# weipeilun/vjepa2

Hardware: AMD Instinct MI355X
Metric: clips/sec/GPU (ViT-L/16, 16×256², bf16) fwd+bwd; 1→8 GPU scaling (higher is better)
Workload: dtype bf16; 1 GPU; vit_large (RoPE) + predictor 12x384, 16x256^2 clips, B=24/GPU, JEPA train step: target fwd + ctx fwd/bwd (2 masks) + predictor fwd/bwd + L1 + AdamW + EMA; model=vit_large, global_batch=24, seq_len=2048, parallelism=dp1

## Files before the change

include/vjepa_hip.h:

```cpp
#ifndef VJEPA_HIP_H
#define VJEPA_HIP_H
#include <stddef.h>

#ifdef __cplusplus
extern "C" {
#endif

int vj_version(void);
int vj_header_crc(void);
int vj_get_last_error(char* buf, size_t n);
int vj_device_sync(void);

enum {
  VJ_EPI_BF16 = 0,
  VJ_EPI_F32 = 1,
  VJ_EPI_F32_RESID = 2,
  VJ_EPI_GELU = 3,
  VJ_EPI_GELU_BWD = 4,
  VJ_EPI_ROPE = 5,
  VJ_EPI_PARTIAL = 6,
  VJ_EPI_BF16_RESID = 7
};

int vj_gemm_bf16(int M, int N, int K, const void* A, long lda, int a_kmajor, const void* B, long ldb, int b_kmajor,
                 int epi, const float* bias, const void* aux, long ldaux, void* C, long ldc, void* C2, long ldc2,
                 void* stream);
int vj_gemm_bf16_splitk(int M, int N, int K, const void* A, long lda, int a_kmajor, const void* B, long ldb,
                        int b_kmajor, int epi, const float* bias, const void* aux, long ldaux, void* C, long ldc,
                        void* C2, long ldc2, int splitk, float* ws, long ws_floats, void* stream);
int vj_gemm_bf16_wgrad(int M, int N, int K, const void* dy, long lddy, const void* x, long ldx, float* dw, long lddw,
                       int accumulate, float* db, int db_accumulate, int splitk, float* ws, long ws_floats,
                       void* stream);

int vj_attn_fwd(int T, int H, int hd, const void* qkv, long ld, int q_off, int k_off, int v_off, void* o, long ldo,
                float* stats, float scale, int ngroups, const int* nseq, const int* len, void* stream);
int vj_attn_bwd(int T, int H, int hd, const void* qkv, long ld, int q_off, int k_off, int v_off, const void* o,
                long ldo, const void* dout, long lddo, float* stats, void* dqkv, long ldd, float scale, int ngroups,
                const int* nseq, const int* len, const int* rope_ids, int rope_mod, int rope_tpf, int rope_tpr,
                const float* cos_t, const float* sin_t, void* stream);
int vj_attn_fwd_fc(int T, int H, int hd, const void* qkv, long ld, int q_off, int k_off, int v_off, void* o, long ldo,
                   float* stats, float scale, int ngroups, const int* nseq, const int* len, int fblk, void* stream);
int vj_attn_bwd_fc(int T, int H, int hd, const void* qkv, long ld, int q_off, int k_off, int v_off, const void* o,
                   long ldo, const void* dout, long lddo, float* stats, void* dqkv, long ldd, float scale, int ngroups,
                   const int* nseq, const int* len, const int* rope_ids, int rope_mod, int rope_tpf, int rope_tpr,
                   const float* cos_t, const float* sin_t, int fblk, void* stream);
int vj_attn_fwd_ex(int T, int H, int hd, const void* qkv, long ld, int q_off, int k_off, int v_off, void* o, long ldo,
                   float* stats, float scale, int ngroups, const int* nseq, const int* len, int fblk, float dropout_p,
                   unsigned seed, void* stream);
int vj_attn_bwd_ex(int T, int H, int hd, const void* qkv, long ld, int q_off, int k_off, int v_off, const void* o,
                   long ldo, const void* dout, long lddo, float* stats, void* dqkv, long ldd, float scale, int ngroups,
                   const int* nseq, const int* len, const int* rope_ids, int rope_mod, int rope_tpf, int rope_tpr,
                   const float* cos_t, const float* sin_t, int fblk, float dropout_p, unsigned seed, void* stream);

int vj_qkv_rope_gemm(int M, int K, const void* A, long lda, const void* B, long ldb, const float* bias, void* C,
                     long ldc, int H, int hd, const int* ids, int ids_mod, int tpf, int tpr, const float* cos_t,
                     const float* sin_t, int npos, void* stream);

int vj_gemm_fp8(int M, int N, int K, const void* A, long lda, const int* ea, const void* B, long ldb, const int* eb,
                int epi, const float* bias, const void* aux, long ldaux, void* C, long ldc, void* C2, long ldc2,
                void* stream);
int vj_qkv_rope_gemm_fp8(int M, int K, const void* A, long lda, const int* ea, const void* B, long ldb, const int* eb,
                         const float* bias, void* C, long ldc, int H, int hd, const int* ids, int ids_mod, int tpf,
                         int tpr, const float* cos_t, const float* sin_t, int npos, void* stream);
int vj_quant_rows_fp8(int M, int K, const void* x, int x_bf16, long ldx, void* y8, long ldy, int* yexp, void* stream);
int vj_layernorm_fwd_fp8(int M, int D, const void* x, int x_bf16, long ldx, const float* gamma, const float* beta,
                         float eps, void* y8, long ldy, int* yexp, float* mean, float* rstd, void* stream);

int vj_layernorm_fwd(int M, int D, const void* x, int x_bf16, long ldx, const float* gamma, const float* beta,
                     float eps, void* y, int y_f32, long ldy, float* mean, float* rstd, void* stream);
int vj_layernorm_bwd_blocks(int M);
int vj_layernorm_bwd(int M, int D, const void* dy, long lddy, const float* x, long ldx, const float* mean,
                     const float* rstd, const float* gamma, const float* dres_in, long ldri, float* dres, long ldr,
                     void* dres_bf16, long ldrb, float* dgamma, float* dbeta, float* sum_in, float* sum_out, float* ws,
                     long ws_floats, void* stream);
int vj_layernorm_bwd_bf16(int M, int D, const void* dy, long lddy, const void* x, long ldx, const float* mean,
                          const float* rstd, const float* gamma, const void* dres_in, long ldri, void* dres, long ldr,
                          float* dgamma, float* dbeta, float* sum_in, float* sum_out, float* ws, long ws_floats,
                          void* stream);

int vj_gelu_eval(int n, const void* x, void* y, void* dy, void* stream);

int vj_colsum_f32(int M, int N, const void* x, int x_bf16, long ld, float* out, int accumulate, float* ws,
                  long ws_floats, void* stream);

int vj_rope(int T, int H, int hd, void* qkv, long ld, int q_off, int k_off, const int* ids, int ids_mod,
            int tokens_per_frame, int tokens_per_row, const float* cos_tab, const float* sin_tab, int half,
            int inverse, void* stream);

int vj_im2col_tubelet(int R, int K, const long* idx, int B, int C, int Tf, int Hf, int Wf, int tub, int pch,
                      const float* clip, void* out, void* stream);

int vj_gather_rows(int R, int rowbytes, const void* src, long src_ld_bytes, const int* idx, void* dst,
                   long dst_ld_bytes, int scatter, void* stream);
int vj_fill_rows(int R, int D, float* dst, long ldd, const int* idx, const float* vec, void* stream);
int vj_add_rows(int R, int D, float* dst, long ldd, const float* table, long ldt, int trows, const int* idx,
                int idx_mod, void* stream);

int vj_pred_index(int B, int K, int Kp, const long* mx, const long* my, int row0, int bmod, int N, int* pos,
                  int* ctx_dst, int* tgt_rows, int* loss_rows, void* stream);
int vj_ids64to32(long n, const long* in, int* out, void* stream);

int vj_jepa_loss(int R, int D, const void* z, int z_bf16, long ldz, const void* tgt, int tgt_bf16, long ldt,
                 const int* loss_rows,
                 const float* gamma, const float* beta, float eps1, float eps2, float loss_exp, int ngroups,
                 const int* group_rows, float pair_weight, void* dz, long lddz, float* row_loss, float* loss_out,
                 void* stream);

int vj_check_finite(long n, const float* g, int* found_inf, void* stream);
int vj_adamw(long n, float* p, const float* g, float* m, float* v, void* p_bf16, float lr, float beta1, float beta2,
             float eps, float weight_decay, int step, float grad_scale, const int* found_inf, void* stream);
int vj_ema(long n, float* target, const float* online, float momentum, void* target_bf16, void* stream);
int vj_adamw_ema(long n, float* p, const float* g, float* m, float* v, void* p_bf16, float lr, float beta1,
                 float beta2, float eps, float weight_decay, int step, float grad_scale, const int* found_inf,
                 float* target, void* target_bf16, float momentum, void* stream);
int vj_cast_bf16(long n, const float* in, void* out, void* stream);
int vj_proxy_copy(void* dst, const void* src, long bytes, int blocks, int mode, void* stream);
int vj_set_reserved_cus(int n);
int vj_gemm256_plan(int M, int N, int K, int a_kmajor, int b_kmajor, int epi, int cus, int* out6);
int vj_transpose_bf16(int rows, int cols, const void* src, long ld_src, void* dst, long ld_dst, void* stream);
int vj_transpose_bf16_batch(int n, const long* desc, long total_tiles, void* stream);

int vj_swiglu_fwd(int M, int h, const void* x12, long ld, void* out, long ldo, void* stream);
int vj_swiglu_bwd(int M, int h, const void* dh, long lddh, const void* x12, long ld, void* dx12, long lddx,
                  void* stream);
int vj_rowscale_add(int M, int N, const float* y, long ldy, const float* scale, const void* resid, long ldr, void* out,
                    long ldo, int bf16_resid, void* stream);
int vj_rowscale_bf16(int M, int N, const float* dx, long ld, const float* scale, void* out, long ldo, void* stream);
int vj_dropout(int M, int N, const void* x, long ldx, int x_f32, const void* aux, long ldaux, const void* resid,
               long ldr, int resid_f32, void* out, long ldo, float dropout_p, unsigned seed, void* stream);

int vj_mask_count(int B, int duration, int height, int width, int npred, const int* boxes, int t, int h, int w,
                  int max_ctx, int* counts, void* stream);
int vj_mask_emit(int B, int duration, int height, int width, int npred, const int* boxes, int t, int h, int w,
                 int max_ctx, int mode, int k_enc, int k_pred, long* enc, long* pred, void* stream);

int vj_video_transform(int B, int T, int H, int W, int C, int S, const void* frames, const int* params,
                       const float* mean, const float* stdv, float* out, void* stream);

int vj_xattn_ws_floats(int B, int nq, int N, int H, int hd, long* out);
int vj_xattn_fwd(int B, int nq, int N, int H, int hd, const void* q, long ldq, const void* kv, long ldkv, void* o,
                 long ldo, float* lse2, float scale, float* ws, long ws_floats, void* stream);
int vj_xattn_bwd(int B, int nq, int N, int H, int hd, const void* q, long ldq, const void* kv, long ldkv,
                 const void* o, long ldo, const void* dout, long lddo, const float* lse2, float scale, void* dq,
                 long lddq, void* dkv, long lddkv, float* ws, long ws_floats, void* stream);

int vj_xent(int V, int B, int C, const float* logits, long ld, const void* labels, int labels_i64, float* loss,
            float* row_loss, float* dlogits, long lddl, int* pred, int* correct, void* stream);

int vj_focal(int B, int nseg, const float* const* logits, const long* ld, const int* C, const void* const* labels,
             int labels_i64, const unsigned char* const* valid, float* const* dlogits, const long* lddl,
             int* const* tp, int* const* fn, float alpha, float gamma, int k, int loss_kind, float* loss,
             float* row_loss, int* hit, void* stream);

int vj_cem_sample(int S, int rollout, const float* noise, const float* mean, const float* std, float maxnorm,
                  float gripper_clip, const int* axis_on, const float* axis_val, int close_from, float* actions,
                  void* stream);
int vj_pose_step(int S, const float* pose, long ldp, const float* action, long lda, float* out, long ldo,
                 void* stream);
int vj_plan_frame(int S, int R, int D, const float* src, long src_sample_stride, long src_row_stride, int normalize,
                  float eps, float* dst, long dst_sample_stride, const float* goal, float* energy, void* stream);
int vj_cem_update(int S, int rollout, int k, const float* energy, const float* actions, double momentum_mean,
                  double momentum_std, double momentum_mean_gripper, double momentum_std_gripper, float* mean,
                  float* std, int* elite_idx, void* stream);

int vj_gemm_f32(int M, int N, int K, const float* A, long lda, const float* B, long ldb, int epi, const float* bias,
                const float* resid, long ldr, float* C, long ldc, float* C2, long ldc2, void* stream);
int vj_attn_fwd_f32(int T, int H, int hd, const float* qkv, long ld, int q_off, int k_off, int v_off, float* o,
                    long ldo, float* lse, float scale, int ngroups, const int* nseq, const int* len, void* stream);
int vj_rope_f32(int T, int H, int hd, float* qkv, long ld, int q_off, int k_off, const int* ids, int ids_mod,
                int tokens_per_frame, int tokens_per_row, const float* cos_tab, const float* sin_tab, int half,
                void* stream);
int vj_im2col_tubelet_f32(int R, int K, const long* idx, int B, int C, int Tf, int Hf, int Wf, int tub, int pch,
                          const float* clip, float* out, void* stream);

#ifdef __cplusplus
}
#endif
#endif
```

vjepa2_amd/_lib.py:

```python

import ctypes
import os

import torch

LIB_PATH = os.environ.get("VJ_LIB") or os.path.join(os.path.dirname(os.path.abspath(__file__)), "libvjepa_hip.so")

_P = ctypes.c_void_p
_I = ctypes.c_int
_L = ctypes.c_long
_F = ctypes.c_float
_U = ctypes.c_uint
_D = ctypes.c_double

SIGNATURES = {
    "vj_version": [],
    "vj_header_crc": [],
    "vj_get_last_error": [ctypes.c_char_p, ctypes.c_size_t],
    "vj_device_sync": [],
    "vj_gemm_bf16": [_I, _I, _I, _P, _L, _I, _P, _L, _I, _I, _P, _P, _L, _P, _L, _P, _L, _P],
    "vj_gemm_bf16_splitk": [_I, _I, _I, _P, _L, _I, _P, _L, _I, _I, _P, _P, _L, _P, _L, _P, _L, _I, _P, _L, _P],
    "vj_gemm_bf16_wgrad": [_I, _I, _I, _P, _L, _P, _L, _P, _L, _I, _P, _I, _I, _P, _L, _P],
    "vj_attn_fwd": [_I, _I, _I, _P, _L, _I, _I, _I, _P, _L, _P, _F, _I, _P, _P, _P],
    "vj_attn_bwd": [_I, _I, _I, _P, _L, _I, _I, _I, _P, _L, _P, _L, _P, _P, _L, _F, _I, _P, _P, _P, _I, _I, _I, _P,
                    _P, _P],
    "vj_attn_fwd_fc": [_I, _I, _I, _P, _L, _I, _I, _I, _P, _L, _P, _F, _I, _P, _P, _I, _P],
    "vj_attn_bwd_fc": [_I, _I, _I, _P, _L, _I, _I, _I, _P, _L, _P, _L, _P, _P, _L, _F, _I, _P, _P, _P, _I, _I, _I, _P,
                       _P, _I, _P],
    "vj_attn_fwd_ex": [_I, _I, _I, _P, _L, _I, _I, _I, _P, _L, _P, _F, _I, _P, _P, _I, _F, _U, _P],
    "vj_attn_bwd_ex": [_I, _I, _I, _P, _L, _I, _I, _I, _P, _L, _P, _L, _P, _P, _L, _F, _I, _P, _P, _P, _I, _I, _I, _P,
                       _P, _I, _F, _U, _P],
    "vj_qkv_rope_gemm": [_I, _I, _P, _L, _P, _L, _P, _P, _L, _I, _I, _P, _I, _I, _I, _P, _P, _I, _P],
    "vj_layernorm_fwd": [_I, _I, _P, _I, _L, _P, _P, _F, _P, _I, _L, _P, _P, _P],
    "vj_gemm_fp8": [_I, _I, _I, _P, _L, _P, _P, _L, _P, _I, _P, _P, _L, _P, _L, _P, _L, _P],
    "vj_qkv_rope_gemm_fp8": [_I, _I, _P, _L, _P, _P, _L, _P, _P, _P, _L, _I, _I, _P, _I, _I, _I, _P, _P, _I, _P],
    "vj_quant_rows_fp8": [_I, _I, _P, _I, _L, _P, _L, _P, _P],
    "vj_layernorm_fwd_fp8": [_I, _I, _P, _I, _L, _P, _P, _F, _P, _L, _P, _P, _P, _P],
    "vj_video_transform": [_I, _I, _I, _I, _I, _I, _P, _P, _P, _P, _P, _P],
    "vj_mask_count": [_I, _I, _I, _I, _I, _P, _I, _I, _I, _I, _P, _P],
    "vj_mask_emit": [_I, _I, _I, _I, _I, _P, _I, _I, _I, _I, _I, _I, _I, _P, _P, _P],
    "vj_gemm_f32": [_I, _I, _I, _P, _L, _P, _L, _I, _P, _P, _L, _P, _L, _P, _L, _P],
    "vj_attn_fwd_f32": [_I, _I, _I, _P, _L, _I, _I, _I, _P, _L, _P, _F, _I, _P, _P, _P],
    "vj_rope_f32": [_I, _I, _I, _P, _L, _I, _I, _P, _I, _I, _I, _P, _P, _I, _P],
    "vj_im2col_tubelet_f32": [_I, _I, _P, _I, _I, _I, _I, _I, _I, _I, _P, _P, _P],
    "vj_layernorm_bwd_blocks": [_I],
    "vj_layernorm_bwd": [_I, _I, _P, _L, _P, _L, _P, _P, _P, _P, _L, _P, _L, _P, _L, _P, _P, _P, _P, _P, _L, _P],
    "vj_gelu_eval": [_I, _P, _P, _P, _P],
    "vj_layernorm_bwd_bf16": [_I, _I, _P, _L, _P, _L, _P, _P, _P, _P, _L, _P, _L, _P, _P, _P, _P, _P, _L, _P],
    "vj_colsum_f32": [_I, _I, _P, _I, _L, _P, _I, _P, _L, _P],
    "vj_rope": [_I, _I, _I, _P, _L, _I, _I, _P, _I, _I, _I, _P, _P, _I, _I, _P],
    "vj_im2col_tubelet": [_I, _I, _P, _I, _I, _I, _I, _I, _I, _I, _P, _P, _P],
    "vj_gather_rows": [_I, _I, _P, _L, _P, _P, _L, _I, _P],
    "vj_fill_rows": [_I, _I, _P, _L, _P, _P, _P],
    "vj_add_rows": [_I, _I, _P, _L, _P, _L, _I, _P, _I, _P],
    "vj_pred_index": [_I, _I, _I, _P, _P, _I, _I, _I, _P, _P, _P, _P, _P],
    "vj_ids64to32": [_L, _P, _P, _P],
    "vj_jepa_loss": [_I, _I, _P, _I, _L, _P, _I, _L, _P, _P, _P, _F, _F, _F, _I, _P, _F, _P, _L, _P, _P, _P],
    "vj_check_finite": [_L, _P, _P, _P],
    "vj_adamw": [_L, _P, _P, _P, _P, _P, _F, _F, _F, _F, _F, _I, _F, _P, _P],
    "vj_ema": [_L, _P, _P, _F, _P, _P],
    "vj_adamw_ema": [_L, _P, _P, _P, _P, _P, _F, _F, _F, _F, _F, _I, _F, _P, _P, _P, _F, _P],
    "vj_cast_bf16": [_L, _P, _P, _P],
    "vj_proxy_copy": [_P, _P, _L, _I, _I, _P],
    "vj_set_reserved_cus": [_I],
    "vj_gemm256_plan": [_I, _I, _I, _I, _I, _I, _I, ctypes.POINTER(_I)],
    "vj_transpose_bf16": [_I, _I, _P, _L, _P, _L, _P],
    "vj_transpose_bf16_batch": [_I, _P, _L, _P],
    "vj_swiglu_fwd": [_I, _I, _P, _L, _P, _L, _P],
    "vj_swiglu_bwd": [_I, _I, _P, _L, _P, _L, _P, _L, _P],
    "vj_rowscale_add": [_I, _I, _P, _L, _P, _P, _L, _P, _L, _I, _P],
    "vj_rowscale_bf16": [_I, _I, _P, _L, _P, _P, _L, _P],
    "vj_dropout": [_I, _I, _P, _L, _I, _P, _L, _P, _L, _I, _P, _L, _F, _U, _P],
    "vj_xattn_ws_floats": [_I, _I, _I, _I, _I, ctypes.POINTER(_L)],
    "vj_xattn_fwd": [_I, _I, _I, _I, _I, _P, _L, _P, _L, _P, _L, _P, _F, _P, _L, _P],
    "vj_xattn_bwd": [_I, _I, _I, _I, _I, _P, _L, _P, _L, _P, _L, _P, _L, _P, _F, _P, _L, _P, _L, _P, _L, _P],
    "vj_xent": [_I, _I, _I, _P, _L, _P, _I, _P, _P, _P, _L, _P, _P, _P],
    "vj_focal": [_I, _I, _P, _P, _P, _P, _I, _P, _P, _P, _P, _P, _F, _F, _I, _I, _P, _P, _P, _P],
    "vj_cem_sample": [_I, _I, _P, _P, _P, _F, _F, _P, _P, _I, _P, _P],
    "vj_pose_step": [_I, _P, _L, _P, _L, _P, _L, _P],
    "vj_plan_frame": [_I, _I, _I, _P, _L, _L, _I, _F, _P, _L, _P, _P, _P],
    "vj_cem_update": [_I, _I, _I, _P, _P, _D, _D, _D, _D, _P, _P, _P, _P],
}

_lib = None


def load():
    global _lib
    if _lib is not None:
        return _lib
    if not os.path.exists(LIB_PATH):
        raise RuntimeError(
            f"{LIB_PATH} not found: the HIP extension is not built (run `python -m vjepa2_amd.build` or "
            "__graft_entry__.build()). There is no CPU fallback."
        )
    lib = ctypes.CDLL(LIB_PATH)
    for name, args in SIGNATURES.items():
        fn = getattr(lib, name, None)
        if fn is None:
            if os.environ.get("VJ_LIB"):
                continue
            raise RuntimeError(f"{LIB_PATH} does not export {name}: stale build (rebuild the extension)")
        fn.argtypes = args
        fn.restype = ctypes.c_int
    if not os.environ.get("VJ_LIB"):
        import zlib

        hdr = os.path.join(os.path.dirname(os.path.dirname(os.path.abspath(__file__))), "include", "vjepa_hip.h")
        crc_fn = getattr(lib, "vj_header_crc", None)
        if crc_fn is None:
            raise RuntimeError(f"{LIB_PATH} predates vj_header_crc: stale build (rebuild the extension)")
        with open(hdr, "rb") as f:
            want = zlib.crc32(f.read()) & 0xFFFFFFFF
        got = crc_fn() & 0xFFFFFFFF
        if got != want:
            raise RuntimeError(f"{LIB_PATH} was built from another include/vjepa_hip.h (crc {got:08x}, "
                               f"header {want:08x}): stale build (rebuild the extension)")
    _lib = lib
    return lib


def last_error():
    buf = ctypes.create_string_buffer(1024)
    load().vj_get_last_error(buf, 1024)
    return buf.value.decode(errors="replace")


def call(name, *args):
    rc = getattr(load(), name)(*args)
    if rc != 0:
        raise RuntimeError(f"{name} failed (code {rc}): {last_error()}")
    return rc


def int_array(vals):
    vals = list(vals)
    return (ctypes.c_int * max(1, len(vals)))(*vals)
```

vjepa2_amd/csrc/vj_common.h:

```cpp
#pragma once
#include <hip/hip_runtime.h>
#include <stdint.h>
#include <stdio.h>
#include <string.h>

typedef __bf16 bf16x8 __attribute__((ext_vector_type(8)));
typedef __bf16 bf16x4 __attribute__((ext_vector_type(4)));
typedef short s16x4 __attribute__((ext_vector_type(4)));
typedef short s16x8 __attribute__((ext_vector_type(8)));
typedef float f32x16 __attribute__((ext_vector_type(16)));
typedef float f32x4 __attribute__((ext_vector_type(4)));
typedef float f32x2 __attribute__((ext_vector_type(2)));
typedef int i32x4 __attribute__((ext_vector_type(4)));
typedef int i32x8 __attribute__((ext_vector_type(8)));
typedef unsigned short bf16_t;

#define LDS_AS __attribute__((address_space(3)))

enum {
  VJ_OK = 0,
  VJ_ERR_ARG = 1,
  VJ_ERR_LAUNCH = 2,
  VJ_ERR_UNSUPPORTED = 3,
};

void vj_set_error(const char* fmt, ...);

#define VJ_CHECK_ARG(cond, ...)          \
  do {                                   \
    if (!(cond)) {                       \
      vj_set_error(__VA_ARGS__);         \
      return VJ_ERR_ARG;                 \
    }                                    \
  } while (0)

#define VJ_LAUNCH_CHECK(what)                                                    \
  do {                                                                           \
    hipError_t e_ = hipGetLastError();                                           \
    if (e_ != hipSuccess) {                                                      \
      vj_set_error("%s: launch failed: %s", what, hipGetErrorString(e_));        \
      return VJ_ERR_LAUNCH;                                                      \
    }                                                                            \
  } while (0)

__device__ __forceinline__ float bf2f(bf16_t v) { return __uint_as_float(((uint32_t)v) << 16); }
__device__ __forceinline__ bf16_t f2bf(float f) {
  __bf16 b = (__bf16)f;
  return __builtin_bit_cast(bf16_t, b);
}
typedef __bf16 bf16x2_t __attribute__((ext_vector_type(2)));
__device__ __forceinline__ uint32_t pack_bf2(float lo, float hi) {
  return __builtin_bit_cast(uint32_t, __builtin_convertvector((f32x2){lo, hi}, bf16x2_t));
}

template <int CTRL>
__device__ __forceinline__ float dpp(float v) {
  return __int_as_float(__builtin_amdgcn_mov_dpp(__float_as_int(v), CTRL, 0xF, 0xF, false));
}
template <int CTRL>
__device__ __forceinline__ uint32_t dpp_u(uint32_t v) {
  return (uint32_t)__builtin_amdgcn_mov_dpp((int)v, CTRL, 0xF, 0xF, false);
}
constexpr int DPP_XOR1 = 0xB1;
constexpr int DPP_XOR2 = 0x4E;
constexpr int DPP_HALF_MIRROR = 0x141;
constexpr int DPP_MIRROR = 0x140;
__device__ __forceinline__ float sum_xor16(float v) {
  const auto r = __builtin_amdgcn_permlane16_swap(__float_as_uint(v), __float_as_uint(v), false, false);
  return __uint_as_float(r[0]) + __uint_as_float(r[1]);
}
__device__ __forceinline__ float sum_xor32(float v) {
  const auto r = __builtin_amdgcn_permlane32_swap(__float_as_uint(v), __float_as_uint(v), false, false);
  return __uint_as_float(r[0]) + __uint_as_float(r[1]);
}
__device__ __forceinline__ float max_xor16(float v) {
  const auto r = __builtin_amdgcn_permlane16_swap(__float_as_uint(v), __float_as_uint(v), false, false);
  return fmaxf(__uint_as_float(r[0]), __uint_as_float(r[1]));
}
__device__ __forceinline__ float max_xor32(float v) {
  const auto r = __builtin_amdgcn_permlane32_swap(__float_as_uint(v), __float_as_uint(v), false, false);
  return fmaxf(__uint_as_float(r[0]), __uint_as_float(r[1]));
}

__device__ __forceinline__ float wave_sum(float v) {
  v += dpp<DPP_XOR1>(v);
  v += dpp<DPP_XOR2>(v);
  v += dpp<DPP_HALF_MIRROR>(v);
  v += dpp<DPP_MIRROR>(v);
  v = sum_xor16(v);
  return sum_xor32(v);
}
__device__ __forceinline__ float wave_max(float v) {
  v = fmaxf(v, dpp<DPP_XOR1>(v));
  v = fmaxf(v, dpp<DPP_XOR2>(v));
  v = fmaxf(v, dpp<DPP_HALF_MIRROR>(v));
  v = fmaxf(v, dpp<DPP_MIRROR>(v));
  v = max_xor16(v);
  return max_xor32(v);
}

__device__ __forceinline__ __amdgpu_buffer_rsrc_t make_rsrc(const void* base, uint32_t bytes) {
  const unsigned long long a = (unsigned long long)base;
  const unsigned long long lo = (unsigned)__builtin_amdgcn_readfirstlane((int)(unsigned)a);
  const unsigned long long hi = (unsigned)__builtin_amdgcn_readfirstlane((int)(unsigned)(a >> 32));
  const int n = __builtin_amdgcn_readfirstlane((int)bytes);
  return __builtin_amdgcn_make_buffer_rsrc((void*)(lo | (hi << 32)), (short)0, n, 0x00020000);
}
#ifndef VJ_DMA_CPOL
#define VJ_DMA_CPOL 0
#endif
__device__ __forceinline__ void dma16(__amdgpu_buffer_rsrc_t r, LDS_AS void* lds_wave_base, uint32_t voff) {
  __builtin_amdgcn_raw_ptr_buffer_load_lds(r, lds_wave_base, 16, voff, 0, 0, VJ_DMA_CPOL);
}
#define VJ_OOB 0x80000000u

__device__ __forceinline__ s16x4 ds_read_tr16(const LDS_AS void* p) {
  return __builtin_amdgcn_ds_read_tr16_b64_v4i16((LDS_AS s16x4*)p);
}
__device__ __forceinline__ s16x4 ds_read_tr16_async(const LDS_AS void* p) {
  s16x4 r;
  asm volatile("ds_read_b64_tr_b16 %0, %1" : "=v"(r) : "v"((uint32_t)(uintptr_t)p) : "memory");
  return r;
}
__device__ __forceinline__ void lds_wait() { asm volatile("s_waitcnt lgkmcnt(0)" ::: "memory"); }
template <typename T, int N>
__device__ __forceinline__ void tie(T (&x)[N]) {
#pragma unroll
  for (int i = 0; i < N; ++i) asm volatile("" : "+v"(x[i]));
}

__device__ __forceinline__ uint32_t f8pack4(float a, float b, float c, float d) {
  int w = __builtin_amdgcn_cvt_pk_fp8_f32(__builtin_amdgcn_fmed3f(a, -448.f, 448.f),
                                          __builtin_amdgcn_fmed3f(b, -448.f, 448.f), 0, false);
  w = __builtin_amdgcn_cvt_pk_fp8_f32(__builtin_amdgcn_fmed3f(c, -448.f, 448.f),
                                      __builtin_amdgcn_fmed3f(d, -448.f, 448.f), w, true);
  return (uint32_t)w;
}

enum { EPI_BF16 = 0, EPI_F32 = 1, EPI_F32_RESID = 2, EPI_GELU = 3, EPI_GELU_BWD = 4, EPI_ROPE = 5, EPI_PARTIAL = 6,
       EPI_BF16_RESID = 7, EPI_PARTIAL_RS = 8 };

static inline int vj_cdiv(long a, long b) { return (int)((a + b - 1) / b); }

__device__ __forceinline__ void gelu_cdf_grad(float x, float& cdf, float& dy) {
  const float zs = x * 0.84932180028801904f;
  const float a = fabsf(zs);
  const float t = __builtin_amdgcn_rcpf(fmaf(0.27273748087922250f, a, 1.f));
  float p = fmaf(1.061405429f, t, -1.453152027f);
  p = fmaf(p, t, 1.421413741f);
  p = fmaf(p, t, -0.284496736f);
  p = fmaf(p, t, 0.254829592f);
  p *= t;
  const float e = __builtin_amdgcn_exp2f(-zs * zs);
  cdf = fmaf(0.5f, copysignf(fmaf(-p, e, 1.f), zs), 0.5f);
  dy = fmaf(x * 0.39894228040143268f, e, cdf);
}
__device__ __forceinline__ void gelu_fwd_grad(float x, float& y, float& dy) {
  float cdf;
  gelu_cdf_grad(x, cdf, dy);
  y = x * cdf;
}

struct VjRope {
  const int* ids;
  int mod, tpf, tpr;
  int half, hd, D;
  const float* cos_t;
  const float* sin_t;
  int npos;
};

__device__ __forceinline__ uint32_t clamp_u31(long b) {
  if (b < 0) return 0;
  return b > 0x7fffffffL ? 0x7fffffffu : (uint32_t)b;
}

__device__ __forceinline__ uint32_t drop_mix(uint32_t x) {
  x ^= x >> 16;
  x *= 0x7feb352du;
  x ^= x >> 15;
  x *= 0x846ca68bu;
  x ^= x >> 16;
  return x;
}
__device__ __forceinline__ uint32_t drop_row(uint32_t seed, uint32_t row) { return drop_mix(seed ^ (row * 0x9e3779b1u)); }
__device__ __forceinline__ uint32_t drop_u(uint32_t rowkey, uint32_t col) { return drop_mix(rowkey + col * 0x85ebca77u); }
uint32_t vj_drop_thresh(float p);
```

vjepa2_amd/csrc/vj_gemm.hip:

```cpp
#include <stdlib.h>
#include "vj_common.h"

namespace {


struct GemmArgs {
  const bf16_t* A;
  const bf16_t* B;
  int M, N, K;
  long lda, ldb;
  void* C;
  long ldc;
  void* C2;
  long ldc2;
  const float* bias;
  const void* aux;
  long ldaux;
  int kslice;
  float* ws;
  const float* rs_ws = nullptr;
  float* rs_out = nullptr;
  int rs_acc = 0;
};

// ... 35 lines not shown

template <bool KMAJ>
__device__ __forceinline__ bf16x8 load_frag(const LDS_AS char* lds, int rb, int s, int lane) {
  if constexpr (KMAJ) {
    const int r = rb + (lane & 31);
    const int c = (2 * s + (lane >> 5)) ^ ((r >> 1) & 7);
    return *(const LDS_AS bf16x8*)(lds + r * 128 + c * 16);
  } else {
    const int r = rb + 16 * ((lane >> 4) & 1) + 4 * (lane & 3);
    const int kr = 16 * s + 8 * (lane >> 5) + ((lane >> 2) & 3);
    const int sw = (kr & 3) << 2;
    const int off = ((r >> 3) ^ sw) * 16 + (r & 7) * 2;
    const s16x4 lo = ds_read_tr16(lds + kr * 256 + off);
    const s16x4 hi = ds_read_tr16(lds + (kr + 4) * 256 + off);
    s16x8 v = {lo[0], lo[1], lo[2], lo[3], hi[0], hi[1], hi[2], hi[3]};
    return __builtin_bit_cast(bf16x8, v);
  }
}

template <bool AK, bool BKM, int EPI>
__global__ __launch_bounds__(256) void k_gemm(GemmArgs g) {
  __shared__ __attribute__((aligned(16))) char smem_raw[4 * TILE_BYTES];
  LDS_AS char* smem = (LDS_AS char*)smem_raw;
  const int lane = threadIdx.x & 63;
  const int wave = threadIdx.x >> 6;
  const int wm = wave >> 1, wn = wave & 1;
  const int m0 = blockIdx.y * BM, n0 = blockIdx.x * BN;

  const bf16_t* abase = AK ? g.A + (long)m0 * g.lda : g.A + m0;
  const bf16_t* bbase = BKM ? g.B + (long)n0 * g.ldb : g.B + n0;
  const uint32_t abytes = AK ? clamp_bytes((long)(g.M - m0) * g.lda * 2) : clamp_bytes(((long)g.K * g.lda - m0) * 2);
  const uint32_t bbytes = BKM ? clamp_bytes((long)(g.N - n0) * g.ldb * 2) : clamp_bytes(((long)g.K * g.ldb - n0) * 2);
  const __amdgpu_buffer_rsrc_t ra = make_rsrc(abase, abytes);
  const __amdgpu_buffer_rsrc_t rb = make_rsrc(bbase, bbytes);
  const int mleft = g.M - m0, nleft = g.N - n0;

  f32x16 acc[2][2];
#pragma unroll
  for (int i = 0; i < 2; ++i)
#pragma unroll
    for (int j = 0; j < 2; ++j)
#pragma unroll
      for (int r = 0; r < 16; ++r) acc[i][j][r] = 0.f;

  const int kb = blockIdx.z * g.kslice;
  const int ke = min(g.K, kb + g.kslice);
  const int nk = (ke - kb + BK - 1) / BK;
  stage_tile<AK>(ra, g.lda, mleft, kb, ke, smem, wave, lane);
  stage_tile<BKM>(rb, g.ldb, nleft, kb, ke, smem + TILE_BYTES, wave, lane);
  __syncthreads();

  for (int kt = 0; kt < nk; ++kt) {
    const int cur = kt & 1;
    if (kt + 1 < nk) {
      LDS_AS char* nxt = smem + (cur ^ 1) * 2 * TILE_BYTES;
      stage_tile<AK>(ra, g.lda, mleft, kb + (kt + 1) * BK, ke, nxt, wave, lane);
      stage_tile<BKM>(rb, g.ldb, nleft, kb + (kt + 1) * BK, ke, nxt + TILE_BYTES, wave, lane);
    }
    const LDS_AS char* As = smem + cur * 2 * TILE_BYTES;
    const LDS_AS char* Bs = As + TILE_BYTES;
#pragma unroll
    for (int s = 0; s < 4; ++s) {
      bf16x8 a0 = load_frag<AK>(As, wm * 64, s, lane);
      bf16x8 a1 = load_frag<AK>(As, wm * 64 + 32, s, lane);
      bf16x8 b0 = load_frag<BKM>(Bs, wn * 64, s, lane);
      bf16x8 b1 = load_frag<BKM>(Bs, wn * 64 + 32, s, lane);
      acc[0][0] = __builtin_amdgcn_mfma_f32_32x32x16_bf16(a0, b0, acc[0][0], 0, 0, 0);
      acc[0][1] = __builtin_amdgcn_mfma_f32_32x32x16_bf16(a0, b1, acc[0][1], 0, 0, 0);
      acc[1][0] = __builtin_amdgcn_mfma_f32_32x32x16_bf16(a1, b0, acc[1][0], 0, 0, 0);
      acc[1][1] = __builtin_amdgcn_mfma_f32_32x32x16_bf16(a1, b1, acc[1][1], 0, 0, 0);
    }
    __syncthreads();
  }

#pragma unroll
  for (int j = 0; j < 2; ++j) {
    const int n = n0 + wn * 64 + j * 32 + (lane & 31);
    if (n >= g.N) continue;
    const float bv = (EPI != EPI_PARTIAL && g.bias) ? g.bias[n] : 0.f;
#pragma unroll
    for (int i = 0; i < 2; ++i) {
#pragma unroll
      for (int r = 0; r < 16; ++r) {
        const int m = m0 + wm * 64 + i * 32 + (r & 3) + 8 * (r >> 2) + 4 * (lane >> 5);
        if (m >= g.M) continue;
        const float v = acc[i][j][r] + bv;
        if constexpr (EPI == EPI_PARTIAL) {
          g.ws[((long)blockIdx.z * g.M + m) * g.N + n] = v;
        } else if constexpr (EPI == EPI_BF16) {
          ((bf16_t*)g.C)[(long)m * g.ldc + n] = f2bf(v);
        } else if constexpr (EPI == EPI_F32) {
          ((float*)g.C)[(long)m * g.ldc + n] = v;
        } else if constexpr (EPI == EPI_F32_RESID) {
          const float res = ((const float*)g.aux)[(long)m * g.ldaux + n];
          ((float*)g.C)[(long)m * g.ldc + n] = res + v;
        } else if constexpr (EPI == EPI_BF16_RESID) {
          const float res = bf2f(((const bf16_t*)g.aux)[(long)m * g.ldaux + n]);
          ((bf16_t*)g.C)[(long)m * g.ldc + n] = f2bf(res + v);
        } else if constexpr (EPI == EPI_GELU) {
          float y, dy;
          gelu_fwd_grad(bf2f(f2bf(v)), y, dy);
          if (g.C) ((bf16_t*)g.C)[(long)m * g.ldc + n] = f2bf(dy);
          ((bf16_t*)g.C2)[(long)m * g.ldc2 + n] = f2bf(y);
        } else if constexpr (EPI == EPI_GELU_BWD) {
          const float dg = bf2f(((const bf16_t*)g.aux)[(long)m * g.ldaux + n]);
          ((bf16_t*)g.C)[(long)m * g.ldc + n] = f2bf(acc[i][j][r] * dg);
        }
      }
    }
  }
}

__device__ __forceinline__ void reduce_rowsum(const GemmArgs& g, int splitk, int m) {
  float s = 0.f;
  for (int z = 0; z < splitk; ++z) s += g.rs_ws[(long)z * g.M + m];
  g.rs_out[m] = g.rs_acc ? g.rs_out[m] + s : s;
}

__global__ void k_splitk_reduce4(GemmArgs g, int splitk, int epi) {
  const long i = ((long)blockIdx.x * blockDim.x + threadIdx.x) * 4;
  const long total = (long)g.M * g.N;
  if (i >= total) return;
  const int m = (int)(i / g.N), n = (int)(i % g.N);
  if (g.rs_out && n == 0) reduce_rowsum(g, splitk, m);
  float4 v = g.bias ? *(const float4*)(g.bias + n) : make_float4(0.f, 0.f, 0.f, 0.f);
  for (int z = 0; z < splitk; ++z) {
    const float4 w = *(const float4*)(g.ws + (long)z * total + i);
    v.x += w.x; v.y += w.y; v.z += w.z; v.w += w.w;
  }
  if (epi == EPI_F32_RESID) {
    const float4 r = *(const float4*)((const float*)g.aux + (long)m * g.ldaux + n);
    *(float4*)((float*)g.C + (long)m * g.ldc + n) = make_float4(r.x + v.x, r.y + v.y, r.z + v.z, r.w + v.w);
  } else if (epi == EPI_F32) {
    *(float4*)((float*)g.C + (long)m * g.ldc + n) = v;
  } else {
    *(uint2*)((bf16_t*)g.C + (long)m * g.ldc + n) = make_uint2(pack_bf2(v.x, v.y), pack_bf2(v.z, v.w));
  }
}

__global__ void k_splitk_reduce(GemmArgs g, int splitk, int epi) {
  const long i = (long)blockIdx.x * blockDim.x + threadIdx.x;
  const long total = (long)g.M * g.N;
  if (i >= total) return;
  const int m = (int)(i / g.N), n = (int)(i % g.N);
  if (g.rs_out && n == 0) reduce_rowsum(g, splitk, m);
  float v = g.bias ? g.bias[n] : 0.f;
  for (int z = 0; z < splitk; ++z) v += g.ws[(long)z * total + i];
  if (epi == EPI_F32_RESID) {
    ((float*)g.C)[(long)m * g.ldc + n] = ((const float*)g.aux)[(long)m * g.ldaux + n] + v;
  } else if (epi == EPI_F32) {
    ((float*)g.C)[(long)m * g.ldc + n] = v;
  } else {
    ((bf16_t*)g.C)[(long)m * g.ldc + n] = f2bf(v);
  }
}

template <bool AK, bool BKM>
int launch_epi(int epi, const GemmArgs& g, dim3 grid, hipStream_t st) {
  switch (epi) {
    case EPI_PARTIAL: hipLaunchKernelGGL((k_gemm<AK, BKM, EPI_PARTIAL>), grid, dim3(256), 0, st, g); break;
    case EPI_BF16: hipLaunchKernelGGL((k_gemm<AK, BKM, EPI_BF16>), grid, dim3(256), 0, st, g); break;
    case EPI_F32: hipLaunchKernelGGL((k_gemm<AK, BKM, EPI_F32>), grid, dim3(256), 0, st, g); break;
    case EPI_F32_RESID: hipLaunchKernelGGL((k_gemm<AK, BKM, EPI_F32_RESID>), grid, dim3(256), 0, st, g); break;
    case EPI_GELU: hipLaunchKernelGGL((k_gemm<AK, BKM, EPI_GELU>), grid, dim3(256), 0, st, g); break;
    case EPI_GELU_BWD: hipLaunchKernelGGL((k_gemm<AK, BKM, EPI_GELU_BWD>), grid, dim3(256), 0, st, g); break;
    case EPI_BF16_RESID: hipLaunchKernelGGL((k_gemm<AK, BKM, EPI_BF16_RESID>), grid, dim3(256), 0, st, g); break;
    default: vj_set_error("vj_gemm_bf16: unknown epilogue %d", epi); return VJ_ERR_ARG;
  }
  VJ_LAUNCH_CHECK("vj_gemm_bf16");
  return VJ_OK;
}

}

int vj_gemm256_partial(int M, int N, int K, const void* A, long lda, int a_kmajor, const void* B, long ldb,
                       int b_kmajor, int kslice, int splitk, float* ws, hipStream_t st, float* rsum);
int vj_gemm256_dispatch(int M, int N, int K, const void* A, long lda, int a_kmajor, const void* B, long ldb,
                        int b_kmajor, int epi, const float* bias, const void* aux, long ldaux, void* C, long ldc,
                        void* C2, long ldc2, hipStream_t st, const void* rope);

static int gemm_splitk(int M, int N, int K, const void* A, long lda, int a_kmajor, const void* B, long ldb,
                       int b_kmajor, int epi, const float* bias, const void* aux, long ldaux, void* C, long ldc,
                       void* C2, long ldc2, int splitk, float* ws, long ws_floats, void* stream, float* rs_out,
                       int rs_acc, int* rs_done) {
  if (rs_done) *rs_done = 0;
  if (M == 0 || N == 0) return VJ_OK;
  VJ_CHECK_ARG(M > 0 && N > 0 && K > 0, "vj_gemm_bf16: bad dims M=%d N=%d K=%d", M, N, K);
  VJ_CHECK_ARG(epi == EPI_BF16 || epi == EPI_F32 || epi == EPI_F32_RESID || epi == EPI_GELU || epi == EPI_GELU_BWD ||
                   epi == EPI_BF16_RESID,
               "vj_gemm_bf16: epilogue %d is not a public epilogue (0-4, 7; include/vjepa_hip.h)", epi);
  VJ_CHECK_ARG(A && B, "vj_gemm_bf16: null operand");
  VJ_CHECK_ARG(((uintptr_t)A & 15) == 0 && ((uintptr_t)B & 15) == 0, "vj_gemm_bf16: operands must be 16-B aligned");
  VJ_CHECK_ARG(lda % 8 == 0 && ldb % 8 == 0, "vj_gemm_bf16: lda/ldb must be multiples of 8 (lda=%ld ldb=%ld)", lda, ldb);
  VJ_CHECK_ARG(a_kmajor ? (K % 8 == 0) : (M % 8 == 0), "vj_gemm_bf16: A contiguous dim must be %%8");
  VJ_CHECK_ARG(b_kmajor ? (K % 8 == 0) : (N % 8 == 0), "vj_gemm_bf16: B contiguous dim must be %%8");
  VJ_CHECK_ARG(a_kmajor ? lda >= K : lda >= M, "vj_gemm_bf16: lda too small");
  VJ_CHECK_ARG(b_kmajor ? ldb >= K : ldb >= N, "vj_gemm_bf16: ldb too small");
  VJ_CHECK_ARG(epi == EPI_GELU ? (C2 != nullptr) : (C != nullptr), "vj_gemm_bf16: null output");
  VJ_CHECK_ARG((epi != EPI_F32_RESID && epi != EPI_GELU_BWD && epi != EPI_BF16_RESID) || aux,
               "vj_gemm_bf16: epilogue needs aux");
  VJ_CHECK_ARG((a_kmajor ? (long)M * lda : (long)K * lda) * 2 < 0x7fffffffL, "vj_gemm_bf16: A too large");
  VJ_CHECK_ARG((b_kmajor ? (long)N * ldb : (long)K * ldb) * 2 < 0x7fffffffL, "vj_gemm_bf16: B too large");
  if (splitk < 1) splitk = 1;
  int kslice = K;
  if (splitk > 1) {
    VJ_CHECK_ARG(epi == EPI_BF16 || epi == EPI_F32 || epi == EPI_F32_RESID,
                 "vj_gemm_bf16_splitk: split-K supports the BF16/F32/F32_RESID epilogues");
    kslice = vj_cdiv(vj_cdiv(K, splitk), BK) * BK;
    splitk = vj_cdiv(K, kslice);
    VJ_CHECK_ARG(ws && ws_floats >= (long)splitk * M * N, "vj_gemm_bf16_splitk: workspace needs %ld floats",
                 (long)splitk * M * N);
  }
  GemmArgs g{(const bf16_t*)A, (const bf16_t*)B, M, N, K, lda, ldb, C, ldc, C2, ldc2, bias, aux, ldaux, kslice, ws};
  dim3 grid(vj_cdiv(N, BN), vj_cdiv(M, BM), splitk);
  VJ_CHECK_ARG(grid.y <= 65535, "vj_gemm_bf16: M too large");
  hipStream_t st = (hipStream_t)stream;
  if (splitk == 1 && M >= 1024 && N >= 128) {
    const int rc = vj_gemm256_dispatch(M, N, K, A, lda, a_kmajor, B, ldb, b_kmajor, epi, bias, aux, ldaux, C, ldc, C2,
                                       ldc2, st, nullptr);
    if (rc != VJ_ERR_UNSUPPORTED) return rc;
  }
  if (splitk > 1) {
    int rc = VJ_ERR_UNSUPPORTED;
    const bool rs = rs_out && ws_floats >= (long)splitk * M * N + (long)splitk * M;
    rc = vj_gemm256_partial(M, N, K, A, lda, a_kmajor, B, ldb, b_kmajor, kslice, splitk, ws, st,
                            rs ? ws + (long)splitk * M * N : nullptr);
    if (rc == VJ_OK && rs) {
      g.rs_ws = ws + (long)splitk * M * N;
      g.rs_out = rs_out;
      g.rs_acc = rs_acc;
      if (rs_done) *rs_done = 1;
    }
    if (rc == VJ_ERR_UNSUPPORTED) {
      if (a_kmajor && b_kmajor) rc = launch_epi<true, true>(EPI_PARTIAL, g, grid, st);
      else if (a_kmajor && !b_kmajor) rc = launch_epi<true, false>(EPI_PARTIAL, g, grid, st);
      else if (!a_kmajor && b_kmajor) rc = launch_epi<false, true>(EPI_PARTIAL, g, grid, st);
      else rc = launch_epi<false, false>(EPI_PARTIAL, g, grid, st);
    }
    if (rc) return rc;
    const long total = (long)M * N;
    const bool vec = N % 4 == 0 && ldc % 4 == 0 && (epi != EPI_F32_RESID || ldaux % 4 == 0) &&
                     ((uintptr_t)C & 15) == 0 && ((uintptr_t)aux & 15) == 0 && ((uintptr_t)bias & 15) == 0;
    if (vec)
      hipLaunchKernelGGL(k_splitk_reduce4, dim3((unsigned)((total / 4 + 255) / 256)), dim3(256), 0, st, g, splitk, epi);
    else
      hipLaunchKernelGGL(k_splitk_reduce, dim3((unsigned)((total + 255) / 256)), dim3(256), 0, st, g, splitk, epi);
    VJ_LAUNCH_CHECK("vj_gemm_bf16_splitk(reduce)");
    return VJ_OK;
  }
  if (a_kmajor && b_kmajor) return launch_epi<true, true>(epi, g, grid, st);
  if (a_kmajor && !b_kmajor) return launch_epi<true, false>(epi, g, grid, st);
  if (!a_kmajor && b_kmajor) return launch_epi<false, true>(epi, g, grid, st);
  return launch_epi<false, false>(epi, g, grid, st);
}

extern "C" int vj_gemm_bf16_splitk(int M, int N, int K, const void* A, long lda, int a_kmajor, const void* B,
                                   long ldb, int b_kmajor, int epi, const float* bias, const void* aux, long ldaux,
                                   void* C, long ldc, void* C2, long ldc2, int splitk, float* ws, long ws_floats,
                                   void* stream) {
  return gemm_splitk(M, N, K, A, lda, a_kmajor, B, ldb, b_kmajor, epi, bias, aux, ldaux, C, ldc, C2, ldc2, splitk, ws,
                     ws_floats, stream, nullptr, 0, nullptr);
}

extern "C" int vj_colsum_f32(int M, int N, const void* x, int x_bf16, long ld, float* out, int accumulate, float* ws,
                             long ws_floats, void* stream);

extern "C" int vj_gemm_bf16_wgrad(int M, int N, int K, const void* dy, long lddy, const void* x, long ldx,
                                  float* dw, long lddw, int accumulate, float* db, int db_accumulate, int splitk,
                                  float* ws, long ws_floats, void* stream) {
  VJ_CHECK_ARG(dw, "vj_gemm_bf16_wgrad: null dw");
  int done = 0;
  const int rc = gemm_splitk(M, N, K, dy, lddy, 0, x, ldx, 0, accumulate ? EPI_F32_RESID : EPI_F32, nullptr,
                             accumulate ? dw : nullptr, lddw, dw, lddw, nullptr, 0, splitk, ws, ws_floats, stream, db,
                             db_accumulate, &done);
  if (rc || !db || done || M == 0) return rc;
  return vj_colsum_f32(K, M, dy, 1, lddy, db, db_accumulate, ws, ws_floats, stream);
}

extern "C" int vj_gemm_bf16(int M, int N, int K, const void* A, long lda, int a_kmajor, const void* B, long ldb,
                            int b_kmajor, int epi, const float* bias, const void* aux, long ldaux, void* C, long ldc,
                            void* C2, long ldc2, void* stream) {
  return vj_gemm_bf16_splitk(M, N, K, A, lda, a_kmajor, B, ldb, b_kmajor, epi, bias, aux, ldaux, C, ldc, C2, ldc2, 1,
                             nullptr, 0, stream);
}
```

vjepa2_amd/csrc/vj_gemm256.hip:

```cpp
#include <stdlib.h>
#include <atomic>
#include <type_traits>
#include "vj_gemm_tile.h"

namespace {

#if VJ_GEMM_STAMPS
__device__ long vj_gemm_stamps[2048 * 16 * 4];
__device__ long vj_gemm_istamps[2048 * 2 * 16];
#endif

template <int N>
__device__ __forceinline__ void vm_wait() {
  static_assert(N >= 0 && N <= 24 && N % 4 == 0, "vm_wait: add the count");
  if constexpr (N == 0) asm volatile("s_waitcnt vmcnt(0)" ::: "memory");
  else if constexpr (N == 4) asm volatile("s_waitcnt vmcnt(4)" ::: "memory");
  else if constexpr (N == 8) asm volatile("s_waitcnt vmcnt(8)" ::: "memory");
  else if constexpr (N == 12) asm volatile("s_waitcnt vmcnt(12)" ::: "memory");
  else if constexpr (N == 16) asm volatile("s_waitcnt vmcnt(16)" ::: "memory");
  else if constexpr (N == 20) asm volatile("s_waitcnt vmcnt(20)" ::: "memory");
  else asm volatile("s_waitcnt vmcnt(24)" ::: "memory");
}

template <bool AK, bool BKM, int EPI, int BN, bool F8 = false, int NWV = 8, int BMT = 256, int STG = 0>
__global__ __launch_bounds__(NWV * 64, 2) void k_gemm256(G256 g) {
  using Cfg = Cfg256<AK, BKM, EPI, BN, F8, NWV, BMT, STG>;
  static_assert(Cfg::supported, "k_gemm256: unsupported (layout, epilogue, tile) combination");
  constexpr bool PART = Cfg::PART, RS = Cfg::RS, DIRECT = Cfg::DIRECT, AUX = Cfg::AUX, F32OUT = Cfg::F32OUT;
  constexpr bool EARLY1 = Cfg::EARLY1, GTAB = Cfg::GTAB, S64 = Cfg::S64, ASYNC = Cfg::ASYNC;
  constexpr int BM = Cfg::BM, MH = Cfg::MH, BK = Cfg::BK, NT = Cfg::NT, WNX = Cfg::WNX, WM = Cfg::WM, WN = Cfg::WN;
  constexpr int PB = Cfg::PB, NTN = Cfg::NTN, A_BYTES = Cfg::A_BYTES, STAGE = Cfg::STAGE, DMAW = Cfg::DMAW;
  constexpr int NSL = Cfg::NSL, DIST = Cfg::DIST, USZ = Cfg::USZ, GSZ = Cfg::GSZ, SA = Cfg::SA, SB = Cfg::SB;
  constexpr int EA = Cfg::EA, EB = Cfg::EB, WRS = Cfg::WRS;
  static_assert(EA >= 2 && EB >= 3, "S64 waits assume at least one interval of DMA lead");
  static_assert(Cfg::SLOT_END <= Cfg::LDS_BYTES && Cfg::GTAB_END <= Cfg::LDS_BYTES && Cfg::RING_END <= Cfg::LDS_BYTES &&
                    Cfg::S64_END <= Cfg::RING_END && Cfg::TAB_END <= Cfg::LDS_BYTES && Cfg::RTAB_END <= Cfg::LDS_BYTES &&
                    Cfg::IMG_END <= Cfg::SLOT_END,
                "an LDS region ends past the array");
  static_assert(Cfg::lds_disjoint, "LDS regions overlap");
  static_assert(Cfg::LDS_BYTES * Cfg::BLOCKS_PER_CU <= LDS_PER_CU, "the CU's workgroups exceed its LDS");
  auto rowoff = [](int i) { return S64 ? (i >> 2) * 128 + (i & 3) * 16 : i * 16; };
  __shared__ __attribute__((aligned(16))) char smem_raw[Cfg::LDS_BYTES];
  LDS_AS char* smem = (LDS_AS char*)smem_raw;
  [[maybe_unused]] LDS_AS char* ring = smem + Cfg::RING0;

  const int lane = threadIdx.x & 63;
  const int wave = __builtin_amdgcn_readfirstlane(threadIdx.x >> 6);
  const int wr = wave / WNX, wc = wave % WNX;

  const int ntile = g.tiles_m * g.tiles_n;
  const int nb = ntile * g.nsplit;
  const int P = gridDim.x >> 3;
  const int xcd = blockIdx.x & 7, jb = blockIdx.x >> 3;
  const int q = nb >> 3, rmd = nb & 7;
  const int run0 = xcd < rmd ? xcd * (q + 1) : rmd * (q + 1) + (xcd - rmd) * q;
  const int runend = run0 + q + (xcd < rmd ? 1 : 0);
  if (run0 + jb >= runend) return;

  auto make_tile = [&](int wg) {
    Tile T;
    const int z = wg / ntile, w = wg - z * ntile;
    int tm, tn;
    if (g.group > 0) {
      const int per = g.group * g.tiles_n, grp = w / per, first = grp * g.group;
      const int gm = min(g.tiles_m - first, g.group), loc = w - grp * per;
      tm = first + loc % gm;
      tn = loc / gm;
    } else {
      tm = w / g.tiles_n;
      tn = w - tm * g.tiles_n;
    }
    T.m0 = __builtin_amdgcn_readfirstlane(tm * BM);
    T.n0 = __builtin_amdgcn_readfirstlane(tn * BN);
    T.z = __builtin_amdgcn_readfirstlane(z);
    const int kb = T.z * g.kslice;
    T.Keff = min(g.K, kb + g.kslice) - kb;
    T.nk = (T.Keff + BK - 1) / BK;
    return T;
  };
  auto rsrc_a = [&](const Tile& T) {
    const int kb = T.z * g.kslice;
    const bf16_t* abase = AK ? g.A + (long)T.m0 * g.lda + kb : g.A + (long)kb * g.lda + T.m0;
    return make_rsrc(abase, AK ? clampb((long)(g.M - T.m0) * g.lda * 2 - kb * 2L)
                               : clampb(((long)(g.K - kb) * g.lda - T.m0) * 2));
  };
  auto rsrc_b = [&](const Tile& T) {
    const int kb = T.z * g.kslice;
    const bf16_t* bbase = BKM ? g.B + (long)T.n0 * g.ldb + kb : g.B + (long)kb * g.ldb + T.n0;
    return make_rsrc(bbase, BKM ? clampb((long)(g.N - T.n0) * g.ldb * 2 - kb * 2L)
                                : clampb(((long)(g.K - kb) * g.ldb - T.n0) * 2));
  };
  const bool iss = DMAW == 8 || wave < DMAW;
  auto load_k = [&](__amdgpu_buffer_rsrc_t ra, __amdgpu_buffer_rsrc_t rb, const Tile& T, int t, int slot,
                    int lane) {
    LDS_AS char* s = smem + slot * STAGE;
    if (iss) {
      stage<AK, BM, false, DMAW, BK, WNX, PB>(ra, g.lda, g.M - T.m0, t * BK, T.Keff, s, wave, lane);
      stage<BKM, BN, DIRECT, DMAW, BK, WNX, PB>(rb, g.ldb, g.N - T.n0, t * BK, T.Keff, s + A_BYTES, wave, lane);
    }
  };
  auto load_tile = [&](const Tile& T, int t, int slot, int lane) {
    load_k(rsrc_a(T), rsrc_b(T), T, t, slot, lane);
  };
  auto load_tile8 = [&](const Tile& T, int t, int slot, int lane) {
    LDS_AS char* s = smem + slot * STAGE;
    stage<AK, BM, false, NWV, BK, WNX, PB>(rsrc_a(T), g.lda, g.M - T.m0, t * BK, T.Keff, s, wave, lane);
    stage<BKM, BN, DIRECT, NWV, BK, WNX, PB>(rsrc_b(T), g.ldb, g.N - T.n0, t * BK, T.Keff, s + A_BYTES, wave, lane);
  };

  constexpr int RTR = EPI == EPI_ROPE ? (ROPE_TAB_MAX + NT - 1) / NT : 0;
  [[maybe_unused]] f32x2 rpf[RTR > 0 ? RTR : 1];
  [[maybe_unused]] const int ntab = EPI == EPI_ROPE ? g.rope.npos * g.rope.half : 0;
  if constexpr (EPI == EPI_ROPE) {
#pragma unroll
    for (int i = 0; i < RTR; ++i) {
      const int e = threadIdx.x + NT * i;
      rpf[i] = e < ntab ? f32x2{g.rope.cos_t[e], g.rope.sin_t[e]} : f32x2{0.f, 0.f};
    }
  }
  [[maybe_unused]] LDS_AS int* rpos = (LDS_AS int*)(smem + Cfg::RPOS_OFF);
  [[maybe_unused]] LDS_AS f32x2* rtab = (LDS_AS f32x2*)(smem + Cfg::RTAB_OFF);

  int wg = run0 + jb;
  Tile cur = make_tile(wg);
  int par = 0;

  [[maybe_unused]] const int nku = STG ? (g.K + 31) / 32 : 0;
  [[maybe_unused]] int dwg = wg, dku = 0, dpos = 0;
  [[maybe_unused]] __amdgpu_buffer_rsrc_t drs;
  [[maybe_unused]] uint32_t dvo[4];
  const bool isA = wave < 4;
  auto dma_setup = [&]() {
    if (dwg < runend) {
      const Tile T = make_tile(dwg);
      const int left = isA ? g.M - T.m0 : g.N - T.n0;
      const long ld = isA ? g.lda : g.ldb;
      if (isA) drs = make_rsrc(g.A + (long)T.m0 * g.lda, clampb((long)left * g.lda * 2));
      else drs = make_rsrc(g.B + (long)T.n0 * g.ldb, clampb((long)left * g.ldb * 2));
#pragma unroll
      for (int j = 0; j < 4; ++j) {
        const int r = (4 * (wave & 3) + j) * 16 + (lane >> 2);
        const int c = (lane & 3) ^ kswz32(r);
        int gr = r;
        if (!isA) {
          const int rl = r & 63;
          gr = (r - rl) + 4 * (rl & 15) + (rl >> 4);
        }
        dvo[j] = gr < left ? (uint32_t)(gr * ld * 2 + c * 16) : VJ_OOB;
      }
    } else {
#pragma unroll
      for (int j = 0; j < 4; ++j) dvo[j] = VJ_OOB;
    }
  };
  auto dma_half = [&](auto h_c) {
    constexpr int h = decltype(h_c)::value;
    LDS_AS char* dst = ring + (dpos % NSL) * USZ + (isA ? 0 : 16384) + (4 * (wave & 3) + 2 * h) * 1024;
    const int soff = __builtin_amdgcn_readfirstlane(dku * 64);
    __builtin_amdgcn_raw_ptr_buffer_load_lds(drs, dst, 16, dvo[2 * h], soff, 0, 0);
    __builtin_amdgcn_raw_ptr_buffer_load_lds(drs, dst + 1024, 16, dvo[2 * h + 1], soff, 0, 0);
    if constexpr (h == 1) {
      ++dpos;
      if (++dku == nku) {
        dku = 0;
        dwg += P;
        dma_setup();
      }
    }
  };
  [[maybe_unused]] const int nks = S64 ? g.K >> 6 : 0;
  [[maybe_unused]] const long dld = isA ? g.lda : g.ldb;
  [[maybe_unused]] const bf16_t* dbase = isA ? g.A : g.B;
  [[maybe_unused]] int dleft = 0, dq = 0, dk = 0, q64 = 0;
  auto dma_setup64 = [&]() {
    if (dwg < runend) {
      const Tile T = make_tile(dwg);
      dbase = isA ? g.A + (long)T.m0 * g.lda : g.B + (long)T.n0 * g.ldb;
      dleft = isA ? g.M - T.m0 : g.N - T.n0;
    } else {
      dleft = 0;
    }
  };
  auto dma_gran = [&]() {
    const int h = dk & 1;
    const __amdgpu_buffer_rsrc_t rs = make_rsrc(dbase + (h ? 128 * dld : 0), clampb((long)(dleft - 128 * h) * dld * 2));
    const int soff = __builtin_amdgcn_readfirstlane((dk >> 1) * 128);
    LDS_AS char* dst = ring + (isA ? dq % SA : SA + dq % SB) * GSZ + (wave & 3) * 4096;
#pragma unroll
    for (int k = 0; k < 4; ++k)
      __builtin_amdgcn_raw_ptr_buffer_load_lds(rs, dst + k * 1024, 16, dvo[k], soff, 0, 0);
    ++dq;
    if (++dk == 2 * nks) {
      dk = 0;
      dwg += P;
      dma_setup64();
    }
  };
  if constexpr (S64) {
#pragma unroll
    for (int k = 0; k < 4; ++k) {
      const int r = 32 * (wave & 3) + 8 * k + (lane >> 3);
      const int c = (lane & 7) ^ ((r >> 1) & 7);
      const int rl = r & 63;
      const int gr = isA ? r : (r - rl) + 4 * (rl & 15) + (rl >> 4);
      dvo[k] = (uint32_t)(gr * dld * 2 + c * 16);
    }
    dma_setup64();
    for (int i = 0; i < (isA ? EA : EB); ++i) dma_gran();
  } else if constexpr (STG) {
    dma_setup();
#pragma unroll
    for (int i = 0; i < DIST; ++i) {
      dma_half(std::integral_constant<int, 0>{});
      dma_half(std::integral_constant<int, 1>{});
    }
  } else {
    load_tile(cur, 0, 0, lane);
    if (cur.nk > 1) load_tile(cur, 1, 1, lane);
  }
  if constexpr (EPI == EPI_ROPE) {
#pragma unroll
    for (int i = 0; i < RTR; ++i) {
      const int e = threadIdx.x + NT * i;
      if (e < ntab) rtab[e] = rpf[i];
    }
  }
  if constexpr (GTAB) gelu_tab_fill((LDS_AS f32x2*)(smem + Cfg::GTAB_OFF), threadIdx.x, NT);

  f32x4 acc[2 * MH][NTN];
  auto accv = [&](int i, int j, int r) -> float { return acc[i][j][r]; };
  auto accs = [&](int i, int j, int r, float v) { acc[i][j][r] = v; };
  bf16x8 Aa[MH], Ab[MH], Ba[NTN], Bb[NTN];
  auto rdA = [&](bf16x8 (&X)[MH], int slot, int mh, int ks) {
    const LDS_AS char* s = smem + slot * STAGE;
#pragma unroll
    for (int i = 0; i < MH; ++i) X[i] = frag<AK, BM, BK>(s, wr * WM + (mh * MH + i) * 16, ks, lane);
  };
  auto rdB = [&](bf16x8 (&Y)[NTN], int slot, int ks) {
    const LDS_AS char* s = smem + slot * STAGE + A_BYTES;
#pragma unroll
    for (int j = 0; j < NTN; ++j) Y[j] = frag<BKM, BN, BK>(s, wc * WN + j * 16, ks, lane);
  };
  [[maybe_unused]] int f8sa[8], f8sb[NTN];
  [[maybe_unused]] i32x8 Xa[2], Xb[2], Y8[NTN];
  auto cat = [](bf16x8 lo, bf16x8 hi) {
    const i32x4 l = __builtin_bit_cast(i32x4, lo), h = __builtin_bit_cast(i32x4, hi);
    return __builtin_shufflevector(l, h, 0, 1, 2, 3, 4, 5, 6, 7);
  };
  auto rdA8 = [&](i32x8 (&X)[2], int slot, int qq) {
    const LDS_AS char* s = smem + slot * STAGE;
#pragma unroll
    for (int i = 0; i < 2; ++i)
      X[i] = cat(frag<AK, BM>(s, wr * 128 + (2 * qq + i) * 16, 0, lane),
                 frag<AK, BM>(s, wr * 128 + (2 * qq + i) * 16, 1, lane));
  };
  auto rdB8 = [&](int j0, int j1, int slot) {
    const LDS_AS char* s = smem + slot * STAGE + A_BYTES;
#pragma unroll
    for (int j = j0; j < j1; ++j)
      Y8[j] = cat(frag<BKM, BN>(s, wc * WN + j * 16, 0, lane), frag<BKM, BN>(s, wc * WN + j * 16, 1, lane));
  };
  auto mm8 = [&](const i32x8 (&X)[2], int qq, int j0, int j1) {
#pragma unroll
    for (int i = 0; i < 2; ++i)
#pragma unroll
      for (int j = j0; j < j1; ++j)
        acc[2 * qq + i][j] = __builtin_amdgcn_mfma_scale_f32_16x16x128_f8f6f4(X[i], Y8[j], acc[2 * qq + i][j], 0, 0,
                                                                              0, f8sa[2 * qq + i], 0, f8sb[j]);
  };
  [[maybe_unused]] float rsa = 0.f, rsb = 0.f;
  [[maybe_unused]] bool rs_on = false;
  auto rsum8 = [](const bf16x8& x, float s) {
    typedef __bf16 bf16x2_t __attribute__((ext_vector_type(2)));
    const bf16x2_t one = {(__bf16)1.0f, (__bf16)1.0f};
    s = __builtin_amdgcn_fdot2_f32_bf16(__builtin_shufflevector(x, x, 0, 1), one, s, false);
    s = __builtin_amdgcn_fdot2_f32_bf16(__builtin_shufflevector(x, x, 2, 3), one, s, false);
    s = __builtin_amdgcn_fdot2_f32_bf16(__builtin_shufflevector(x, x, 4, 5), one, s, false);
    return __builtin_amdgcn_fdot2_f32_bf16(__builtin_shufflevector(x, x, 6, 7), one, s, false);
  };
  auto rs_phase = [&](const bf16x8 (&X)[MH], int mh) {
    if constexpr (RS && MH == 4) {
      if (rs_on && (wc >> 1) == mh) {
        if (wc & 1) {
          rsa = rsum8(X[2], rsa);
          rsb = rsum8(X[3], rsb);
        } else {
          rsa = rsum8(X[0], rsa);
          rsb = rsum8(X[1], rsb);
        }
      }
    }
  };
  auto mm = [&](const bf16x8 (&X)[MH], int mh, const bf16x8 (&Y)[NTN]) {
#pragma unroll
    for (int i = 0; i < MH; ++i)
#pragma unroll
      for (int j = 0; j < NTN; ++j)
        acc[mh * MH + i][j] = __builtin_amdgcn_mfma_f32_16x16x32_bf16(X[i], Y[j], acc[mh * MH + i][j], 0, 0, 0);
    rs_phase(X, mh);
  };
  auto mm_rows = [&](const bf16x8 (&X)[MH], int mh, const bf16x8 (&Y)[NTN], int i0, int i1) {
#pragma unroll
    for (int i = 0; i < MH; ++i)
      if (i >= i0 && i < i1)
#pragma unroll
        for (int j = 0; j < NTN; ++j)
          acc[mh * MH + i][j] = __builtin_amdgcn_mfma_f32_16x16x32_bf16(X[i], Y[j], acc[mh * MH + i][j], 0, 0, 0);
    if (i1 == MH) rs_phase(X, mh);
  };
  auto release = [&](bf16x8 (&X)[MH], bf16x8 (&Y)[NTN]) {
    if constexpr (ASYNC) {
      lds_wait();
      tie(X);
      tie(Y);
    }
  };

#if VJ_GEMM_STAMPS
  int stamp_it = 0;
#endif
  for (;;) {
#if VJ_GEMM_STAMPS
    const long st0 = __builtin_amdgcn_s_memtime();
    long st_k1 = 0;
#endif
    const int wgn = wg + P;
    const bool has_next = wgn < runend;
    const int nk = cur.nk;
    const int parn = (nk + par) & 1;
    const int sle = (nk - 1 + par) & 1;
    [[maybe_unused]] int pf_id = 0;
    if constexpr (EPI == EPI_ROPE) {
      const int t = threadIdx.x;
      if (t < BM && cur.m0 + t < g.M) pf_id = g.rope.ids ? g.rope.ids[cur.m0 + t] : (cur.m0 + t) % g.rope.mod;
    }
#pragma unroll
    for (int i = 0; i < 2 * MH; ++i)
#pragma unroll
      for (int j = 0; j < NTN; ++j) acc[i][j] = f32x4{0.f, 0.f, 0.f, 0.f};
    if constexpr (RS) {
      rs_on = g.rsum && cur.n0 == 0;
      rsa = rsb = 0.f;
    }
    if constexpr (F8) {
#pragma unroll
      for (int i = 0; i < 8; ++i) {
        const int m = cur.m0 + wr * 128 + i * 16 + (lane & 15);
        f8sa[i] = 127 + (m < g.M ? g.ea[m] : 0);
      }
#pragma unroll
      for (int j = 0; j < NTN; ++j) {
        int r = wc * WN + j * 16 + (lane & 15);
        if constexpr (DIRECT) {
          const int rl = r % WN;
          r = (r - rl) + NTN * (rl & 15) + (rl >> 4);
        }
        const int n = cur.n0 + r;
        f8sb[j] = 127 + (n < g.N ? g.eb[n] : 0);
      }
    }
    [[maybe_unused]] float biasp[NTN];
    if constexpr (STG) {
      const int nbp = cur.n0 + wc * WN + NTN * (lane & 15);
#pragma unroll
      for (int j = 0; j < NTN; ++j) biasp[j] = 0.f;
      if (EPI != EPI_GELU_BWD && g.bias && nbp < g.N) {
        const float4 bv = *(const float4*)(g.bias + nbp);
        biasp[0] = bv.x; biasp[1] = bv.y; biasp[2] = bv.z; biasp[3] = bv.w;
      }
    }
    [[maybe_unused]] f32x4 auxr[AUX && STG ? 4 : 1];
    auto stg_aux = [&] {
      if constexpr (AUX && STG) {
        const int m = cur.m0 + wr * WRS + 4 * (lane >> 4);
        const int n = cur.n0 + wc * WN + NTN * (lane & 15);
#pragma unroll
        for (int r = 0; r < 4; ++r) {
          const bool ok = m + r < g.M && n < g.N;
          const long off = ok ? (long)(m + r) * g.ldaux + n : 0;
          if constexpr (EPI == EPI_F32_RESID) {
            auxr[r] = *(const f32x4*)((const float*)g.aux + off);
          } else {
            const uint2 x = *(const uint2*)((const bf16_t*)g.aux + off);
            auxr[r] = f32x4{__builtin_bit_cast(float, x.x), __builtin_bit_cast(float, x.y), 0.f, 0.f};
          }
        }
      }
    };
    if constexpr (S64) {
      if (wg == run0 + jb) {
        if (isA) vm_wait<4 * (EA - 1)>();
        else vm_wait<4 * (EB - 2)>();
        __builtin_amdgcn_s_barrier();
        if (wr == 1) __builtin_amdgcn_s_barrier();
      }
      auto bar = [] {
        __builtin_amdgcn_sched_barrier(0);
        __builtin_amdgcn_s_barrier();
        __builtin_amdgcn_sched_barrier(0);
      };
      auto mm64 = [&](auto h_c) {
        constexpr int h = decltype(h_c)::value;
#pragma unroll
        for (int i = 0; i < 4; ++i)
#pragma unroll
          for (int j = 0; j < 4; ++j)
            acc[4 * h + i][j] = __builtin_amdgcn_mfma_f32_16x16x32_bf16(Aa[i], Ba[j], acc[4 * h + i][j], 0, 0, 0);
#pragma unroll
        for (int i = 0; i < 4; ++i)
#pragma unroll
          for (int j = 0; j < 4; ++j)
            acc[4 * h + i][j] = __builtin_amdgcn_mfma_f32_16x16x32_bf16(Ab[i], Bb[j], acc[4 * h + i][j], 0, 0, 0);
      };
      const int qt = q64;
#if VJ_GEMM_STAMPS
      long* ist = (stamp_it == 1 && (wave & 3) == 0 && lane == 0 && blockIdx.x < 2048)
                      ? vj_gemm_istamps + ((long)blockIdx.x * 2 + (wave >> 2)) * 16 : nullptr;
      auto istamp = [&](int s, int k) {
        if (ist && s >= 1 && s <= 4) ist[(s - 1) * 4 + k] = __builtin_amdgcn_s_memtime();
      };
#else
      auto istamp = [](int, int) {};
#endif
      for (int s = 0; s < nks; ++s) {
        const int p = qt + 2 * s;
        const LDS_AS char* sA0 = ring + (p % SA) * GSZ;
        const LDS_AS char* sA1 = ring + ((p + 1) % SA) * GSZ;
        const LDS_AS char* sB = ring + (SA + (p + (wc >> 1)) % SB) * GSZ;
        const bool last = s + 1 == nks;
#pragma unroll
        for (int i = 0; i < 4; ++i) Aa[i] = frag<true, 128, 64>(sA0, wr * 64 + i * 16, 0, lane);
#pragma unroll
        for (int j = 0; j < 4; ++j) Ba[j] = frag<true, 128, 64>(sB, (wc & 1) * 64 + j * 16, 0, lane);
#pragma unroll
        for (int i = 0; i < 4; ++i) Ab[i] = frag<true, 128, 64>(sA0, wr * 64 + i * 16, 1, lane);
#pragma unroll
        for (int j = 0; j < 4; ++j) Bb[j] = frag<true, 128, 64>(sB, (wc & 1) * 64 + j * 16, 1, lane);
        dma_gran();
        if (isA) vm_wait<4 * (EA - 1)>();
        if (AUX && last) stg_aux();
        bar();
        istamp(s, 0);
        mm64(std::integral_constant<int, 0>{});
        bar();
        istamp(s, 1);
#pragma unroll
        for (int i = 0; i < 4; ++i) Aa[i] = frag<true, 128, 64>(sA1, wr * 64 + i * 16, 0, lane);
#pragma unroll
        for (int i = 0; i < 4; ++i) Ab[i] = frag<true, 128, 64>(sA1, wr * 64 + i * 16, 1, lane);
        dma_gran();
        constexpr int WA = 4 * (EA - 1), WB = 4 * (EB - 2);
        if (AUX && last) {
          if (isA) vm_wait<WA + 4>();
          else vm_wait<WB + 4>();
        } else {
          if (isA) vm_wait<WA>();
          else vm_wait<WB>();
        }
        bar();
        istamp(s, 2);
        mm64(std::integral_constant<int, 1>{});
#if VJ_GEMM_STAMPS
        if (s == 0) st_k1 = __builtin_amdgcn_s_memtime();
#endif
        if (!last || wr == 0) bar();
        istamp(s, 3);
      }
      q64 = qt + 2 * nks;
    } else if constexpr (STG) {
      if (wg == run0 + jb) {
        if constexpr (DIST == 3) asm volatile("s_waitcnt vmcnt(8)" ::: "memory");
        else asm volatile("s_waitcnt vmcnt(4)" ::: "memory");
        __builtin_amdgcn_s_barrier();
        if (wr == 1) __builtin_amdgcn_s_barrier();
      }
      const int q0 = dpos - DIST;
      auto bar = [] {
        __builtin_amdgcn_sched_barrier(0);
        __builtin_amdgcn_s_barrier();
        __builtin_amdgcn_sched_barrier(0);
      };
      for (int u = 0; u < nku; ++u) {
        const LDS_AS char* sA = ring + ((q0 + u) % NSL) * USZ;
        const LDS_AS char* sB = sA + 16384;
#pragma unroll
        for (int i = 0; i < 4; ++i) Aa[i] = frag<true, 256, 32>(sA, wr * 128 + i * 16, 0, lane);
#pragma unroll
        for (int j = 0; j < NTN; ++j) Ba[j] = frag<true, 256, 32>(sB, wc * WN + j * 16, 0, lane);
#pragma unroll
        for (int i = 0; i < 4; ++i) Ab[i] = frag<true, 256, 32>(sA, wr * 128 + 64 + i * 16, 0, lane);
        dma_half(std::integral_constant<int, 0>{});
        dma_half(std::integral_constant<int, 1>{});
        if (AUX && u == nku - 1 && nku > 1) {
          if constexpr (DIST == 3) asm volatile("s_waitcnt vmcnt(12)" ::: "memory");
          else asm volatile("s_waitcnt vmcnt(8)" ::: "memory");
        } else {
          if constexpr (DIST == 3) asm volatile("s_waitcnt vmcnt(8)" ::: "memory");
          else asm volatile("s_waitcnt vmcnt(4)" ::: "memory");
        }
        if (AUX && u == nku - 2) stg_aux();
        if (AUX && nku == 1) stg_aux();
        bar();
        mm(Aa, 0, Ba);
        mm(Ab, 1, Ba);
#if VJ_GEMM_STAMPS
        if (u == 1) st_k1 = __builtin_amdgcn_s_memtime();
#endif
        if (u + 1 < nku || wr == 0) bar();
      }
    } else {
      asm volatile("s_waitcnt vmcnt(0)" ::: "memory");
      __syncthreads();
      if constexpr (F8) {
        rdA8(Xa, par, 0);
        rdB8(0, NTN / 2, par);
      } else {
        rdA(Aa, par, 0, 0);
        rdB(Ba, par, 0);
      }

      const __amdgpu_buffer_rsrc_t ra = rsrc_a(cur), rb = rsrc_b(cur);
      constexpr bool SPREAD = NWV == 8 && !F8 && BK == 64;
      constexpr int SPLIT = MH == 4 ? SPLIT_AT : MH - 1;
      auto ktile = [&](const int t, auto tail_c) {
        constexpr bool TAIL = decltype(tail_c)::value;
        const int sl = (t + par) & 1;
        if constexpr (F8) {
          rdB8(NTN / 2, NTN, sl);
          rdA8(Xb, sl, 1);
          __builtin_amdgcn_sched_barrier(0);
          mm8(Xa, 0, 0, NTN / 2);
          mm8(Xa, 0, NTN / 2, NTN);
          __builtin_amdgcn_sched_barrier(0);
          rdA8(Xa, sl, 2);
          __builtin_amdgcn_sched_barrier(0);
          mm8(Xb, 1, 0, NTN);
          __builtin_amdgcn_sched_barrier(0);
          rdA8(Xb, sl, 3);
          __builtin_amdgcn_sched_barrier(0);
          mm8(Xa, 2, 0, NTN);
          __builtin_amdgcn_sched_barrier(0);
        } else if constexpr (BK == 32) {
          rdA(Ab, sl, 1, 0);
          __builtin_amdgcn_sched_barrier(0);
          mm(Aa, 0, Ba);
          __builtin_amdgcn_sched_barrier(0);
        } else {
          release(Aa, Ba);
          rdA(Ab, sl, 1, 0);
          __builtin_amdgcn_sched_barrier(0);
          mm(Aa, 0, Ba);
          __builtin_amdgcn_sched_barrier(0);
          release(Ab, Ba);
          rdA(Aa, sl, 0, 1);
          rdB(Bb, sl, 1);
          __builtin_amdgcn_sched_barrier(0);
          mm(Ab, 1, Ba);
          __builtin_amdgcn_sched_barrier(0);
          release(Aa, Bb);
          rdA(Ab, sl, 1, 1);
          __builtin_amdgcn_sched_barrier(0);
          mm(Aa, 0, Bb);
          __builtin_amdgcn_sched_barrier(0);
        }
        if (t + 1 < nk) asm volatile("s_waitcnt vmcnt(0) lgkmcnt(0)" ::: "memory");
        else asm volatile("s_waitcnt lgkmcnt(0)" ::: "memory");
        if constexpr (ASYNC) {
          tie(Ab);
          tie(Bb);
        }
        __builtin_amdgcn_s_barrier();
        __builtin_amdgcn_sched_barrier(0);
        if constexpr (!TAIL) {
          if constexpr (SPREAD) {
            if (iss)
              stage<AK, BM, false, DMAW, BK, WNX, PB>(ra, g.lda, g.M - cur.m0, (t + 2) * BK, cur.Keff,
                                                       smem + sl * STAGE, wave, lane);
          } else {
            load_k(ra, rb, cur, t + 2, sl, lane);
          }
        } else if (has_next) {
          int lt = lane;
          asm volatile("" : "+v"(lt));
          const Tile nx = make_tile(wgn);
          if (t + 2 == nk) {
            load_tile(nx, 0, sl, lt);
          } else {
            if (nk == 1) load_tile(nx, 0, sl ^ 1, lt);
            if (EARLY1 && nx.nk > 1) load_tile8(nx, 1, sl, lt);
          }
        }
        auto b_pieces = [&] {
          if (iss)
            stage<BKM, BN, DIRECT, DMAW, BK, WNX, PB>(rb, g.ldb, g.N - cur.n0, (t + 2) * BK, cur.Keff,
                                                       smem + sl * STAGE + A_BYTES, wave, lane);
        };
        if constexpr (F8) {
          if (t + 1 < nk) rdA8(Xa, sl ^ 1, 0);
          __builtin_amdgcn_sched_barrier(0);
          mm8(Xb, 3, 0, NTN / 2);
          __builtin_amdgcn_sched_barrier(0);
          if (t + 1 < nk) rdB8(0, NTN / 2, sl ^ 1);
          __builtin_amdgcn_sched_barrier(0);
          mm8(Xb, 3, NTN / 2, NTN);
          __builtin_amdgcn_sched_barrier(0);
        } else if constexpr (BK == 32) {
          mm(Ab, 1, Ba);
          __builtin_amdgcn_sched_barrier(0);
          if (t + 1 < nk) {
            rdA(Aa, sl ^ 1, 0, 0);
            rdB(Ba, sl ^ 1, 0);
          }
          __builtin_amdgcn_sched_barrier(0);
        } else {
          if (t + 1 < nk) {
            rdA(Aa, sl ^ 1, 0, 0);
            rdB(Ba, sl ^ 1, 0);
          }
          __builtin_amdgcn_sched_barrier(0);
          if constexpr (SPREAD && !TAIL) {
            mm_rows(Ab, 1, Bb, 0, SPLIT);
            __builtin_amdgcn_sched_barrier(0);
            b_pieces();
            __builtin_amdgcn_sched_barrier(0);
            mm_rows(Ab, 1, Bb, SPLIT, MH);
          } else {
            mm(Ab, 1, Bb);
          }
          __builtin_amdgcn_sched_barrier(0);
        }
      };
      int t = 0;
      for (; t + 2 < nk; ++t) ktile(t, std::false_type{});
      for (; t < nk; ++t) ktile(t, std::true_type{});
    }

#if VJ_GEMM_STAMPS
    const long st1 = __builtin_amdgcn_s_memtime();
#endif
    int lane_e = lane;
    asm volatile("" : "+v"(lane_e));
    if constexpr (DIRECT) {
      const int lane = lane_e;
      const int lrow = 4 * (lane >> 4);
      const int nb = cur.n0 + wc * WN + NTN * (lane & 15);
      const bool nok = nb < g.N;
      const int mb = cur.m0 + wr * WRS + lrow;
      float bias[NTN];
#pragma unroll
      for (int j = 0; j < NTN; ++j) bias[j] = STG ? biasp[j] : 0.f;
      if (!STG && EPI != EPI_GELU_BWD && !PART && g.bias && nok)
#pragma unroll
        for (int j = 0; j < NTN; ++j) bias[j] = g.bias[nb + j];
      [[maybe_unused]] bool ract[NTN / 2];
      [[maybe_unused]] int rsh[NTN / 2], rf0[NTN / 2], rf1[NTN / 2];
      if constexpr (EPI == EPI_ROPE) {
        const RopeP& r = g.rope;
        const int t = threadIdx.x;
        if (t < BM) {
          const int fr = pf_id / r.tpf, rem = pf_id - r.tpf * fr, hr = rem / r.tpr;
          rpos[t] = fr | (hr << 10) | ((rem - r.tpr * hr) << 20);
        }
        const int sw = 2 * r.half, e0 = (nb % r.D) % r.hd;
#pragma unroll
        for (int p = 0; p < NTN / 2; ++p) {
          const int e = e0 + 2 * p, ax = e / sw, js = e - ax * sw;
          ract[p] = nok && nb < 2 * r.D && e < 3 * sw;
          rsh[p] = 10 * ax;
          rf0[p] = js % r.half;
          rf1[p] = (js + 1) % r.half;
        }
        __syncthreads();
      }
      [[maybe_unused]] float aux[AUX_PF + 1][4][NTN];
      [[maybe_unused]] const long off_aux = AUX ? (long)mb * g.ldaux + nb : 0;
      auto fetch = [&](int i, float (&dst)[4][NTN]) {
#pragma unroll
        for (int r = 0; r < 4; ++r) {
          const int m = mb + rowoff(i) + r;
          const bool ok = m < g.M && nok;
          const long off = ok ? off_aux + (long)(rowoff(i) + r) * g.ldaux : 0;
          if constexpr (EPI == EPI_F32_RESID) {
            if constexpr (NTN == 4) {
              const float4 x = *(const float4*)((const float*)g.aux + off);
              dst[r][0] = x.x; dst[r][1] = x.y; dst[r][2] = x.z; dst[r][3] = x.w;
            } else {
              const float2 x = *(const float2*)((const float*)g.aux + off);
              dst[r][0] = x.x; dst[r][1] = x.y;
            }
          } else {
            if constexpr (NTN == 4) {
              const uint2 x = *(const uint2*)((const bf16_t*)g.aux + off);
              dst[r][0] = bf_lo(x.x); dst[r][1] = bf_hi(x.x);
              dst[r][2] = bf_lo(x.y); dst[r][3] = bf_hi(x.y);
            } else {
              const uint32_t x = *(const uint32_t*)((const bf16_t*)g.aux + off);
              dst[r][0] = bf_lo(x); dst[r][1] = bf_hi(x);
            }
          }
        }
      };
      const bool odd = lane & 1;
      const int nb8 = nb - (odd ? 4 : 0);
      const bool nok8 = nb8 < g.N;
      const int mrow = mb + (odd ? 2 : 0);
      auto store_wide = [&](bf16_t* base, long ld, long off, int i, const uint32_t (&pk)[4][2]) {
        uint32_t snd[4], keep[4], rcv[4];
#pragma unroll
        for (int k = 0; k < 4; ++k) {
          snd[k] = odd ? pk[k >> 1][k & 1] : pk[2 + (k >> 1)][k & 1];
          keep[k] = odd ? pk[2 + (k >> 1)][k & 1] : pk[k >> 1][k & 1];
        }
#pragma unroll
        for (int k = 0; k < 4; ++k) rcv[k] = dpp_u<DPP_XOR1>(snd[k]);
#pragma unroll
        for (int h = 0; h < 2; ++h) {
          if (mrow + rowoff(i) + h < g.M && nok8) {
            const uint32_t a = 2 * h, b = 2 * h + 1;
            const uint4 v = make_uint4(odd ? rcv[a] : keep[a], odd ? rcv[b] : keep[b], odd ? keep[a] : rcv[a],
                                       odd ? keep[b] : rcv[b]);
            *(uint4*)(base + off + (long)(rowoff(i) + h) * ld) = v;
          }
        }
      };
      [[maybe_unused]] const long off_c = (long)mrow * g.ldc + nb8;
      [[maybe_unused]] const long off_c2 = EPI == EPI_GELU ? (long)mrow * g.ldc2 + nb8 : 0;
      [[maybe_unused]] const long off_f = PART ? ((long)cur.z * g.M + mb) * g.N + nb
                                                             : (long)mb * g.ldc + nb;
      [[maybe_unused]] const long ld_f = PART ? (long)g.N : g.ldc;
      [[maybe_unused]] float* const base_f = PART ? g.ws : (float*)g.C;
      if constexpr (AUX)
#pragma unroll
        for (int i = 0; i < AUX_PF; ++i) {
          if constexpr (STG) {
            static_assert(AUX_PF == 1, "STG prefetches one m-tile of aux rows");
#pragma unroll
            for (int r = 0; r < 4; ++r) {
              if constexpr (EPI == EPI_F32_RESID) {
#pragma unroll
                for (int j = 0; j < NTN; ++j) aux[0][r][j] = auxr[r][j];
              } else {
                aux[0][r][0] = bf_lo(auxr[r][0]); aux[0][r][1] = bf_hi(auxr[r][0]);
                aux[0][r][2] = bf_lo(auxr[r][1]); aux[0][r][3] = bf_hi(auxr[r][1]);
              }
            }
          } else {
            fetch(i, aux[i]);
          }
        }
      auto rows = [&](auto save_c) {
      constexpr bool SAVE_D = decltype(save_c)::value;
#pragma unroll
      for (int i = 0; i < 2 * MH; ++i) {
        if constexpr (AUX) {
          if (i + AUX_PF < 2 * MH) fetch(i + AUX_PF, aux[(i + AUX_PF) % (AUX_PF + 1)]);
          if (!STG && i == 2 * MH - 1 - AUX_PF && has_next) {
            const Tile nxt = make_tile(wgn);
            if (nxt.nk > 1) load_tile8(nxt, 1, sle, lane);
          }
        }
        if constexpr (F32OUT && NTN == 4) {
#pragma unroll
          for (int a = 0; a < 4; ++a)
#pragma unroll
            for (int b = a + 1; b < 4; ++b) {
              float x = accv(i, a, b), y = accv(i, b, a);
              asm volatile("v_swap_b32 %0, %1" : "+v"(x), "+v"(y));
              accs(i, a, b, x);
              accs(i, b, a, y);
            }
#pragma unroll
          for (int r = 0; r < 4; ++r)
#pragma unroll
            for (int e = 0; e < 4; ++e) {
              float x = accv(i, r, e);
              asm volatile("v_add_f32 %0, %0, %1" : "+v"(x) : "v"(bias[e]));
              if constexpr (EPI == EPI_F32_RESID) asm volatile("v_add_f32 %0, %0, %1" : "+v"(x) : "v"(aux[i % (AUX_PF + 1)][r][e]));
              accs(i, r, e, x);
            }
#pragma unroll
          for (int r = 0; r < 4; ++r) {
            const int m = mb + rowoff(i) + r;
            if (m < g.M && nok) {
              float* dst = base_f + off_f + (long)(rowoff(i) + r) * ld_f;
              *(f32x4*)dst = acc[i][r];
            }
          }
          continue;
        }
        [[maybe_unused]] uint32_t pk[4][2], ga[4][2];
#pragma unroll
        for (int r = 0; r < 4; ++r) {
          const int m = mb + rowoff(i) + r;
          float v[NTN];
#pragma unroll
          for (int j = 0; j < NTN; ++j) v[j] = accv(i, j, r) + bias[j];
          if constexpr (EPI == EPI_ROPE) {
            const int rp = rpos[wr * WRS + rowoff(i) + lrow + r];
#pragma unroll
            for (int p = 0; p < NTN / 2; ++p) {
              if (!ract[p]) continue;
              const int pos = min((rp >> rsh[p]) & 1023, g.rope.npos - 1) * g.rope.half;
              const f32x2 a = rtab[pos + rf0[p]], b = rtab[pos + rf1[p]];
              const float x0 = v[2 * p], x1 = v[2 * p + 1];
              v[2 * p] = x0 * a[0] - x1 * a[1];
              v[2 * p + 1] = x1 * b[0] + x0 * b[1];
            }
          }
          if constexpr (EPI == EPI_F32_RESID || EPI == EPI_BF16_RESID) {
#pragma unroll
            for (int j = 0; j < NTN; ++j) v[j] += aux[i % (AUX_PF + 1)][r][j];
          }
          if constexpr (F32OUT) {
            if (m < g.M && nok) {
              float* dst = base_f + off_f + (long)(rowoff(i) + r) * ld_f;
              *(float4*)dst = make_float4(v[0], v[1], v[2], v[3]);
            }
          } else {
#pragma unroll
            for (int q2 = 0; q2 < 2; ++q2) {
              if constexpr (EPI == EPI_GELU_BWD)
                pk[r][q2] = pack_bf2(v[2 * q2] * aux[i % (AUX_PF + 1)][r][2 * q2],
                                     v[2 * q2 + 1] * aux[i % (AUX_PF + 1)][r][2 * q2 + 1]);
              else
                pk[r][q2] = pack_bf2(v[2 * q2], v[2 * q2 + 1]);
              if constexpr (EPI == EPI_GELU) {
                if constexpr (GTAB) ga[r][q2] = gelu_pair_tab<SAVE_D>(pk[r][q2], smem + Cfg::GTAB_OFF, &pk[r][q2]);
                else ga[r][q2] = gelu_pair(pk[r][q2], SAVE_D ? &pk[r][q2] : nullptr);
              }
            }
          }
        }
        if constexpr (!F32OUT) {
          if (EPI != EPI_GELU || SAVE_D) store_wide((bf16_t*)g.C, g.ldc, off_c, i, pk);
          if constexpr (EPI == EPI_GELU) store_wide((bf16_t*)g.C2, g.ldc2, off_c2, i, ga);
        }
      }
      };
      if (EPI == EPI_GELU && g.C) rows(std::true_type{});
      else rows(std::false_type{});
    } else {
      const int lane = lane_e;
      constexpr int STR = Cfg::STR, LPR = Cfg::LPR, RPI = Cfg::RPI, MTP = Cfg::MTP, PR = Cfg::PR, IT = Cfg::IT;
      LDS_AS float* wl = (LDS_AS float*)(smem + sle * STAGE + wave * PR * STR * 4);
      if constexpr (RS && MH == 4) {
        if (rs_on) {
          float sa = rsa + __shfl_xor(rsa, 16), sb = rsb + __shfl_xor(rsb, 16);
          sa += __shfl_xor(sa, 32);
          sb += __shfl_xor(sb, 32);
          const int m = cur.m0 + wr * 128 + 32 * wc + (lane & 31);
          if (lane < 32 && m < g.M) g.rsum[(long)cur.z * g.M + m] = lane < 16 ? sa : sb;
        }
      }
      bool ract[2] = {false, false};
      int rsh[2] = {0, 0}, rf0[2] = {0, 0}, rf1[2] = {0, 0};
      const int col = (lane % LPR) * 4;
      const int ncol = cur.n0 + wc * WN + col;
      if constexpr (EPI == EPI_ROPE) {
        const RopeP& r = g.rope;
        const int t = threadIdx.x;
        if (t < BM) {
          const int fr = pf_id / r.tpf, rem = pf_id - r.tpf * fr, hr = rem / r.tpr;
          rpos[t] = fr | (hr << 10) | ((rem - r.tpr * hr) << 20);
        }
        const int sw = 2 * r.half, e0 = (ncol % r.D) % r.hd;
#pragma unroll
        for (int p = 0; p < 2; ++p) {
          const int e = e0 + 2 * p, ax = e / sw, js = e - ax * sw;
          ract[p] = ncol < 2 * r.D && e < 3 * sw;
          rsh[p] = 10 * ax;
          rf0[p] = js % r.half;
          rf1[p] = (js + 1) % r.half;
        }
        __syncthreads();
      }
      float4 bias4 = make_float4(0.f, 0.f, 0.f, 0.f);
      if (EPI != EPI_GELU_BWD && !PART && g.bias && ncol < g.N) bias4 = *(const float4*)(g.bias + ncol);
#pragma unroll
      for (int pass = 0; pass < 8 / MTP; ++pass) {
#pragma unroll
        for (int ii = 0; ii < MTP; ++ii)
#pragma unroll
          for (int j = 0; j < NTN; ++j)
#pragma unroll
            for (int r = 0; r < 4; ++r)
              wl[(ii * 16 + (lane >> 4) * 4 + r) * STR + j * 16 + (lane & 15)] = acc[pass * MTP + ii][j][r];
        __builtin_amdgcn_s_waitcnt(0xc07f);
        [[maybe_unused]] float4 rres[EPI == EPI_F32_RESID ? IT : 1];
        [[maybe_unused]] uint2 rpre[EPI == EPI_GELU_BWD || EPI == EPI_BF16_RESID ? IT : 1];
        if constexpr (AUX) {
#pragma unroll
          for (int it = 0; it < IT; ++it) {
            const int m = cur.m0 + wr * 128 + pass * PR + it * RPI + lane / LPR;
            const bool ok = m < g.M && ncol < g.N;
            const long mm2 = ok ? m : 0;
            const int nn = ok ? ncol : 0;
            if constexpr (EPI == EPI_F32_RESID) rres[it] = *(const float4*)((const float*)g.aux + mm2 * g.ldaux + nn);
            else rpre[it] = *(const uint2*)((const bf16_t*)g.aux + mm2 * g.ldaux + nn);
          }
        }
#pragma unroll
        for (int it = 0; it < IT; ++it) {
          const int row = it * RPI + lane / LPR;
          const f32x4 v4 = *(const LDS_AS f32x4*)(wl + row * STR + col);
          const int m = cur.m0 + wr * 128 + pass * PR + row;
          const int n = ncol;
          if (m >= g.M || n >= g.N) continue;
          float v[4] = {v4[0] + bias4.x, v4[1] + bias4.y, v4[2] + bias4.z, v4[3] + bias4.w};
          if constexpr (EPI == EPI_BF16 || EPI == EPI_ROPE) {
            if constexpr (EPI == EPI_ROPE) {
              const int rp = rpos[wr * 128 + pass * PR + row];
#pragma unroll
              for (int p = 0; p < 2; ++p) {
                if (!ract[p]) continue;
                const int pos = min((rp >> rsh[p]) & 1023, g.rope.npos - 1) * g.rope.half;
                const f32x2 a = rtab[pos + rf0[p]], b = rtab[pos + rf1[p]];
                const float x0 = v[2 * p], x1 = v[2 * p + 1];
                v[2 * p] = x0 * a[0] - x1 * a[1];
                v[2 * p + 1] = x1 * b[0] + x0 * b[1];
              }
            }
            *(uint2*)((bf16_t*)g.C + (long)m * g.ldc + n) = make_uint2(pack_bf2(v[0], v[1]), pack_bf2(v[2], v[3]));
          } else if constexpr (EPI == EPI_F32) {
            *(float4*)((float*)g.C + (long)m * g.ldc + n) = make_float4(v[0], v[1], v[2], v[3]);
          } else if constexpr (PART) {
            *(float4*)(g.ws + ((long)cur.z * g.M + m) * g.N + n) = make_float4(v[0], v[1], v[2], v[3]);
          } else if constexpr (EPI == EPI_F32_RESID) {
            const float4 rr = rres[it];
            *(float4*)((float*)g.C + (long)m * g.ldc + n) = make_float4(rr.x + v[0], rr.y + v[1], rr.z + v[2], rr.w + v[3]);
          } else if constexpr (EPI == EPI_GELU) {
            uint32_t d0, d1;
            const uint32_t a0 = gelu_pair(pack_bf2(v[0], v[1]), &d0), a1 = gelu_pair(pack_bf2(v[2], v[3]), &d1);
            if (g.C) *(uint2*)((bf16_t*)g.C + (long)m * g.ldc + n) = make_uint2(d0, d1);
            *(uint2*)((bf16_t*)g.C2 + (long)m * g.ldc2 + n) = make_uint2(a0, a1);
          } else if constexpr (EPI == EPI_BF16_RESID) {
            const uint2 pu = rpre[it];
            *(uint2*)((bf16_t*)g.C + (long)m * g.ldc + n) =
                make_uint2(pack_bf2(bf_lo(pu.x) + v[0], bf_hi(pu.x) + v[1]), pack_bf2(bf_lo(pu.y) + v[2], bf_hi(pu.y) + v[3]));
          } else {
            const uint2 pu = rpre[it];
            *(uint2*)((bf16_t*)g.C + (long)m * g.ldc + n) =
                make_uint2(pack_bf2(v[0] * bf_lo(pu.x), v[1] * bf_hi(pu.x)), pack_bf2(v[2] * bf_lo(pu.y), v[3] * bf_hi(pu.y)));
          }
        }
        __builtin_amdgcn_s_waitcnt(0xc07f);
      }
      __syncthreads();
      if (has_next) {
        const Tile nxt = make_tile(wgn);
        if (nxt.nk > 1) load_tile8(nxt, 1, sle, lane);
      }
    }

#if VJ_GEMM_STAMPS
    {
      if constexpr (!STG) asm volatile("s_waitcnt vmcnt(0)" ::: "memory");
      const long st2 = __builtin_amdgcn_s_memtime();
      if (threadIdx.x == 0 && blockIdx.x < 2048 && stamp_it < 16) {
        long* d = vj_gemm_stamps + ((long)blockIdx.x * 16 + stamp_it) * 4;
        d[0] = st0; d[1] = st1; d[2] = st2; d[3] = st_k1;
      }
      ++stamp_it;
    }
#endif
    if constexpr (STG) {
      if (wr == 1 || !has_next) __builtin_amdgcn_s_barrier();
    }
    if (!has_next) break;
    wg = wgn;
    cur = make_tile(wgn);
    par = parn;
  }
}

int num_cus() {
  static int cus[64];
  int dev = 0;
  if (hipGetDevice(&dev) != hipSuccess || dev < 0 || dev >= 64) dev = 0;
  if (cus[dev] <= 0) {
    int v = 0;
    if (hipDeviceGetAttribute(&v, hipDeviceAttributeMultiprocessorCount, dev) != hipSuccess || v <= 0) v = 256;
    cus[dev] = v;
  }
  return cus[dev];
}

struct Knobs {
  int stg, stg64, bm192, w2, w2_192;
  int group;
  int pxcd;
};
Knobs read_knobs() {
  auto sw = [](const char* name) {
    const char* e = getenv(name);
    return e && (e[0] == '0' || e[0] == '1') ? e[0] - '0' : -1;
  };
  const char* grp = getenv("VJ_GEMM_GROUP");
  const char* px = getenv("VJ_GEMM_PXCD");
  return Knobs{sw("VJ_GEMM_STG"),   sw("VJ_GEMM_STG64"), sw("VJ_GEMM_BM192"),
               sw("VJ_GEMM_2W"),    sw("VJ_GEMM_2W192"), grp ? (atoi(grp) > 0 ? atoi(grp) : 0) : -1,
               px && atoi(px) > 0 ? atoi(px) : 0};
}

std::atomic<int> g_reserved_cus{0};

int grid256(long nb, int per_cu, const Knobs& kn) {
  int per_xcd = per_cu * (num_cus() - g_reserved_cus.load(std::memory_order_relaxed)) / 8;
  if (kn.pxcd > 0) per_xcd = kn.pxcd;
  if (per_xcd < 1) per_xcd = 1;
  const long need = (nb + 7) / 8;
  return 8 * (int)(need < per_xcd ? need : per_xcd);
}

int tile_group(const Knobs& kn) { return kn.group >= 0 ? kn.group : 4; }

bool wide_tile_ok(int N) { return N % 256 == 0 || (N > 256 && vj_cdiv(N, 256) * 256L * 100 <= 115L * N); }

struct Plan256 {
  bool ok;
  int bm, bn, waves, stg, per_cu, group;
};

Plan256 plan256(int M, int N, int K, bool a_kmajor, bool b_kmajor, int epi, int cus, const Knobs& kn) {
  if (epi < EPI_BF16 || (epi > EPI_ROPE && epi != EPI_BF16_RESID) || N % 8) return Plan256{false};
  Plan256 p{true, 256, wide_tile_ok(N) ? 256 : 128, 8, 0, 1, tile_group(kn)};
  if (!a_kmajor || !b_kmajor) return p;
  if (kn.w2 >= 0 ? kn.w2 : p.bn == 128) {
    p.bn = 128;
    p.waves = 4;
    p.per_cu = 2;
    if (kn.w2_192 != 0 && epi != EPI_ROPE) p.bm = 192;
    return p;
  }
  if (p.bn == 128) return p;
  if (K % 32 == 0 && kn.stg != 0) {
    const bool aux = epi == EPI_F32_RESID || epi == EPI_BF16_RESID || epi == EPI_GELU_BWD;
    p.stg = (kn.stg64 == 0 || K % 64) ? 1 : 2;
    if (aux && p.stg == 1 && kn.stg != 1) p.stg = 0;
  }
  if (p.stg == 2 && kn.bm192 != 1) return p;
  const long tn = vj_cdiv(N, 256);
  const long r256 = (vj_cdiv(M, 256) * tn + cus - 1) / cus, r192 = (vj_cdiv(M, 192) * tn + cus - 1) / cus;
  if (kn.bm192 >= 0 ? kn.bm192 : r192 * 192 * 108 < r256 * 256 * 85) {
    p.bm = 192;
    p.stg = 0;
  }
  return p;
}

template <int... E>
struct EpiList {};
using Epilogues = EpiList<EPI_BF16, EPI_F32, EPI_F32_RESID, EPI_GELU, EPI_GELU_BWD, EPI_ROPE, EPI_PARTIAL, EPI_BF16_RESID,
                          EPI_PARTIAL_RS>;

template <bool AK, bool BKM, int EPI, int BN, bool F8, int NWV, int BMT, int STG>
int launch_epi256(const G256& g, hipStream_t st, const Knobs& kn) {
  using Cfg = Cfg256<AK, BKM, EPI, BN, F8, NWV, BMT, STG>;
  if constexpr (Cfg::supported) {
    const dim3 grid(grid256((long)g.tiles_m * g.tiles_n * g.nsplit, Cfg::BLOCKS_PER_CU, kn));
    hipLaunchKernelGGL((k_gemm256<AK, BKM, EPI, BN, F8, NWV, BMT, STG>), grid, dim3(Cfg::THREADS), 0, st, g);
    VJ_LAUNCH_CHECK("vj_gemm256");
    return VJ_OK;
  } else {
    return VJ_ERR_UNSUPPORTED;
  }
}

template <bool AK, bool BKM, int BN, bool F8, int NWV, int BMT, int STG, int... E>
int launch_list256(int epi, const G256& g, hipStream_t st, const Knobs& kn, EpiList<E...>) {
  int rc = -1;
  (void)((epi == E && ((rc = launch_epi256<AK, BKM, E, BN, F8, NWV, BMT, STG>(g, st, kn)), true)) || ...);
  if (rc >= 0) return rc;
  vj_set_error("vj_gemm256: bad epilogue %d", epi);
  return VJ_ERR_ARG;
}
template <bool AK, bool BKM, int BN, bool F8 = false, int NWV = 8, int BMT = 256, int STG = 0>
int launch256(int epi, const G256& g, hipStream_t st, const Knobs& kn) {
  return launch_list256<AK, BKM, BN, F8, NWV, BMT, STG>(epi, g, st, kn, Epilogues{});
}

int launch_plan(const Plan256& p, bool ak, bool bkm, int epi, G256& g, hipStream_t st, const Knobs& kn) {
  g.tiles_m = vj_cdiv(g.M, p.bm);
  g.tiles_n = vj_cdiv(g.N, p.bn);
  g.group = p.group;
  if (p.waves == 4)
    return p.bm == 192 ? launch256<true, true, 128, false, 4, 192>(epi, g, st, kn)
                       : launch256<true, true, 128, false, 4, 256>(epi, g, st, kn);
  if (p.bm == 192) return launch256<true, true, 256, false, 8, 192>(epi, g, st, kn);
  if (p.stg == 2) return launch256<true, true, 256, false, 8, 256, 2>(epi, g, st, kn);
  if (p.stg == 1) return launch256<true, true, 256, false, 8, 256, 1>(epi, g, st, kn);
  if (p.bn == 256) {
    if (ak) return bkm ? launch256<true, true, 256>(epi, g, st, kn) : launch256<true, false, 256>(epi, g, st, kn);
    return bkm ? launch256<false, true, 256>(epi, g, st, kn) : launch256<false, false, 256>(epi, g, st, kn);
  }
  if (ak) return bkm ? launch256<true, true, 128>(epi, g, st, kn) : launch256<true, false, 128>(epi, g, st, kn);
  return bkm ? launch256<false, true, 128>(epi, g, st, kn) : launch256<false, false, 128>(epi, g, st, kn);
}

}

extern "C" int vj_set_reserved_cus(int n) {
  VJ_CHECK_ARG(n >= 0 && n <= num_cus() - 8, "vj_set_reserved_cus: %d of %d CUs", n, num_cus());
  g_reserved_cus.store(n, std::memory_order_relaxed);
  return VJ_OK;
}

extern "C" int vj_gemm256_plan(int M, int N, int K, int a_kmajor, int b_kmajor, int epi, int cus, int* out6) {
  VJ_CHECK_ARG(M > 0 && N > 0 && K > 0 && cus >= 0 && out6, "vj_gemm256_plan: bad arguments");
  const Plan256 p = plan256(M, N, K, a_kmajor, b_kmajor, epi, cus ? cus : num_cus(), read_knobs());
  if (!p.ok) return VJ_ERR_UNSUPPORTED;
  const int v[6] = {p.bm, p.bn, p.waves, p.stg, p.per_cu, p.group};
  memcpy(out6, v, sizeof(v));
  return VJ_OK;
}

int vj_gemm256_dispatch(int M, int N, int K, const void* A, long lda, int a_kmajor, const void* B, long ldb,
                        int b_kmajor, int epi, const float* bias, const void* aux, long ldaux, void* C, long ldc,
                        void* C2, long ldc2, hipStream_t st, const void* rope) {
  if (ldc % 4 || ldc2 % 4 || ldaux % 4) return VJ_ERR_UNSUPPORTED;
  if (((uintptr_t)C & 15) || ((uintptr_t)C2 & 15) || ((uintptr_t)aux & 15) || ((uintptr_t)bias & 15))
    return VJ_ERR_UNSUPPORTED;
  const Knobs kn = read_knobs();
  const Plan256 p = plan256(M, N, K, a_kmajor, b_kmajor, epi, num_cus(), kn);
  if (!p.ok) return VJ_ERR_UNSUPPORTED;
  G256 g{(const bf16_t*)A, (const bf16_t*)B, M, N, K, lda, ldb, C, ldc, C2, ldc2, bias, aux, ldaux,
         0, 0, RopeP{}, K, 1, nullptr, 0};
  if (epi == EPI_ROPE) {
    if (!rope) return VJ_ERR_UNSUPPORTED;
    g.rope = *(const RopeP*)rope;
    if (g.rope.hd % 4 || g.rope.D % 4 || g.rope.npos < 1 || g.rope.npos > 1024) return VJ_ERR_UNSUPPORTED;
    if ((long)g.rope.npos * g.rope.half > ROPE_TAB_MAX) return VJ_ERR_UNSUPPORTED;
  }
  return launch_plan(p, a_kmajor, b_kmajor, epi, g, st, kn);
}

int vj_gemm256_partial(int M, int N, int K, const void* A, long lda, int a_kmajor, const void* B, long ldb,
                       int b_kmajor, int kslice, int splitk, float* ws, hipStream_t st, float* rsum) {
  if (a_kmajor || b_kmajor || N % 8 || M < 256 || N < 128) return VJ_ERR_UNSUPPORTED;
  const Knobs kn = read_knobs();
  const Plan256 p{true, 256, wide_tile_ok(N) ? 256 : 128, 8, 0, 1, tile_group(kn)};
  if ((long)vj_cdiv(M, p.bm) * vj_cdiv(N, p.bn) * splitk > 0x7fffffffL) return VJ_ERR_UNSUPPORTED;
  G256 g{(const bf16_t*)A, (const bf16_t*)B, M, N, K, lda, ldb, nullptr, 0, nullptr, 0, nullptr, nullptr, 0,
         0, 0, RopeP{}, kslice, splitk, ws, 0};
  g.rsum = rsum;
  return launch_plan(p, false, false, rsum ? EPI_PARTIAL_RS : EPI_PARTIAL, g, st, kn);
}

extern "C" int vj_gemm_bf16(int M, int N, int K, const void* A, long lda, int a_kmajor, const void* B, long ldb,
                            int b_kmajor, int epi, const float* bias, const void* aux, long ldaux, void* C, long ldc,
                            void* C2, long ldc2, void* stream);

extern "C" int vj_rope(int T, int H, int hd, void* qkv, long ld, int q_off, int k_off, const int* ids, int ids_mod,
                       int tokens_per_frame, int tokens_per_row, const float* cos_tab, const float* sin_tab, int half,
                       int inverse, void* stream);

extern "C" int vj_qkv_rope_gemm(int M, int K, const void* A, long lda, const void* B, long ldb, const float* bias,
                                void* C, long ldc, int H, int hd, const int* ids, int ids_mod, int tpf, int tpr,
                                const float* cos_t, const float* sin_t, int npos, void* stream) {
  if (M == 0) return VJ_OK;
  const int N = 3 * H * hd;
  VJ_CHECK_ARG(hd % 8 == 0 && cos_t && sin_t && (ids || ids_mod > 0), "vj_qkv_rope_gemm: bad rope arguments");
  VJ_CHECK_ARG(tpf > 0 && tpr > 0 && npos > 0, "vj_qkv_rope_gemm: tokens_per_frame/row and npos must be > 0");
  const int half = (hd / 3) / 2;
  if (M >= 1024) {
    RopeP rp{ids, ids_mod, tpf, tpr, half, hd, H * hd, cos_t, sin_t, npos};
    const int rc = vj_gemm256_dispatch(M, N, K, A, lda, 1, B, ldb, 1, EPI_ROPE, bias, nullptr, 0, C, ldc, nullptr, 0,
                                       (hipStream_t)stream, &rp);
    if (rc != VJ_ERR_UNSUPPORTED) return rc;
  }
  int rc = vj_gemm_bf16(M, N, K, A, lda, 1, B, ldb, 1, EPI_BF16, bias, nullptr, 0, C, ldc, nullptr, 0, stream);
  if (rc) return rc;
  return vj_rope(M, H, hd, C, ldc, 0, H * hd, ids, ids_mod, tpf, tpr, cos_t, sin_t, half, 0, stream);
}

static int gemm256_f8(int M, int N, int K, const void* A, long lda, const int* ea, const void* B, long ldb,
                      const int* eb, int epi, const float* bias, const void* aux, long ldaux, void* C, long ldc,
                      void* C2, long ldc2, hipStream_t st, const RopeP* rope) {
  if (M == 0 || N == 0) return VJ_OK;
  VJ_CHECK_ARG(M > 0 && N > 0 && K > 0 && K % 16 == 0 && lda % 16 == 0 && ldb % 16 == 0 && lda >= K && ldb >= K,
               "vj_gemm_fp8: K, lda, ldb must be multiples of 16 (M=%d N=%d K=%d lda=%ld ldb=%ld)", M, N, K, lda, ldb);
  VJ_CHECK_ARG(N % 8 == 0 && ldc % 4 == 0 && ldc2 % 4 == 0 && ldaux % 4 == 0, "vj_gemm_fp8: N %% 8, ld %% 4");
  VJ_CHECK_ARG(!(((uintptr_t)A | (uintptr_t)B | (uintptr_t)C | (uintptr_t)C2 | (uintptr_t)aux | (uintptr_t)bias) & 15),
               "vj_gemm_fp8: operands must be 16-B aligned");
  VJ_CHECK_ARG(A && B && ea && eb, "vj_gemm_fp8: null operand or scale exponents");
  VJ_CHECK_ARG(epi == EPI_BF16 || epi == EPI_F32 || epi == EPI_F32_RESID || epi == EPI_GELU || epi == EPI_ROPE,
               "vj_gemm_fp8: epilogue %d unsupported (forward only)", epi);
  VJ_CHECK_ARG(epi != EPI_F32_RESID || aux, "vj_gemm_fp8: EPI_F32_RESID needs the residual");
  VJ_CHECK_ARG(epi != EPI_GELU || C2, "vj_gemm_fp8: EPI_GELU needs the activation output C2");
  VJ_CHECK_ARG(epi == EPI_GELU || C, "vj_gemm_fp8: output C is required");
  VJ_CHECK_ARG((long)M * lda < 0x7fffffffL && (long)N * ldb < 0x7fffffffL, "vj_gemm_fp8: operand too large");
  const Knobs kn = read_knobs();
  G256 g{(const bf16_t*)A, (const bf16_t*)B, M, N, K / 2, lda / 2, ldb / 2, C, ldc, C2, ldc2, bias, aux, ldaux,
         vj_cdiv(M, 256), vj_cdiv(N, 128), RopeP{}, K / 2, 1, nullptr, tile_group(kn), ea, eb};
  if (epi == EPI_ROPE) {
    VJ_CHECK_ARG(rope != nullptr, "vj_gemm_fp8: EPI_ROPE needs the rope tables");
    g.rope = *rope;
    VJ_CHECK_ARG(g.rope.hd % 4 == 0 && g.rope.D % 4 == 0 && g.rope.npos >= 1 && g.rope.npos <= 1024 &&
                     (long)g.rope.npos * g.rope.half <= ROPE_TAB_MAX,
                 "vj_gemm_fp8: rope table too large (npos=%d)", g.rope.npos);
  }
  return launch256<true, true, 128, true>(epi, g, st, kn);
}

extern "C" int vj_gemm_fp8(int M, int N, int K, const void* A, long lda, const int* ea, const void* B, long ldb,
                           const int* eb, int epi, const float* bias, const void* aux, long ldaux, void* C, long ldc,
                           void* C2, long ldc2, void* stream) {
  VJ_CHECK_ARG(epi != EPI_ROPE, "vj_gemm_fp8: use vj_qkv_rope_gemm_fp8 for the RoPE epilogue");
  return gemm256_f8(M, N, K, A, lda, ea, B, ldb, eb, epi, bias, aux, ldaux, C, ldc, C2, ldc2, (hipStream_t)stream,
                    nullptr);
}

extern "C" int vj_qkv_rope_gemm_fp8(int M, int K, const void* A, long lda, const int* ea, const void* B, long ldb,
                                    const int* eb, const float* bias, void* C, long ldc, int H, int hd,
                                    const int* ids, int ids_mod, int tpf, int tpr, const float* cos_t,
                                    const float* sin_t, int npos, void* stream) {
  if (M == 0) return VJ_OK;
  VJ_CHECK_ARG(hd % 8 == 0 && cos_t && sin_t && (ids || ids_mod > 0), "vj_qkv_rope_gemm_fp8: bad rope arguments");
  VJ_CHECK_ARG(tpf > 0 && tpr > 0 && npos > 0, "vj_qkv_rope_gemm_fp8: tokens_per_frame/row and npos must be > 0");
  const RopeP rp{ids, ids_mod, tpf, tpr, (hd / 3) / 2, hd, H * hd, cos_t, sin_t, npos};
  return gemm256_f8(M, 3 * H * hd, K, A, lda, ea, B, ldb, eb, EPI_ROPE, bias, nullptr, 0, C, ldc, nullptr, 0,
                    (hipStream_t)stream, &rp);
}

#if VJ_GEMM_STAMPS
extern "C" int vj_debug_gemm_stamps(void* dst, long nbytes) {
  hipMemset(dst, 0, 0);
  return hipMemcpyFromSymbol(dst, HIP_SYMBOL(vj_gemm_stamps), nbytes, 0, hipMemcpyDeviceToHost) == hipSuccess ? 0 : 1;
}
extern "C" int vj_debug_gemm_istamps(void* dst, long nbytes) {
  return hipMemcpyFromSymbol(dst, HIP_SYMBOL(vj_gemm_istamps), nbytes, 0, hipMemcpyDeviceToHost) == hipSuccess ? 0 : 1;
}
extern "C" int vj_debug_gemm_stamps_clear() {
  static long z[2048 * 16 * 4];
  return hipMemcpyToSymbol(HIP_SYMBOL(vj_gemm_stamps), z, sizeof(z), 0, hipMemcpyHostToDevice) == hipSuccess ? 0 : 1;
}
#endif
```

vjepa2_amd/csrc/vj_gemm_tile.h:

```cpp
#pragma once
#include "vj_common.h"

namespace {


using RopeP = VjRope;

struct G256 {
  const bf16_t* A;
  const bf16_t* B;
  int M, N, K;
  long lda, ldb;
  void* C;
  long ldc;
  void* C2;
  long ldc2;
  const float* bias;
  const void* aux;
  long ldaux;
  int tiles_m, tiles_n;
  RopeP rope;
  int kslice;
  int nsplit;
  float* ws;
  int group;
  const int* ea = nullptr;
  const int* eb = nullptr;
  float* rsum = nullptr;
};

constexpr int BK = 64;
constexpr int TAB_BYTES = 16384;
constexpr int ROPE_TAB_MAX = (TAB_BYTES - 256 * 4) / 8;

__device__ __forceinline__ uint32_t clampb(long b) {
  if (b < 0) return 0;
  return b > 0x7fffffffL ? 0x7fffffffu : (uint32_t)b;
}

__device__ __forceinline__ int mn_swz(int k) { return 2 * (k & 3) + 8 * ((k >> 3) & 1); }

__device__ __forceinline__ int kswz32(int r) { return 3 * ((r >> 3) & 1); }

template <bool KMAJ, int ROWS, bool PERM = false, int NW = 8, int BKT = 64, int WNX = 4, int PB = 16>
__device__ __forceinline__ void stage(__amdgpu_buffer_rsrc_t rs, long ld, int rows_left, int k0, int K,
                                      LDS_AS char* lds, int wave, int lane) {
  constexpr int PIECES = ROWS * BKT * 2 / 1024;
  constexpr int PPW = PIECES / NW;
  static_assert(KMAJ || BKT == 64, "MN-major staging is written for 64-deep K tiles");
#pragma unroll
  for (int i = 0; i < PPW; ++i) {
    const int p = wave * PPW + i;
    uint32_t voff;
    if constexpr (KMAJ) {
      constexpr int CPR = BKT / 8, RPP = 64 / CPR;
      const int r = p * RPP + lane / CPR;
      const int c = (lane % CPR) ^ (BKT == 64 ? ((r >> 1) & 7) : kswz32(r));
      const int kk = k0 + c * 8;
      int gr = r;
      if constexpr (PERM) {
        constexpr int WN = ROWS / WNX, NTN = WN / PB;
        const int rl = r % WN;
        gr = (r - rl) + NTN * (rl % PB) + (rl / PB);
      }
      voff = (gr < rows_left && kk < K) ? (uint32_t)(((long)gr * ld + kk) * 2) : VJ_OOB;
    } else {
      constexpr int CPR = ROWS / 8;
      constexpr int RPP = 64 / CPR;
      const int kr = p * RPP + lane / CPR;
      const int c = (lane % CPR) ^ mn_swz(kr);
      const int col = c * 8;
      voff = (k0 + kr < K && col < rows_left) ? (uint32_t)(((long)(k0 + kr) * ld + col) * 2) : VJ_OOB;
    }
    dma16(rs, lds + p * 1024, voff);
  }
}

template <bool KMAJ, int ROWS, int BKT = 64>
__device__ __forceinline__ bf16x8 frag(const LDS_AS char* lds, int rb, int s, int lane) {
  if constexpr (KMAJ) {
    const int r = rb + (lane & 15);
    if constexpr (BKT == 32) {
      const int c = (lane >> 4) ^ kswz32(r);
      return *(const LDS_AS bf16x8*)(lds + r * 64 + c * 16);
    }
    const int c = (4 * s + (lane >> 4)) ^ ((r >> 1) & 7);
    return *(const LDS_AS bf16x8*)(lds + r * 128 + c * 16);
  } else {
    const int gi = lane & 15;
    const int k0 = 32 * s + 8 * (lane >> 4) + (gi >> 2);
    const int col = rb + 4 * (gi & 3);
    const int within = (col & 7) * 2;
    const int c = col >> 3;
    const s16x4 lo = ds_read_tr16_async(lds + k0 * (ROWS * 2) + ((c ^ mn_swz(k0)) * 16) + within);
    const s16x4 hi = ds_read_tr16_async(lds + (k0 + 4) * (ROWS * 2) + ((c ^ mn_swz(k0 + 4)) * 16) + within);
    s16x8 v = {lo[0], lo[1], lo[2], lo[3], hi[0], hi[1], hi[2], hi[3]};
    return __builtin_bit_cast(bf16x8, v);
  }
}

__device__ __forceinline__ uint32_t gelu_pair(uint32_t pk, uint32_t* dpk) {
  float y0, d0, y1, d1;
  gelu_fwd_grad(__builtin_bit_cast(float, pk << 16), y0, d0);
  gelu_fwd_grad(__builtin_bit_cast(float, pk & 0xffff0000u), y1, d1);
  if (dpk) *dpk = pack_bf2(d0, d1);
  return pack_bf2(y0, y1);
}

constexpr uint32_t GT_LO = 0x3A80;
constexpr uint32_t GT_HI = 0x417F;
constexpr int GT_N = GT_HI - GT_LO + 2;
constexpr int GT_BYTES = 2 * GT_N * 8;

__device__ __forceinline__ void gelu_tab_fill(LDS_AS f32x2* tab, int tid, int nthreads) {
  for (int e = tid; e < 2 * GT_N; e += nthreads) {
    const uint32_t i = (uint32_t)e >> 1, sg = (uint32_t)e & 1;
    const uint32_t bits = (i == 0 ? 0u : GT_LO - 1 + i) | (sg << 15);
    float cdf, dy;
    gelu_cdf_grad(__builtin_bit_cast(float, bits << 16), cdf, dy);
    tab[e] = f32x2{cdf, dy};
  }
}

template <bool SAVE_D>
__device__ __forceinline__ uint32_t gelu_pair_tab(uint32_t pk, const LDS_AS char* tab, uint32_t* dpk) {
  typedef unsigned short u16x2 __attribute__((ext_vector_type(2)));
  const u16x2 b = __builtin_bit_cast(u16x2, pk);
  u16x2 i = __builtin_elementwise_sub_sat(b & (u16x2)0x7fff, (u16x2)(GT_LO - 1));
  i = __builtin_elementwise_min(i, (u16x2)(GT_N - 1));
  const uint32_t a = __builtin_bit_cast(uint32_t, (u16x2)((i << 4) | ((b >> 12) & (u16x2)8)));
  const float x0 = __builtin_bit_cast(float, pk << 16), x1 = __builtin_bit_cast(float, pk & 0xffff0000u);
  if constexpr (SAVE_D) {
    const f32x2 t0 = *(const LDS_AS f32x2*)(tab + (a & 0xffffu));
    const f32x2 t1 = *(const LDS_AS f32x2*)(tab + (a >> 16));
    *dpk = pack_bf2(fmaf(x0, 0.f, t0[1]), fmaf(x1, 0.f, t1[1]));
    return pack_bf2(x0 * t0[0], x1 * t1[0]);
  } else {
    const float c0 = *(const LDS_AS float*)(tab + (a & 0xffffu));
    const float c1 = *(const LDS_AS float*)(tab + (a >> 16));
    return pack_bf2(x0 * c0, x1 * c1);
  }
}

struct Tile {
  int m0, n0, z, Keff, nk;
};

__device__ __forceinline__ float bf_lo(uint32_t u) { return __builtin_bit_cast(float, u << 16); }
__device__ __forceinline__ float bf_hi(uint32_t u) { return __builtin_bit_cast(float, u & 0xffff0000u); }
__device__ __forceinline__ float bf_lo(float u) { return __builtin_bit_cast(float, __builtin_bit_cast(uint32_t, u) << 16); }
__device__ __forceinline__ float bf_hi(float u) {
  return __builtin_bit_cast(float, __builtin_bit_cast(uint32_t, u) & 0xffff0000u);
}

constexpr int SPLIT_AT = 3;
constexpr int DMA_WAVES = 4;
constexpr int AUX_PF = 1;

constexpr int LDS_PER_CU = 163840;
constexpr int cmax(int a, int b) { return a > b ? a : b; }

template <bool AK, bool BKM, int EPI, int BN, bool F8, int NWV, int BMT, int STG>
struct Cfg256 {
  static constexpr bool PART = EPI == EPI_PARTIAL || EPI == EPI_PARTIAL_RS;
  static constexpr bool RS = EPI == EPI_PARTIAL_RS;
  static constexpr int BM = BMT;
  static constexpr int MH = BM / 64;
  static constexpr int BK = (NWV == 8 || BMT == 192) ? 64 : 32;
  static constexpr int NT = NWV * 64;
  static constexpr int WNX = NWV / 2;
  static constexpr int WMX = NWV / WNX;
  static constexpr int WM = BM / WMX;
  static constexpr int WN = BN / WNX;
  static constexpr int PB = 16;
  static constexpr int NTN = WN / PB;
  static constexpr int A_BYTES = BM * BK * 2;
  static constexpr int B_BYTES = BN * BK * 2;
  static constexpr int STAGE = A_BYTES + B_BYTES;
  static constexpr bool VALU_EPI = EPI == EPI_ROPE || EPI == EPI_GELU || EPI == EPI_GELU_BWD;
  static constexpr int DMAW = NWV != 8 ? NWV : (VALU_EPI || BN != 256 || F8) ? 8 : DMA_WAVES;
  static constexpr bool DIRECT = BKM && NTN == 4;
  static constexpr bool AUX = EPI == EPI_F32_RESID || EPI == EPI_GELU_BWD || EPI == EPI_BF16_RESID;
  static constexpr bool F32OUT = EPI == EPI_F32 || EPI == EPI_F32_RESID || PART;
  static constexpr bool ASYNC = !AK || !BKM;
  static constexpr bool EARLY1 = DIRECT && !AUX;

  static constexpr bool supported =
      (!STG || (AK && BKM && !F8 && NWV == 8 && BMT == 256 && BN == 256 && !PART)) &&
      (!F8 || (AK && BKM && (EPI == EPI_BF16 || EPI == EPI_F32 || EPI == EPI_F32_RESID || EPI == EPI_GELU ||
                             EPI == EPI_ROPE))) &&
      (NWV == 8 || (NWV == 4 && AK && BKM && !F8)) &&
      (BMT == 256 || (BMT == 192 && !F8 && AK && DIRECT && (NWV == 8 || EPI != EPI_ROPE))) &&
      (EPI != EPI_BF16_RESID || (AK && BKM)) && (!PART || (!AK && !BKM));

  static constexpr bool GTAB = STG && EPI == EPI_GELU;
  static constexpr int USZ = 32768;
  static constexpr int NSL = STG ? ((EPI == EPI_ROPE || GTAB) ? 4 : 5) : 1;
  static constexpr int DIST = NSL - 2;
  static constexpr bool S64 = STG == 2;
  static constexpr int GSZ = 16384;
  static constexpr int SA = 4, SB = 4;
  static constexpr int EA = SA - 1, EB = SB - 1;
  static constexpr int WRS = S64 ? 64 : WM;

  static constexpr int STR = WN + 4;
  static constexpr int LPR = WN / 4;
  static constexpr int RPI = 64 / LPR;
  static constexpr int MTP = (NWV * 32 * STR * 4 <= STAGE) ? 2 : 1;
  static constexpr int PR = 16 * MTP;
  static constexpr int IT = PR / RPI;

  static constexpr int SLOT_OFF = 0, SLOT_END = STG ? 0 : 2 * STAGE;
  static constexpr int GTAB_OFF = 0, GTAB_END = GTAB ? GT_BYTES : 0;
  static constexpr int RING0 = GTAB ? 32768 : 0, RING_END = STG ? RING0 + NSL * USZ : 0;
  static constexpr int S64_END = S64 ? RING0 + (SA + SB) * GSZ : 0;
  static constexpr int TABB = (STG ? EPI != EPI_ROPE : (NWV == 4 && BMT == 192)) ? 0 : TAB_BYTES;
  static constexpr int TAB_OFF = 2 * STAGE, TAB_END = TABB ? TAB_OFF + TABB : 0;
  static constexpr int RPOS_OFF = TAB_OFF, RTAB_OFF = RPOS_OFF + BM * 4;
  static constexpr int RTAB_END = EPI == EPI_ROPE ? RTAB_OFF + ROPE_TAB_MAX * 8 : 0;
  static constexpr int IMG_END = DIRECT ? 0 : STAGE + NWV * PR * STR * 4;
  static constexpr int LDS_BYTES = cmax(cmax(SLOT_END, RING_END), TAB_END);
  static constexpr int THREADS = NT;
  static constexpr int BLOCKS_PER_CU = NWV == 4 ? 2 : 1;
  static constexpr bool lds_disjoint = GTAB_END <= RING0 && (TABB == 0 || cmax(SLOT_END, RING_END) <= TAB_OFF) &&
                                       (EPI != EPI_ROPE || RTAB_END <= TAB_END);
};

}
```

vjepa2_amd/functions.py:

```python

import os
import weakref

import torch

from . import ops
from .ops import BF16, EPI_BF16, EPI_BF16_RESID, EPI_F32, EPI_F32_RESID, EPI_GELU, F32



def weight_bf16(p):
    v = getattr(p, "_vj_bf16", None)
    if v is not None:
        return v
    key = (p.data_ptr(), p._version)
    c = getattr(p, "_vj_bf16_cache", None)
    if c is None or c[0] != key:
        c = (key, ops.cast_bf16(p.detach().contiguous()))
        p._vj_bf16_cache = c
    return c[1]


SHADOW_EPOCH = [0]


def weight_bf16_t(p):
    src = weight_bf16(p)
    arena_owned = getattr(p, "_vj_bf16", None) is not None
    key = (src.data_ptr(), SHADOW_EPOCH[0] if arena_owned else p._version)
    c = getattr(p, "_vj_bf16_t", None)
    if c is None or c[0] != key:
        out = c[1] if c is not None and c[1].shape == (src.shape[1], src.shape[0]) else None
        c = (key, ops.transpose_bf16(src.reshape(src.shape[0], -1), out=out))
        p._vj_bf16_t = c
        if arena_owned:
            _WT_REG[id(p)] = p
    return c[1]


_WT_REG = weakref.WeakValueDictionary()
_WT_BATCH = [None]


def refresh_weight_transposes():
    stale = [p for p in _WT_REG.values() if p._vj_bf16_t[0][1] != SHADOW_EPOCH[0]]
    if not stale:
        return
    pairs = []
    for p in stale:
        src = weight_bf16(p)
        pairs.append((src.reshape(src.shape[0], -1), p._vj_bf16_t[1]))
    key = tuple((s.data_ptr(), d.data_ptr()) for s, d in pairs)
    if _WT_BATCH[0] is None or _WT_BATCH[0][0] != key:
        desc, tiles = ops.transpose_batch_desc(pairs)
        _WT_BATCH[0] = (key, desc, tiles)
    ops.transpose_bf16_batch(_WT_BATCH[0][1], len(pairs), _WT_BATCH[0][2])
    for p, (s, _) in zip(stale, pairs):
        p._vj_bf16_t = ((s.data_ptr(), SHADOW_EPOCH[0]), p._vj_bf16_t[1])


def weight_fp8(p):
    arena_owned = getattr(p, "_vj_bf16", None) is not None
    key = (p.data_ptr(), SHADOW_EPOCH[0] if arena_owned else p._version)
    c = getattr(p, "_vj_fp8", None)
    if c is None or c[0] != key:
        w = p.detach().reshape(p.shape[0], -1)
        if not w.is_contiguous():
            w = w.contiguous()
        out = c[1] if c is not None else (None, None)
        c = (key, ops.quant_rows_fp8(w, out=out[0], exps=out[1]))
        p._vj_fp8 = c
    return c[1]


def grad_buf(p):
    if p.grad is None:
        p.grad = torch.zeros_like(p)
    a = getattr(p, "_vj_arena", None)
    if a is not None and p._vj_gepoch != a.epoch:
        p.grad.zero_()
        p._vj_gepoch = a.epoch
    return p.grad


def wgrad_buf(p):
    a = getattr(p, "_vj_arena", None)
    if a is None or p.grad is None:
        return grad_buf(p), True
    p._vj_ow = True
    if p._vj_gepoch != a.epoch:
        p._vj_gepoch = a.epoch
        return p.grad, False
    return p.grad, True


def wgrad(dy, x, w, shape=None, lin=None):
    buf, acc = wgrad_buf(w)
    db = _bias_buf(lin) if lin is not None else None
    ops.linear_wgrad(dy, x, buf if shape is None else buf.view(*shape), accumulate=acc, db=db)


_ROPE_TABLES = {}


def rope_tables(hd, device, npos):
    key = (hd, str(device), npos)
    t = _ROPE_TABLES.get(key)
    if t is None:
        sw = 2 * ((hd // 3) // 2)
        omega = torch.arange(sw // 2, dtype=torch.float32)
        omega /= sw / 2.0
        omega = 1.0 / 10000**omega
        freq = torch.arange(npos, dtype=torch.float32)[:, None] * omega[None, :]
        t = (freq.cos().contiguous().to(device), freq.sin().contiguous().to(device))
        if t[0].is_cuda:
            torch.cuda.current_stream().synchronize()
        _ROPE_TABLES[key] = t
    return t


class TokenLayout:

    def __init__(self, groups, ids=None, ids_mod=0, tpf=1, tpr=1, fblk=0):
        self.fblk = int(fblk)
        self.groups = [(int(n), int(l)) for n, l in groups if n > 0]
        self.T = sum(n * l for n, l in self.groups)
        self.ids, self.ids_mod, self.tpf, self.tpr = ids, int(ids_mod), int(tpf), int(tpr)
        self.npos = max(-(-self.ids_mod // self.tpf), -(-self.tpf // self.tpr), self.tpr, 1)




def _attn_scale(attn, hd, lay=None):
    if attn.use_sdpa or (lay is not None and lay.fblk > 0):
        return hd**-0.5
    return attn.scale


def _resid_epi(x):
    return EPI_BF16_RESID if x.dtype == BF16 else EPI_F32_RESID


def block_forward_fp8(x, blk, lay):
    attn, mlp = blk.attn, blk.mlp
    if getattr(mlp, "swiglu", False) or _drop_scales(blk, lay, x.device) is not None or _has_dropout(blk):
        raise NotImplementedError("the fp8 block path covers the GELU MLP without drop_path / dropout")
    H = attn.num_heads
    hd = x.shape[1] // H
    ln1, e1 = ops.layernorm_fwd_fp8(x, blk.norm1.weight, blk.norm1.bias, blk.norm1.eps)
    w8, ew = weight_fp8(attn.qkv.weight)
    if attn.use_rope:
        c, s = rope_tables(hd, x.device, lay.npos)
        qkv = ops.qkv_rope_fp8(ln1, e1, w8, ew, attn.qkv.bias, H, hd, lay.ids, lay.ids_mod, lay.tpf, lay.tpr, c, s)
    else:
        qkv = ops.linear_fwd_fp8(ln1, e1, w8, ew, attn.qkv.bias, EPI_BF16)
    o, _ = ops.attn_fwd(qkv, H, hd, lay.groups, _attn_scale(attn, hd, lay), fblk=lay.fblk)
    x_mid = ops.linear_fwd(o, weight_bf16(attn.proj.weight), attn.proj.bias, _resid_epi(x), resid=x)
    ln2, e2 = ops.layernorm_fwd_fp8(x_mid, blk.norm2.weight, blk.norm2.bias, blk.norm2.eps)
    w18, ew1 = weight_fp8(mlp.fc1.weight)
    _, act = ops.linear_fwd_fp8(ln2, e2, w18, ew1, mlp.fc1.bias, EPI_GELU)
    return ops.linear_fwd(act, weight_bf16(mlp.fc2.weight), mlp.fc2.bias, _resid_epi(x), resid=x_mid)


def _drop_scales(blk, lay, device):
    dp = blk.drop_path
    if not getattr(dp, "drop_prob", None) or not dp.training:
        return None
    lens = getattr(lay, "_vj_seq_lens", None)
    if lens is None or lens.device != torch.device(device):
        lens = lay._vj_seq_lens = torch.tensor([ln for n, ln in lay.groups for _ in range(n)], device=device)
    return tuple(dp.sample(lens.numel(), device).repeat_interleave(lens, output_size=lay.T) for _ in range(2))


class DropCfg:

    def __init__(self, attn=None, mlp=None):
        self.pa, self.pp = _attn_drop_probs(attn) if attn is not None else (0.0, 0.0)
        self.pm = _mlp_drop_prob(mlp) if mlp is not None else 0.0
        self.sa, self.sp, self.sm1, self.sm2 = (_drop_seed() if p > 0 else 0 for p in (self.pa, self.pp, self.pm,
                                                                                        self.pm))

    @property
    def branches(self):
        return self.pp > 0 or self.pm > 0


def _attn_drop_probs(attn):
    if getattr(attn, "use_sdpa", True):
        pa = float(getattr(attn, "proj_drop_prob", 0.0) or 0.0)
    else:
        pa = float(attn.attn_drop.p) if attn.attn_drop.training else 0.0
    pp = float(attn.proj_drop.p) if attn.proj_drop.training else 0.0
    return pa, pp


def _mlp_drop_prob(mlp):
    drop = None if getattr(mlp, "swiglu", False) else getattr(mlp, "drop", None)
    return float(drop.p) if drop is not None and drop.training else 0.0


def _has_dropout(blk):
    return any(_attn_drop_probs(blk.attn)) or _mlp_drop_prob(blk.mlp) > 0


def _drop_seed():
    return int(torch.randint(0, 2**32, (1,), dtype=torch.int64))


def _drop_cfg(blk):
    return DropCfg(blk.attn, blk.mlp) if _has_dropout(blk) else None


def _branch_out(inp, lin, resid, scale, p=0.0, seed=0):
    if scale is None and p == 0:
        return ops.linear_fwd(inp, weight_bf16(lin.weight), lin.bias, _resid_epi(resid), resid=resid)
    y = ops.linear_fwd(inp, weight_bf16(lin.weight), lin.bias, EPI_F32)
    if p == 0:
        return ops.rowscale_add(y, scale, resid)
    if scale is None:
        return ops.dropout(y, p, seed, resid=resid)
    return ops.rowscale_add(ops.dropout(y, p, seed).float(), scale, resid)


def _branch_grad(dxo, scale, p, seed):
    g = ops.rowscale_bf16(dxo, scale) if scale is not None else dxo
    if p > 0:
        return ops.dropout(g, p, seed)
    return g if g.dtype == BF16 else ops.cast_bf16(g)


def _mlp_forward(ln2, mlp, save, p=0.0, seed=0):
    T = ln2.shape[0]
    if getattr(mlp, "swiglu", False):
        h = mlp.fc1.weight.shape[0]
        x12 = torch.empty(T, 2 * h, dtype=BF16, device=ln2.device)
        ops.linear_fwd(ln2, weight_bf16(mlp.fc1.weight), mlp.fc1.bias, EPI_BF16, out=x12[:, :h])
        ops.linear_fwd(ln2, weight_bf16(mlp.fc2.weight), mlp.fc2.bias, EPI_BF16, out=x12[:, h:])
        hidden = ops.swiglu_fwd(x12)
        return hidden, mlp.fc3, ((x12, hidden) if save else None)
    dgelu = torch.empty(T, mlp.fc1.weight.shape[0], dtype=BF16, device=ln2.device) if save else None
    _, act = ops.linear_fwd(ln2, weight_bf16(mlp.fc1.weight), mlp.fc1.bias, EPI_GELU, out=dgelu)
    if p > 0:
        act = ops.dropout(act, p, seed)
    return act, mlp.fc2, ((dgelu, act) if save else None)


def block_forward(x, blk, lay, save):
    T, D = x.shape
    attn, mlp = blk.attn, blk.mlp
    H = attn.num_heads
    hd = D // H
    scales = _drop_scales(blk, lay, x.device)
# ... 34 lines not shown
    x_mid = ops.linear_fwd_f32(o, attn.proj.weight.detach().float(), attn.proj.bias, EPI_F32_RESID, resid=x)
    ln2, _, _ = ops.layernorm_fwd(x_mid, blk.norm2.weight, blk.norm2.bias, blk.norm2.eps, out_dtype=F32,
                                  want_stats=False)
    _, act = ops.linear_fwd_f32(ln2, mlp.fc1.weight.detach().float(), mlp.fc1.bias, EPI_GELU)
    return ops.linear_fwd_f32(act, mlp.fc2.weight.detach().float(), mlp.fc2.bias, EPI_F32_RESID, resid=x_mid)


def patch_embed_forward_f32(clip, pe, masks, pos_table=None, pos_ids=None, pos_mod=0):
    proj = pe.proj
    D = proj.weight.shape[0]
    p, tub = pe.patch_size, pe.tubelet_size
    cols = ops.im2col_f32(clip, p, tub) if masks is None else torch.cat(
        [ops.im2col_f32(clip, p, tub, idx=m.contiguous()) for m in masks], 0)
    x = ops.linear_fwd_f32(cols, proj.weight.detach().float().reshape(D, -1).contiguous(), proj.bias, EPI_F32)
    if pos_table is not None:
        ops.add_rows(x, pos_table, idx=pos_ids, idx_mod=pos_mod)
    return x



_WG_STREAMS = {}


def wgrad_stream():
    if os.environ.get("VJ_WGRAD_STREAM", "1") != "1" or not torch.cuda.is_available():
        return None
    dev = torch.cuda.current_device()
    s = _WG_STREAMS.get(dev)
    if s is None:
        s = _WG_STREAMS[dev] = torch.cuda.Stream(device=dev)
    return s


def join_wgrad_stream():
    s = _WG_STREAMS.get(torch.cuda.current_device()) if torch.cuda.is_available() else None
    if s is not None:
        torch.cuda.current_stream().wait_stream(s)


_WG_JOIN_TASK = [None]


class JoinQueue(list):
    """Work to issue on the weight-gradient stream right after its next join with the current stream
    (distributed.GradReducer: a bucket's all-reduce also needs the LayerNorm / bias gradients written on
    the current stream; riding on the join every block's weight gradients take anyway saves a join of
    its own per bucket). One queue per owner, so two armed reducers in one process (a trainer and an
    eval probe, two frames-per-clip groups) never issue each other's collectives; at a join the queues
    are drained in the order their owners were created, which is the same host program order on every
    rank, whatever the interleaving of the owners' backward hooks."""


_JOIN_QUEUES = []


def join_queue():
    q = JoinQueue()
    _JOIN_QUEUES.append(weakref.ref(q))
    return q


def _drain_join_queues():
    live = []
    for r in _JOIN_QUEUES:
        q = r()
        if q is None:
            continue
        live.append(r)
        while q:
            q.pop(0)()
    _JOIN_QUEUES[:] = live


def drain_join_queue(q):
    if not q:
        return
    side = wgrad_stream()
    if side is None:
        while q:
            q.pop(0)()
        return
    side.wait_stream(torch.cuda.current_stream())
    with torch.cuda.stream(side):
        while q:
            q.pop(0)()


def _join_at_backward_end():
    _WG_JOIN_TASK[0] = None
    join_wgrad_stream()


class _OnWgradStream:

    def __init__(self, *tensors):
        self.tensors = tensors
        self.side = wgrad_stream()
        self.ctx = None

    def __enter__(self):
        if self.side is None:
            return self
        self.side.wait_stream(torch.cuda.current_stream())
        for t in self.tensors:
            t.record_stream(self.side)
        task = torch._C._current_graph_task_id()
        self.join_on_exit = task == -1
        if task != -1 and _WG_JOIN_TASK[0] != task:
            torch.autograd.Variable._execution_engine.queue_callback(_join_at_backward_end)
            _WG_JOIN_TASK[0] = task
        self.ctx = torch.cuda.stream(self.side)
        self.ctx.__enter__()
        _drain_join_queues()
        return self

    def __exit__(self, *exc):
        if self.ctx is not None:
            self.ctx.__exit__(*exc)
            if self.join_on_exit:
                join_wgrad_stream()
        return False


def _bias_buf(lin):
    return grad_buf(lin.bias) if lin.bias is not None and lin.bias.requires_grad else None


def _bias_grad(lin, dy):
    if lin.bias is not None and lin.bias.requires_grad:
        ops.colsum(dy, grad_buf(lin.bias))


def _ln_grads(ln):
    if ln.weight is None:
        return None, None
    return grad_buf(ln.weight), grad_buf(ln.bias)


def _mlp_backward(dy_b, mlp, ln2, saved, p=0.0, seed=0):
    if getattr(mlp, "swiglu", False):
        x12, hidden = saved
        h = hidden.shape[1]
        with _OnWgradStream(dy_b, hidden):
            wgrad(dy_b, hidden, mlp.fc3.weight)
        dh = ops.linear_dgrad(dy_b, weight_bf16(mlp.fc3.weight), wt=weight_bf16_t(mlp.fc3.weight))
        dx12 = ops.swiglu_bwd(dh, x12)
        dx1, dx2 = dx12[:, :h], dx12[:, h:]
        with _OnWgradStream(dx12, ln2):
            wgrad(dx1, ln2, mlp.fc1.weight, lin=mlp.fc1)
            wgrad(dx2, ln2, mlp.fc2.weight, lin=mlp.fc2)
        dl = ops.linear_dgrad(dx1, weight_bf16(mlp.fc1.weight), wt=weight_bf16_t(mlp.fc1.weight))
        return ops.linear_dgrad(dx2, weight_bf16(mlp.fc2.weight), wt=weight_bf16_t(mlp.fc2.weight), resid=dl)
    dgelu, act = saved
    with _OnWgradStream(dy_b, act):
        wgrad(dy_b, act, mlp.fc2.weight)
    if p > 0:
        dh = ops.linear_dgrad(dy_b, weight_bf16(mlp.fc2.weight), wt=weight_bf16_t(mlp.fc2.weight))
        dpre = ops.dropout(dh, p, seed, aux=dgelu)
    else:
        dpre = ops.linear_dgrad(dy_b, weight_bf16(mlp.fc2.weight), gelu_grad=dgelu, wt=weight_bf16_t(mlp.fc2.weight))
    with _OnWgradStream(dpre, ln2):
        wgrad(dpre, ln2, mlp.fc1.weight, lin=mlp.fc1)
    return ops.linear_dgrad(dpre, weight_bf16(mlp.fc1.weight), wt=weight_bf16_t(mlp.fc1.weight))


def block_backward(dxo, blk, lay, saved):
    x, ln1, m1, r1, qkv, o, stats, x_mid, ln2, m2, r2, msaved, scales, dc = saved
    branch_drop = dc is not None and dc.branches
    attn, mlp = blk.attn, blk.mlp
    out_lin = mlp.fc3 if getattr(mlp, "swiglu", False) else mlp.fc2
    T, D = x.shape
    H = attn.num_heads
    hd = D // H
    if branch_drop:
        dy_mlp = _branch_grad(dxo, scales and scales[1], dc.pm, dc.sm2)
        _bias_grad(out_lin, dy_mlp)
    elif dxo.dtype == BF16:
        dy_mlp = dxo
    elif scales is None:
        twin = getattr(dxo, "_vj_grad_bf16", None)
        dy_mlp = twin[0] if twin is not None and twin[1] == dxo._version else ops.cast_bf16(dxo)
    else:
        dy_mlp = ops.rowscale_bf16(dxo, scales[1])
        _bias_grad(out_lin, dy_mlp)
    dln2 = _mlp_backward(dy_mlp, mlp, ln2, msaved, *((dc.pm, dc.sm1) if dc else ()))
    gw, gb = _ln_grads(blk.norm2)
    fused = scales is None and not branch_drop
    dxm, dxm_b = ops.layernorm_bwd(dln2, x_mid, m2, r2, blk.norm2.weight, dres_in=dxo, dweight=gw, dbias=gb,
                                   want_bf16=fused, sum_in=_bias_buf(out_lin) if fused else None,
                                   sum_out=_bias_buf(attn.proj) if fused else None)
    if not fused:
        dxm_b = _branch_grad(dxm, scales and scales[0], dc.pp if dc else 0.0, dc.sp if dc else 0)
        _bias_grad(attn.proj, dxm_b)
    with _OnWgradStream(dxm_b, o):
        wgrad(dxm_b, o, attn.proj.weight)
    do = ops.linear_dgrad(dxm_b, weight_bf16(attn.proj.weight), wt=weight_bf16_t(attn.proj.weight))
    rope = None
    if attn.use_rope:
        c, s = rope_tables(hd, x.device, lay.npos)
        rope = (lay.ids, lay.ids_mod, lay.tpf, lay.tpr, c, s)
    dqkv = ops.attn_bwd(qkv, o, do, stats, H, hd, lay.groups, _attn_scale(attn, hd, lay), rope=rope, fblk=lay.fblk,
                        dropout_p=dc.pa if dc else 0.0, seed=dc.sa if dc else 0)
    with _OnWgradStream(dqkv, ln1):
        wgrad(dqkv, ln1, attn.qkv.weight, lin=attn.qkv)
    dln1 = ops.linear_dgrad(dqkv, weight_bf16(attn.qkv.weight), wt=weight_bf16_t(attn.qkv.weight))
    gw, gb = _ln_grads(blk.norm1)
    dxi, dxi_b = ops.layernorm_bwd(dln1, x, m1, r1, blk.norm1.weight, dres_in=dxm, dweight=gw, dbias=gb,
                                   want_bf16=True)
    if dxi.dtype == F32:
        dxi._vj_grad_bf16 = (dxi_b, dxi._version)
    return dxi


def _fire_hook(mod):
    hook = getattr(mod, "_vj_grad_ready", None)
    if hook is not None:
        hook(mod)


class _BlockFn(torch.autograd.Function):
    @staticmethod
    def forward(ctx, x, anchor, blk, lay):
        y, saved = block_forward(x, blk, lay, save=True)
        ctx.blk, ctx.lay, ctx.saved = blk, lay, saved
        return y

    @staticmethod
    def backward(ctx, dy):
        dx = block_backward(dy.contiguous(), ctx.blk, ctx.lay, ctx.saved)
        ctx.saved = None
        _fire_hook(ctx.blk)
        return dx, None, None, None


def _needs_grad(x, mod):
    return torch.is_grad_enabled() and (
        (x is not None and x.requires_grad) or any(p.requires_grad for p in mod.parameters()))


def run_block(x, blk, lay, fp8=False):
    if _needs_grad(x, blk):
        if fp8:
            raise NotImplementedError("the fp8 block path is forward-only (the no-grad target encoder)")
        return _BlockFn.apply(x, blk.norm1.weight, blk, lay)
    if fp8:
        return block_forward_fp8(x, blk, lay)
    return block_forward(x, blk, lay, save=False)[0]




def attn_module_forward(x, attn, lay):
    H = attn.num_heads
    hd = x.shape[1] // H
    if attn.use_rope:
        c, s = rope_tables(hd, x.device, lay.npos)
        qkv = ops.qkv_rope(x, weight_bf16(attn.qkv.weight), attn.qkv.bias, H, hd, lay.ids, lay.ids_mod, lay.tpf,
                           lay.tpr, c, s)
    else:
        qkv = ops.linear_fwd(x, weight_bf16(attn.qkv.weight), attn.qkv.bias, EPI_BF16)
    dc = DropCfg(attn=attn) if any(_attn_drop_probs(attn)) else None
    o, stats = ops.attn_fwd(qkv, H, hd, lay.groups, _attn_scale(attn, hd, lay), fblk=lay.fblk,
                            dropout_p=dc.pa if dc else 0.0, seed=dc.sa if dc else 0)
    y = ops.linear_fwd(o, weight_bf16(attn.proj.weight), attn.proj.bias, EPI_F32)
    if dc is not None and dc.pp > 0:
        y = ops.dropout(y, dc.pp, dc.sp).float()
    return y, (x, qkv, o, stats, dc)


def attn_module_backward(dy, attn, lay, saved):
    x, qkv, o, stats, dc = saved
    H = attn.num_heads
    hd = x.shape[1] // H
    if dc is not None and dc.pp > 0:
        dy = ops.dropout(dy, dc.pp, dc.sp).float()
    dy_b = ops.cast_bf16(dy)
    do = ops.linear_dgrad(dy_b, weight_bf16(attn.proj.weight), wt=weight_bf16_t(attn.proj.weight))
    wgrad(dy_b, o, attn.proj.weight)
    _bias_grad(attn.proj, dy)
    rope = None
    if attn.use_rope:
        c, s = rope_tables(hd, x.device, lay.npos)
        rope = (lay.ids, lay.ids_mod, lay.tpf, lay.tpr, c, s)
    dqkv = ops.attn_bwd(qkv, o, do, stats, H, hd, lay.groups, _attn_scale(attn, hd, lay), rope=rope, fblk=lay.fblk,
                        dropout_p=dc.pa if dc else 0.0, seed=dc.sa if dc else 0)
    dx = ops.linear_dgrad(dqkv, weight_bf16(attn.qkv.weight), wt=weight_bf16_t(attn.qkv.weight))
    wgrad(dqkv, x, attn.qkv.weight, lin=attn.qkv)
    return dx


def mlp_module_forward(x, mlp):
    dc = DropCfg(mlp=mlp) if _mlp_drop_prob(mlp) > 0 else None
    hidden, out_lin, msaved = _mlp_forward(x, mlp, True, *((dc.pm, dc.sm1) if dc else ()))
    y = ops.linear_fwd(hidden, weight_bf16(out_lin.weight), out_lin.bias, EPI_F32)
    if dc is not None:
        y = ops.dropout(y, dc.pm, dc.sm2).float()
    return y, (x, msaved, dc)


def mlp_module_backward(dy, mlp, saved):
    x, msaved, dc = saved
    if dc is not None:
        dy = ops.dropout(dy, dc.pm, dc.sm2).float()
    dx = _mlp_backward(ops.cast_bf16(dy), mlp, x, msaved, *((dc.pm, dc.sm1) if dc else ()))
    _bias_grad(mlp.fc3 if getattr(mlp, "swiglu", False) else mlp.fc2, dy)
    return dx


class _SubLayerFn(torch.autograd.Function):

    @staticmethod
    def forward(ctx, x, anchor, mod, lay):
        xb = ops.cast_bf16(x.contiguous()) if x.dtype != BF16 else x.contiguous()
        if lay is None:
            y, saved = mlp_module_forward(xb, mod)
        else:
            y, saved = attn_module_forward(xb, mod, lay)
        ctx.mod, ctx.lay, ctx.saved, ctx.in_dtype = mod, lay, saved, x.dtype
        return y

    @staticmethod
    def backward(ctx, dy):
        dy = dy.contiguous().float()
        if ctx.lay is None:
            dx = mlp_module_backward(dy, ctx.mod, ctx.saved)
        else:
            dx = attn_module_backward(dy, ctx.mod, ctx.lay, ctx.saved)
        ctx.saved = None
        _fire_hook(ctx.mod)
        return dx.to(ctx.in_dtype), None, None, None


def run_sublayer(x, mod, lay=None):
    if _needs_grad(x, mod):
        return _SubLayerFn.apply(x, next(mod.parameters()), mod, lay)
    xb = ops.cast_bf16(x.contiguous()) if x.dtype != BF16 else x.contiguous()
    return (mlp_module_forward(xb, mod) if lay is None else attn_module_forward(xb, mod, lay))[0]




def patch_embed_forward(clip, pe, masks, pos_table=None, pos_ids=None, pos_mod=0, save=False, out_bf16=False):
    proj = pe.proj
    D = proj.weight.shape[0]
    kdim = proj.weight[0].numel()
    p, tub = pe.patch_size, pe.tubelet_size
    if masks is None:
        cols = ops.im2col(clip, p, tub)
    else:
        B = clip.shape[0]
        R = sum(B * m.shape[1] for m in masks)
        cols = torch.empty(R, kdim, dtype=BF16, device=clip.device)
        r0 = 0
        for m in masks:
            n = B * m.shape[1]
            ops.im2col(clip, p, tub, idx=m.contiguous(), out=cols[r0:r0 + n])
            r0 += n
    assert not (out_bf16 and pos_table is not None), "bf16 tokens: no pos-embed add (RoPE models)"
    x = ops.linear_fwd(cols, weight_bf16(proj.weight).view(D, kdim), proj.bias, EPI_BF16 if out_bf16 else EPI_F32)
    if pos_table is not None:
        ops.add_rows(x, pos_table, idx=pos_ids, idx_mod=pos_mod)
    return x, (cols if save else None)


class _PatchEmbedFn(torch.autograd.Function):
    @staticmethod
    def forward(ctx, clip, anchor, pe, masks, pos_table, pos_ids, pos_mod, out_bf16):
        x, cols = patch_embed_forward(clip, pe, masks, pos_table, pos_ids, pos_mod, save=True, out_bf16=out_bf16)
        ctx.pe, ctx.cols = pe, cols
        return x

    @staticmethod
    def backward(ctx, dx):
        proj = ctx.pe.proj
        D = proj.weight.shape[0]
        dx = dx.contiguous()
        wgrad(dx if dx.dtype == BF16 else ops.cast_bf16(dx), ctx.cols, proj.weight, (D, -1))
        _bias_grad(proj, dx)
        ctx.cols = None
        _fire_hook(ctx.pe)
        return None, None, None, None, None, None, None, None


def run_patch_embed(clip, pe, masks, pos_table=None, pos_ids=None, pos_mod=0, out_bf16=False):
    if _needs_grad(None, pe):
        return _PatchEmbedFn.apply(clip, pe.proj.weight, pe, masks, pos_table, pos_ids, pos_mod, out_bf16)
    return patch_embed_forward(clip, pe, masks, pos_table, pos_ids, pos_mod, out_bf16=out_bf16)[0]




class _LayerNormFn(torch.autograd.Function):
    @staticmethod
    def forward(ctx, x, anchor, ln, out_dtype):
        y, m, r = ops.layernorm_fwd(x, ln.weight, ln.bias, ln.eps, out_dtype=out_dtype)
        ctx.ln, ctx.x, ctx.m, ctx.r = ln, x, m, r
        return y

    @staticmethod
    def backward(ctx, dy):
        dy = dy.contiguous()
        dy_b = dy if dy.dtype == BF16 else ops.cast_bf16(dy)
        gw, gb = _ln_grads(ctx.ln)
        dx, _ = ops.layernorm_bwd(dy_b, ctx.x, ctx.m, ctx.r, ctx.ln.weight, dweight=gw, dbias=gb)
        ctx.x = ctx.m = ctx.r = None
        _fire_hook(ctx.ln)
        return dx, None, None, None


def run_layernorm(x, ln, out_dtype=F32):
    if _needs_grad(x, ln):
        return _LayerNormFn.apply(x, ln.weight, ln, out_dtype)
    return ops.layernorm_fwd(x, ln.weight, ln.bias, ln.eps, out_dtype=out_dtype, want_stats=False)[0]




class _LinearFn(torch.autograd.Function):
    @staticmethod
    def forward(ctx, x, anchor, lin, out_dtype):
        xb = x.contiguous() if x.dtype == BF16 else ops.cast_bf16(x.contiguous())
        y = ops.linear_fwd(xb, weight_bf16(lin.weight), lin.bias, EPI_BF16 if out_dtype == BF16 else EPI_F32)
        ctx.lin, ctx.x, ctx.in_dtype = lin, xb, x.dtype
        return y

    @staticmethod
    def backward(ctx, dy):
        dy = dy.contiguous()
        dy_b = dy if dy.dtype == BF16 else ops.cast_bf16(dy)
        lin = ctx.lin
        w = lin.weight
        wt = weight_bf16_t(w) if w.shape[0] % 8 == 0 and w.shape[1] % 8 == 0 else None
        dx = ops.linear_dgrad(dy_b, weight_bf16(lin.weight), wt=wt)
        wgrad(dy_b, ctx.x, lin.weight)
        _bias_grad(lin, dy)
        ctx.x = None
        _fire_hook(lin)
        return dx.to(ctx.in_dtype), None, None, None


# ... 76 lines not shown
```

vjepa2_amd/ops.py:

```python

import ctypes
import os

import torch

from ._lib import call, int_array

EPI_BF16, EPI_F32, EPI_F32_RESID, EPI_GELU, EPI_GELU_BWD = 0, 1, 2, 3, 4
EPI_ROPE, EPI_PARTIAL = 5, 6
EPI_BF16_RESID = 7
EPI_NAMES = ["EPI_BF16", "EPI_F32", "EPI_F32_RESID", "EPI_GELU", "EPI_GELU_BWD", "EPI_ROPE", "EPI_PARTIAL", "EPI_BF16_RESID"]
BF16 = torch.bfloat16
F32 = torch.float32


_SHAPE_LABELS = bool(int(__import__("os").environ.get("VJ_SHAPE_LABELS", "0")))
_WGRAD_BIAS = os.environ.get("VJ_WGRAD_BIAS", "1") != "0"


class KernelEvents:

    active = None

    def __init__(self, only=None):
        self.rec = []
        self.only = only

    def start(self):
        KernelEvents.active = self

    def stop(self):
        KernelEvents.active = None
        torch.cuda.synchronize()

    def summary(self):
        out = {}
        for name, flops, s, e in self.rec:
            d = out.setdefault(name, dict(count=0, total_ms=0.0, flops=0.0))
            d["count"] += 1
            d["total_ms"] += s.elapsed_time(e)
            d["flops"] += flops
        return out


def _call(fn, *args, label=None, flops=0):
    prof = KernelEvents.active
    if prof is None or (prof.only is not None and (label or fn) not in prof.only):
        return call(fn, *args)
    s = torch.cuda.Event(enable_timing=True)
    e = torch.cuda.Event(enable_timing=True)
    s.record()
    rc = call(fn, *args)
    e.record()
    prof.rec.append((label or fn, flops, s, e))
    return rc


def _stream():
    return torch.cuda.current_stream().cuda_stream


def _p(t):
    return None if t is None else t.data_ptr()


def _dev(*ts):
    for t in ts:
        if t is not None and not t.is_cuda:
            raise RuntimeError("vjepa2_amd ops require device (HIP) tensors; there is no CPU path")


def _rowmajor(t, name):
    if t.dim() != 2 or t.stride(1) != 1:
        raise ValueError(f"{name}: expected a 2-D row-major tensor (stride(1)==1), got {tuple(t.shape)} {t.stride()}")
    return t.stride(0)


def gemm(M, N, K, a, lda, a_kmajor, b, ldb, b_kmajor, epi, out=None, ldc=0, out2=None, ldc2=0, bias=None, aux=None,
         ldaux=0, splitk=1):
    _dev(a, b, out, out2, bias, aux)
    if a.dtype != BF16 or b.dtype != BF16:
        raise TypeError("gemm operands must be bf16")
    if bias is not None and (bias.dtype != F32 or bias.numel() < N):
        raise TypeError("gemm bias must be f32 [N]")
    label = f"k_gemm<{int(a_kmajor)},{int(b_kmajor)},{EPI_NAMES[epi]}>"
    if _SHAPE_LABELS:
        label += f"[{M}x{N}x{K}]"
    splitk = _effective_splitk(K, splitk)
    if splitk > 1:
        ws = torch.empty(splitk * M * N, dtype=F32, device=a.device)
        _call("vj_gemm_bf16_splitk", M, N, K, _p(a), lda, int(a_kmajor), _p(b), ldb, int(b_kmajor), epi, _p(bias),
              _p(aux), ldaux, _p(out), ldc, _p(out2), ldc2, splitk, _p(ws), ws.numel(), _stream(),
              label=label + "[splitk]", flops=2.0 * M * N * K)
        return
    _call("vj_gemm_bf16", M, N, K, _p(a), lda, int(a_kmajor), _p(b), ldb, int(b_kmajor), epi, _p(bias), _p(aux), ldaux,
          _p(out), ldc, _p(out2), ldc2, _stream(), label=label, flops=2.0 * M * N * K)


def _effective_splitk(K, splitk):
    if splitk <= 1:
        return 1
    kslice = (K + splitk - 1) // splitk
    kslice = (kslice + 63) // 64 * 64
    return (K + kslice - 1) // kslice


def wgrad_wide_tile(N):
    return N % 256 == 0 or (N > 256 and -(-N // 256) * 256 * 100 <= 115 * N)


def wgrad_splitk(M, N, K, cus=None):
    if cus is None:
        cus = 256
    if M >= 256 and N >= 128:
        tm, tn, per_cu = 256, (256 if wgrad_wide_tile(N) else 128), 1
    else:
        tm, tn, per_cu = 128, 128, 2
    tiles = -(-M // tm) * -(-N // tn)
    best, best_t = 1, None
    for s in range(1, max(1, K // 512) + 1):
        waves = -(-tiles * s // (cus * per_cu))
        t = waves * (K / s) * tm * tn * 2 / 3.9e12 + (s * M * N * 8 / 5.0e12 if s > 1 else 0.0)
        if best_t is None or t < best_t * 0.98:
            best, best_t = s, t
    return best


def linear_fwd(x, w, bias=None, epi=EPI_BF16, out=None, out2=None, resid=None):
    M, K = x.shape
    N = w.shape[0]
    assert w.shape[1] == K, (tuple(x.shape), tuple(w.shape))
    if K % 8:
        x, w = _pad_cols(x), _pad_cols(w)
        K = x.shape[1]
    lda = _rowmajor(x, "x")
    ldb = _rowmajor(w, "w")
    if epi == EPI_BF16:
        out = out if out is not None else torch.empty(M, N, dtype=BF16, device=x.device)
    elif epi in (EPI_F32, EPI_F32_RESID):
        out = out if out is not None else torch.empty(M, N, dtype=F32, device=x.device)
        if epi == EPI_F32_RESID:
            assert resid is not None and resid.dtype == F32 and resid.shape == (M, N)
    elif epi == EPI_GELU:
        out2 = out2 if out2 is not None else torch.empty(M, N, dtype=BF16, device=x.device)
    elif epi == EPI_BF16_RESID:
        assert resid is not None and resid.dtype == BF16 and resid.shape == (M, N)
        out = out if out is not None else torch.empty(M, N, dtype=BF16, device=x.device)
    ldc = out.stride(0) if out is not None else 0
    ldc2 = out2.stride(0) if out2 is not None else 0
    gemm(M, N, K, x, lda, True, w, ldb, True, epi, out=out, ldc=ldc, out2=out2, ldc2=ldc2, bias=bias,
         aux=resid, ldaux=resid.stride(0) if resid is not None else 0)
    return (out, out2) if epi == EPI_GELU else out


def linear_dgrad(dy, w, out=None, gelu_grad=None, wt=None, resid=None):
    if resid is not None:
        M, K = dy.shape[0], w.shape[1]
        assert gelu_grad is None and wt is not None and resid.dtype == BF16 and resid.shape == (M, K)
        assert dy.shape[1] % 8 == 0 and K % 8 == 0
        out = out if out is not None else torch.empty(M, K, dtype=BF16, device=dy.device)
        gemm(M, K, dy.shape[1], dy, _rowmajor(dy, "dy"), True, wt, _rowmajor(wt, "wt"), True, EPI_BF16_RESID, out=out,
             ldc=out.stride(0), aux=resid, ldaux=_rowmajor(resid, "resid"))
        return out
    M, N = dy.shape
    K = w.shape[1]
    assert w.shape[0] == N
    if N % 8:
        dy, w, wt = _pad_cols(dy), _pad_rows(w), None
        N = dy.shape[1]
    if K % 8:
        assert gelu_grad is None and out is None
        return linear_dgrad(dy, _pad_cols(w))[:, :K]
    out = out if out is not None else torch.empty(M, K, dtype=BF16, device=dy.device)
    epi = EPI_GELU_BWD if gelu_grad is not None else EPI_BF16
    aux = dict(aux=gelu_grad, ldaux=gelu_grad.stride(0) if gelu_grad is not None else 0)
    if wt is not None:
        assert wt.shape == (K, N), (tuple(wt.shape), (K, N))
        gemm(M, K, N, dy, _rowmajor(dy, "dy"), True, wt, _rowmajor(wt, "wt"), True, epi, out=out, ldc=out.stride(0),
             **aux)
    else:
        gemm(M, K, N, dy, _rowmajor(dy, "dy"), True, w, _rowmajor(w, "w"), False, epi, out=out, ldc=out.stride(0),
             **aux)
    return out


def transpose_bf16(x, out=None):
    _dev(x)
    assert x.dtype == BF16 and x.dim() == 2
    R, C = x.shape
    out = out if out is not None else torch.empty(C, R, dtype=BF16, device=x.device)
    _call("vj_transpose_bf16", R, C, _p(x), _rowmajor(x, "x"), _p(out), _rowmajor(out, "out"), _stream())
    return out


def transpose_batch_desc(pairs):
    rows, tiles = [], 0
    for src, dst in pairs:
        _dev(src, dst)
        R, C = src.shape
        assert src.dtype == BF16 and dst.dtype == BF16 and dst.shape == (C, R), (tuple(src.shape), tuple(dst.shape))
        lds, ldd = _rowmajor(src, "src"), _rowmajor(dst, "dst")
        if R % 8 or C % 8 or lds % 8 or ldd % 8 or (src.data_ptr() | dst.data_ptr()) & 15:
            raise ValueError("transpose_batch_desc: rows, cols, strides must be multiples of 8, pointers 16-B aligned")
        tx, ty = -(-C // 64), -(-R // 64)
        rows.append([src.data_ptr(), dst.data_ptr(), R, C, lds, ldd, tiles, tx])
        tiles += tx * ty
    return torch.tensor(rows, dtype=torch.int64).to(pairs[0][0].device), tiles


def transpose_bf16_batch(desc, n, tiles):
    _call("vj_transpose_bf16_batch", n, _p(desc), tiles, _stream())


def _pad_cols(t):
    out = torch.zeros(t.shape[0], (t.shape[1] + 7) // 8 * 8, dtype=t.dtype, device=t.device)
    out[:, :t.shape[1]] = t
    return out


def _pad_rows(t):
    out = torch.zeros((t.shape[0] + 7) // 8 * 8, t.shape[1], dtype=t.dtype, device=t.device)
    out[:t.shape[0]] = t
    return out


def linear_wgrad(dy, x, dw, accumulate=True, db=None):
    M, N = dy.shape
    K = x.shape[1]
    assert x.shape[0] == M and dw.shape == (N, K) and dw.dtype == F32
    if db is not None and (N % 8 or K % 8 or not _WGRAD_BIAS):
        linear_wgrad(dy, x, dw, accumulate)
        return colsum(dy, db)
    if db is not None:
        _dev(dy, x, dw, db)
        assert db.dtype == F32 and db.numel() == N and db.is_contiguous()
        s = wgrad_splitk(N, K, M)
        s = _effective_splitk(M, s)
        nws = max(s * (N * K + N) if s > 1 else 0, min(256, max(1, (M + 63) // 64)) * N)
        ws = torch.empty(nws, dtype=F32, device=dy.device)
        _call("vj_gemm_bf16_wgrad", N, K, M, _p(dy), _rowmajor(dy, "dy"), _p(x), _rowmajor(x, "x"), _p(dw),
              _rowmajor(dw, "dw"), int(accumulate), _p(db), 1, s, _p(ws), ws.numel(), _stream(),
              label="k_gemm<0,0,wgrad+bias>", flops=2.0 * M * N * K)
        return dw
    if N % 8:
        tmp = torch.zeros((N + 7) // 8 * 8, K, dtype=F32, device=dw.device)
        linear_wgrad(_pad_cols(dy), x, tmp)
        if accumulate:
            dw += tmp[:N]
        else:
            dw.copy_(tmp[:N])
        return dw
    if K % 8:
        tmp = torch.zeros(N, (K + 7) // 8 * 8, dtype=F32, device=dw.device)
        linear_wgrad(dy, _pad_cols(x), tmp)
        if accumulate:
            dw += tmp[:, :K]
        else:
            dw.copy_(tmp[:, :K])
        return dw
    if accumulate:
        gemm(N, K, M, dy, _rowmajor(dy, "dy"), False, x, _rowmajor(x, "x"), False, EPI_F32_RESID, out=dw,
             ldc=dw.stride(0), aux=dw, ldaux=dw.stride(0), splitk=wgrad_splitk(N, K, M))
    else:
        gemm(N, K, M, dy, _rowmajor(dy, "dy"), False, x, _rowmajor(x, "x"), False, EPI_F32, out=dw,
             ldc=dw.stride(0), splitk=wgrad_splitk(N, K, M))
    return dw


def swiglu_fwd(x12, out=None):
    _dev(x12, out)
    assert x12.dtype == BF16 and x12.shape[1] % 2 == 0
    M, h = x12.shape[0], x12.shape[1] // 2
    out = out if out is not None else torch.empty(M, h, dtype=BF16, device=x12.device)
    _call("vj_swiglu_fwd", M, h, _p(x12), _rowmajor(x12, "x12"), _p(out), _rowmajor(out, "out"), _stream())
    return out


def swiglu_bwd(dh, x12, out=None):
# ... 674 lines not shown
```

Measured before the change: 235.2 clips/s.

## Group split-K weight-gradient GEMMs of paired linears into one launch

Adds a grouped split-K wgrad GEMM that runs up to four weight-gradient problems sharing the token dimension (proj+qkv, fc2+fc1) in a single persistent kernel launch, followed by one grouped split-K reduction. The point is to fill the GPU's CUs better when each wgrad alone gives too few tiles, and to cut launch and tail overhead. A cost model picks the split factor and only groups when it predicts a win. The trade-off is per-tile problem selection inside the kernel, deferring the proj wgrad until after attention backward, and a larger workspace allocation.

```diff
diff --git a/include/vjepa_hip.h b/include/vjepa_hip.h
--- a/include/vjepa_hip.h
+++ b/include/vjepa_hip.h
@@ -31,6 +31,10 @@
 int vj_gemm_bf16_wgrad(int M, int N, int K, const void* dy, long lddy, const void* x, long ldx, float* dw, long lddw,
                        int accumulate, float* db, int db_accumulate, int splitk, float* ws, long ws_floats,
                        void* stream);
+int vj_gemm_bf16_wgrad_group(int nprob, const int* M, const int* N, int K, const void* const* dy, const long* lddy,
+                             const void* const* x, const long* ldx, float* const* dw, const long* lddw,
+                             const int* accumulate, float* const* db, const int* db_accumulate, int splitk,
+                             float* ws, long ws_floats, void* stream);
 
 int vj_attn_fwd(int T, int H, int hd, const void* qkv, long ld, int q_off, int k_off, int v_off, void* o, long ldo,
                 float* stats, float scale, int ngroups, const int* nseq, const int* len, void* stream);
diff --git a/vjepa2_amd/_lib.py b/vjepa2_amd/_lib.py
--- a/vjepa2_amd/_lib.py
+++ b/vjepa2_amd/_lib.py
@@ -21,6 +21,7 @@
     "vj_gemm_bf16": [_I, _I, _I, _P, _L, _I, _P, _L, _I, _I, _P, _P, _L, _P, _L, _P, _L, _P],
     "vj_gemm_bf16_splitk": [_I, _I, _I, _P, _L, _I, _P, _L, _I, _I, _P, _P, _L, _P, _L, _P, _L, _I, _P, _L, _P],
     "vj_gemm_bf16_wgrad": [_I, _I, _I, _P, _L, _P, _L, _P, _L, _I, _P, _I, _I, _P, _L, _P],
+    "vj_gemm_bf16_wgrad_group": [_I, _P, _P, _I, _P, _P, _P, _P, _P, _P, _P, _P, _P, _I, _P, _L, _P],
     "vj_attn_fwd": [_I, _I, _I, _P, _L, _I, _I, _I, _P, _L, _P, _F, _I, _P, _P, _P],
     "vj_attn_bwd": [_I, _I, _I, _P, _L, _I, _I, _I, _P, _L, _P, _L, _P, _P, _L, _F, _I, _P, _P, _P, _I, _I, _I, _P,
                     _P, _P],
diff --git a/vjepa2_amd/csrc/vj_common.h b/vjepa2_amd/csrc/vj_common.h
--- a/vjepa2_amd/csrc/vj_common.h
+++ b/vjepa2_amd/csrc/vj_common.h
@@ -142,6 +142,17 @@
 
 static inline int vj_cdiv(long a, long b) { return (int)((a + b - 1) / b); }
 
+constexpr int VJ_WGROUP_MAX = 4;
+struct VjWgradProb {
+  const void* dy;
+  long lddy;
+  const void* x;
+  long ldx;
+  int M, N;
+  float* ws;
+  float* rsum;
+};
+
 __device__ __forceinline__ void gelu_cdf_grad(float x, float& cdf, float& dy) {
   const float zs = x * 0.84932180028801904f;
   const float a = fabsf(zs);
diff --git a/vjepa2_amd/csrc/vj_gemm.hip b/vjepa2_amd/csrc/vj_gemm.hip
--- a/vjepa2_amd/csrc/vj_gemm.hip
+++ b/vjepa2_amd/csrc/vj_gemm.hip
@@ -211,6 +211,50 @@
     ((float*)g.C)[(long)m * g.ldc + n] = v;
   } else {
     ((bf16_t*)g.C)[(long)m * g.ldc + n] = f2bf(v);
+  }
+}
+
+struct ReduceProb {
+  const float* ws;
+  float* dw;
+  long lddw;
+  const float* rs_ws;
+  float* rs_out;
+  int M, N, acc, rs_acc;
+  unsigned blk0;
+};
+struct ReduceGroup {
+  ReduceProb pr[VJ_WGROUP_MAX];
+  int splitk;
+};
+
+__global__ void k_splitk_reduce4_group(ReduceGroup g) {
+  const unsigned b = blockIdx.x;
+  const int p = (b >= g.pr[1].blk0) + (b >= g.pr[2].blk0) + (b >= g.pr[3].blk0);
+  ReduceProb q = g.pr[0];
+  if (p == 1) q = g.pr[1];
+  if (p == 2) q = g.pr[2];
+  if (p == 3) q = g.pr[3];
+  const long i = ((long)(b - q.blk0) * blockDim.x + threadIdx.x) * 4;
+  const long total = (long)q.M * q.N;
+  if (i >= total) return;
+  const int m = (int)(i / q.N), n = (int)(i % q.N);
+  if (q.rs_out && n == 0) {
+    float s = 0.f;
+    for (int z = 0; z < g.splitk; ++z) s += q.rs_ws[(long)z * q.M + m];
+    q.rs_out[m] = q.rs_acc ? q.rs_out[m] + s : s;
+  }
+  float4 v = make_float4(0.f, 0.f, 0.f, 0.f);
+  for (int z = 0; z < g.splitk; ++z) {
+    const float4 w = *(const float4*)(q.ws + (long)z * total + i);
+    v.x += w.x; v.y += w.y; v.z += w.z; v.w += w.w;
+  }
+  float4* out = (float4*)(q.dw + (long)m * q.lddw + n);
+  if (q.acc) {
+    const float4 r = *out;
+    *out = make_float4(r.x + v.x, r.y + v.y, r.z + v.z, r.w + v.w);
+  } else {
+    *out = v;
   }
 }
 
@@ -336,6 +380,89 @@
   return vj_colsum_f32(K, M, dy, 1, lddy, db, db_accumulate, ws, ws_floats, stream);
 }
 
+int vj_gemm256_partial_group(int np, const VjWgradProb* pr, int K, int kslice, int splitk, hipStream_t st);
+
+extern "C" int vj_gemm_bf16_wgrad_group(int nprob, const int* M, const int* N, int K, const void* const* dy,
+                                        const long* lddy, const void* const* x, const long* ldx, float* const* dw,
+                                        const long* lddw, const int* accumulate, float* const* db,
+                                        const int* db_accumulate, int splitk, float* ws, long ws_floats,
+                                        void* stream) {
+  const char* fn = "vj_gemm_bf16_wgrad_group";
+  VJ_CHECK_ARG(nprob >= 1 && nprob <= VJ_WGROUP_MAX, "%s: %d problems (1 .. %d)", fn, nprob, VJ_WGROUP_MAX);
+  VJ_CHECK_ARG(M && N && dy && lddy && x && ldx && dw && lddw && accumulate, "%s: null argument array", fn);
+  VJ_CHECK_ARG(!db || db_accumulate, "%s: db without db_accumulate", fn);
+  VJ_CHECK_ARG(K > 0, "%s: bad token count K=%d", fn, K);
+  if (splitk < 1) splitk = 1;
+  int kslice = K;
+  if (splitk > 1) {
+    kslice = vj_cdiv(vj_cdiv(K, splitk), BK) * BK;
+    splitk = vj_cdiv(K, kslice);
+  }
+  long need = 0;
+  for (int p = 0; p < nprob; ++p) {
+    VJ_CHECK_ARG(M[p] > 0 && N[p] > 0, "%s: problem %d: bad dims M=%d N=%d", fn, p, M[p], N[p]);
+    VJ_CHECK_ARG(dy[p] && x[p] && dw[p], "%s: problem %d: null dy, x or dw", fn, p);
+    VJ_CHECK_ARG((((uintptr_t)dy[p] | (uintptr_t)x[p] | (uintptr_t)dw[p]) & 15) == 0,
+                 "%s: problem %d: dy, x and dw must be 16-B aligned", fn, p);
+    VJ_CHECK_ARG(M[p] % 8 == 0 && N[p] % 8 == 0, "%s: problem %d: M and N must be multiples of 8", fn, p);
+    VJ_CHECK_ARG(lddy[p] % 8 == 0 && ldx[p] % 8 == 0 && lddw[p] % 4 == 0,
+                 "%s: problem %d: row pitches must be multiples of 16 B (lddy=%ld ldx=%ld lddw=%ld)", fn, p, lddy[p],
+                 ldx[p], lddw[p]);
+    VJ_CHECK_ARG(lddy[p] >= M[p] && ldx[p] >= N[p] && lddw[p] >= N[p], "%s: problem %d: row pitch too small", fn, p);
+    VJ_CHECK_ARG((long)K * lddy[p] * 2 < 0x7fffffffL && (long)K * ldx[p] * 2 < 0x7fffffffL,
+                 "%s: problem %d: operand too large", fn, p);
+    const bool bias = db && db[p];
+    if (splitk > 1) {
+      VJ_CHECK_ARG(M[p] >= 256 && N[p] >= 128, "%s: problem %d: %d x %d is below the 256 x 128 split-K tile", fn, p,
+                   M[p], N[p]);
+      need += (long)splitk * ((long)M[p] * N[p] + M[p]);
+    } else if (bias) {
+      const long cs = (long)(vj_cdiv(K, 64) < 256 ? vj_cdiv(K, 64) : 256) * M[p];
+      need = need > cs ? need : cs;
+    }
+  }
+  VJ_CHECK_ARG(need == 0 || (ws && ((uintptr_t)ws & 15) == 0 && ws_floats >= need),
+               "%s: workspace needs %ld floats (16-B aligned), got %ld", fn, need, ws ? ws_floats : 0L);
+  hipStream_t st = (hipStream_t)stream;
+  if (splitk == 1) {
+    for (int p = 0; p < nprob; ++p) {
+      const int rc = vj_gemm_bf16_wgrad(M[p], N[p], K, dy[p], lddy[p], x[p], ldx[p], dw[p], lddw[p], accumulate[p],
+                                        db ? db[p] : nullptr, db ? db_accumulate[p] : 0, 1, ws, ws_floats, stream);
+      if (rc) return rc;
+    }
+    return VJ_OK;
+  }
+  VjWgradProb pr[VJ_WGROUP_MAX];
+  ReduceGroup rg{};
+  rg.splitk = splitk;
+  float* w = ws;
+  unsigned blk = 0;
+  for (int p = 0; p < VJ_WGROUP_MAX; ++p) {
+    ReduceProb& r = rg.pr[p];
+    if (p >= nprob) {
+      r.blk0 = 0xffffffffu;
+      continue;
+    }
+    const long mn = (long)M[p] * N[p];
+    float* rs = w + splitk * mn;
+    const bool bias = db && db[p];
+    pr[p] = VjWgradProb{dy[p], lddy[p], x[p], ldx[p], M[p], N[p], w, bias ? rs : nullptr};
+    r = ReduceProb{w, dw[p], lddw[p], rs, bias ? db[p] : nullptr, M[p], N[p], accumulate[p],
+                   bias ? db_accumulate[p] : 0, blk};
+    blk += (unsigned)((mn / 4 + 255) / 256);
+    w = rs + (long)splitk * M[p];
+  }
+  const int rc = vj_gemm256_partial_group(nprob, pr, K, kslice, splitk, st);
+  if (rc == VJ_ERR_UNSUPPORTED) {
+    vj_set_error("%s: the problems do not share one column-tile width (group only such problems)", fn);
+    return VJ_ERR_ARG;
+  }
+  if (rc) return rc;
+  hipLaunchKernelGGL(k_splitk_reduce4_group, dim3(blk), dim3(256), 0, st, rg);
+  VJ_LAUNCH_CHECK("vj_gemm_bf16_wgrad_group(reduce)");
+  return VJ_OK;
+}
+
 extern "C" int vj_gemm_bf16(int M, int N, int K, const void* A, long lda, int a_kmajor, const void* B, long ldb,
                             int b_kmajor, int epi, const float* bias, const void* aux, long ldaux, void* C, long ldc,
                             void* C2, long ldc2, void* stream) {
diff --git a/vjepa2_amd/csrc/vj_gemm256.hip b/vjepa2_amd/csrc/vj_gemm256.hip
--- a/vjepa2_amd/csrc/vj_gemm256.hip
+++ b/vjepa2_amd/csrc/vj_gemm256.hip
@@ -48,7 +48,7 @@
   const int wave = __builtin_amdgcn_readfirstlane(threadIdx.x >> 6);
   const int wr = wave / WNX, wc = wave % WNX;
 
-  const int ntile = g.tiles_m * g.tiles_n;
+  const int ntile = PART ? g.ntile_all : g.tiles_m * g.tiles_n;
   const int nb = ntile * g.nsplit;
   const int P = gridDim.x >> 3;
   const int xcd = blockIdx.x & 7, jb = blockIdx.x >> 3;
@@ -57,18 +57,47 @@
   const int runend = run0 + q + (xcd < rmd ? 1 : 0);
   if (run0 + jb >= runend) return;
 
+  [[maybe_unused]] auto pick = [&](int p, auto f) {
+    auto v = f(g.pr[0]);
+    if (p == 1) v = f(g.pr[1]);
+    if (p == 2) v = f(g.pr[2]);
+    if (p == 3) v = f(g.pr[3]);
+    return v;
+  };
   auto make_tile = [&](int wg) {
     Tile T;
-    const int z = wg / ntile, w = wg - z * ntile;
+    const int z = wg / ntile;
+    int w = wg - z * ntile, tiles_m = g.tiles_m, tiles_n = g.tiles_n;
+    if constexpr (PART) {
+      const int p = __builtin_amdgcn_readfirstlane((w >= g.pr[1].tile0) + (w >= g.pr[2].tile0) + (w >= g.pr[3].tile0));
+      w -= pick(p, [](const WProb& q) { return q.tile0; });
+      tiles_m = pick(p, [](const WProb& q) { return q.tiles_m; });
+      tiles_n = pick(p, [](const WProb& q) { return q.tiles_n; });
+      T.p = p;
+      T.M = pick(p, [](const WProb& q) { return q.M; });
+      T.N = pick(p, [](const WProb& q) { return q.N; });
+      T.lda = pick(p, [](const WProb& q) { return q.lda; });
+      T.ldb = pick(p, [](const WProb& q) { return q.ldb; });
+      T.A = pick(p, [](const WProb& q) { return q.A; });
+      T.B = pick(p, [](const WProb& q) { return q.B; });
+    } else {
+      T.p = 0;
+      T.M = g.M;
+      T.N = g.N;
+      T.lda = g.lda;
+      T.ldb = g.ldb;
+      T.A = g.A;
+      T.B = g.B;
+    }
     int tm, tn;
     if (g.group > 0) {
-      const int per = g.group * g.tiles_n, grp = w / per, first = grp * g.group;
-      const int gm = min(g.tiles_m - first, g.group), loc = w - grp * per;
+      const int per = g.group * tiles_n, grp = w / per, first = grp * g.group;
+      const int gm = min(tiles_m - first, g.group), loc = w - grp * per;
       tm = first + loc % gm;
       tn = loc / gm;
     } else {
-      tm = w / g.tiles_n;
-      tn = w - tm * g.tiles_n;
+      tm = w / tiles_n;
+      tn = w - tm * tiles_n;
     }
     T.m0 = __builtin_amdgcn_readfirstlane(tm * BM);
     T.n0 = __builtin_amdgcn_readfirstlane(tn * BN);
@@ -80,23 +109,23 @@
   };
   auto rsrc_a = [&](const Tile& T) {
     const int kb = T.z * g.kslice;
-    const bf16_t* abase = AK ? g.A + (long)T.m0 * g.lda + kb : g.A + (long)kb * g.lda + T.m0;
-    return make_rsrc(abase, AK ? clampb((long)(g.M - T.m0) * g.lda * 2 - kb * 2L)
-                               : clampb(((long)(g.K - kb) * g.lda - T.m0) * 2));
+    const bf16_t* abase = AK ? T.A + (long)T.m0 * T.lda + kb : T.A + (long)kb * T.lda + T.m0;
+    return make_rsrc(abase, AK ? clampb((long)(T.M - T.m0) * T.lda * 2 - kb * 2L)
+                               : clampb(((long)(g.K - kb) * T.lda - T.m0) * 2));
   };
   auto rsrc_b = [&](const Tile& T) {
     const int kb = T.z * g.kslice;
-    const bf16_t* bbase = BKM ? g.B + (long)T.n0 * g.ldb + kb : g.B + (long)kb * g.ldb + T.n0;
-    return make_rsrc(bbase, BKM ? clampb((long)(g.N - T.n0) * g.ldb * 2 - kb * 2L)
-                                : clampb(((long)(g.K - kb) * g.ldb - T.n0) * 2));
+    const bf16_t* bbase = BKM ? T.B + (long)T.n0 * T.ldb + kb : T.B + (long)kb * T.ldb + T.n0;
+    return make_rsrc(bbase, BKM ? clampb((long)(T.N - T.n0) * T.ldb * 2 - kb * 2L)
+                                : clampb(((long)(g.K - kb) * T.ldb - T.n0) * 2));
   };
   const bool iss = DMAW == 8 || wave < DMAW;
   auto load_k = [&](__amdgpu_buffer_rsrc_t ra, __amdgpu_buffer_rsrc_t rb, const Tile& T, int t, int slot,
                     int lane) {
     LDS_AS char* s = smem + slot * STAGE;
     if (iss) {
-      stage<AK, BM, false, DMAW, BK, WNX, PB>(ra, g.lda, g.M - T.m0, t * BK, T.Keff, s, wave, lane);
-      stage<BKM, BN, DIRECT, DMAW, BK, WNX, PB>(rb, g.ldb, g.N - T.n0, t * BK, T.Keff, s + A_BYTES, wave, lane);
+      stage<AK, BM, false, DMAW, BK, WNX, PB>(ra, T.lda, T.M - T.m0, t * BK, T.Keff, s, wave, lane);
+      stage<BKM, BN, DIRECT, DMAW, BK, WNX, PB>(rb, T.ldb, T.N - T.n0, t * BK, T.Keff, s + A_BYTES, wave, lane);
     }
   };
   auto load_tile = [&](const Tile& T, int t, int slot, int lane) {
@@ -104,8 +133,8 @@
   };
   auto load_tile8 = [&](const Tile& T, int t, int slot, int lane) {
     LDS_AS char* s = smem + slot * STAGE;
-    stage<AK, BM, false, NWV, BK, WNX, PB>(rsrc_a(T), g.lda, g.M - T.m0, t * BK, T.Keff, s, wave, lane);
-    stage<BKM, BN, DIRECT, NWV, BK, WNX, PB>(rsrc_b(T), g.ldb, g.N - T.n0, t * BK, T.Keff, s + A_BYTES, wave, lane);
+    stage<AK, BM, false, NWV, BK, WNX, PB>(rsrc_a(T), T.lda, T.M - T.m0, t * BK, T.Keff, s, wave, lane);
+    stage<BKM, BN, DIRECT, NWV, BK, WNX, PB>(rsrc_b(T), T.ldb, T.N - T.n0, t * BK, T.Keff, s + A_BYTES, wave, lane);
   };
 
   constexpr int RTR = EPI == EPI_ROPE ? (ROPE_TAB_MAX + NT - 1) / NT : 0;
@@ -339,7 +368,7 @@
 #pragma unroll
       for (int j = 0; j < NTN; ++j) acc[i][j] = f32x4{0.f, 0.f, 0.f, 0.f};
     if constexpr (RS) {
-      rs_on = g.rsum && cur.n0 == 0;
+      rs_on = pick(cur.p, [](const WProb& q) { return q.rsum; }) != nullptr && cur.n0 == 0;
       rsa = rsb = 0.f;
     }
     if constexpr (F8) {
@@ -520,6 +549,8 @@
       }
 
       const __amdgpu_buffer_rsrc_t ra = rsrc_a(cur), rb = rsrc_b(cur);
+      int lane_k = lane;
+      if constexpr (PART) asm volatile("" : "+v"(lane_k));
       constexpr bool SPREAD = NWV == 8 && !F8 && BK == 64;
       constexpr int SPLIT = MH == 4 ? SPLIT_AT : MH - 1;
       auto ktile = [&](const int t, auto tail_c) {
@@ -574,10 +605,10 @@
         if constexpr (!TAIL) {
           if constexpr (SPREAD) {
             if (iss)
-              stage<AK, BM, false, DMAW, BK, WNX, PB>(ra, g.lda, g.M - cur.m0, (t + 2) * BK, cur.Keff,
-                                                       smem + sl * STAGE, wave, lane);
+              stage<AK, BM, false, DMAW, BK, WNX, PB>(ra, cur.lda, cur.M - cur.m0, (t + 2) * BK, cur.Keff,
+                                                       smem + sl * STAGE, wave, lane_k);
           } else {
-            load_k(ra, rb, cur, t + 2, sl, lane);
+            load_k(ra, rb, cur, t + 2, sl, lane_k);
           }
         } else if (has_next) {
           int lt = lane;
@@ -592,8 +623,8 @@
         }
         auto b_pieces = [&] {
           if (iss)
-            stage<BKM, BN, DIRECT, DMAW, BK, WNX, PB>(rb, g.ldb, g.N - cur.n0, (t + 2) * BK, cur.Keff,
-                                                       smem + sl * STAGE + A_BYTES, wave, lane);
+            stage<BKM, BN, DIRECT, DMAW, BK, WNX, PB>(rb, cur.ldb, cur.N - cur.n0, (t + 2) * BK, cur.Keff,
+                                                       smem + sl * STAGE + A_BYTES, wave, lane_k);
         };
         if constexpr (F8) {
           if (t + 1 < nk) rdA8(Xa, sl ^ 1, 0);
@@ -849,9 +880,12 @@
           sa += __shfl_xor(sa, 32);
           sb += __shfl_xor(sb, 32);
           const int m = cur.m0 + wr * 128 + 32 * wc + (lane & 31);
-          if (lane < 32 && m < g.M) g.rsum[(long)cur.z * g.M + m] = lane < 16 ? sa : sb;
-        }
-      }
+          float* const rsum = pick(cur.p, [](const WProb& q) { return q.rsum; });
+          if (lane < 32 && m < cur.M) rsum[(long)cur.z * cur.M + m] = lane < 16 ? sa : sb;
+        }
+      }
+      [[maybe_unused]] float* ws = nullptr;
+      if constexpr (PART) ws = pick(cur.p, [](const WProb& q) { return q.ws; });
       bool ract[2] = {false, false};
       int rsh[2] = {0, 0}, rf0[2] = {0, 0}, rf1[2] = {0, 0};
       const int col = (lane % LPR) * 4;
@@ -905,7 +939,7 @@
           const f32x4 v4 = *(const LDS_AS f32x4*)(wl + row * STR + col);
           const int m = cur.m0 + wr * 128 + pass * PR + row;
           const int n = ncol;
-          if (m >= g.M || n >= g.N) continue;
+          if (m >= cur.M || n >= cur.N) continue;
           float v[4] = {v4[0] + bias4.x, v4[1] + bias4.y, v4[2] + bias4.z, v4[3] + bias4.w};
           if constexpr (EPI == EPI_BF16 || EPI == EPI_ROPE) {
             if constexpr (EPI == EPI_ROPE) {
@@ -924,7 +958,7 @@
           } else if constexpr (EPI == EPI_F32) {
             *(float4*)((float*)g.C + (long)m * g.ldc + n) = make_float4(v[0], v[1], v[2], v[3]);
           } else if constexpr (PART) {
-            *(float4*)(g.ws + ((long)cur.z * g.M + m) * g.N + n) = make_float4(v[0], v[1], v[2], v[3]);
+            *(float4*)(ws + ((long)cur.z * cur.M + m) * cur.N + n) = make_float4(v[0], v[1], v[2], v[3]);
           } else if constexpr (EPI == EPI_F32_RESID) {
             const float4 rr = rres[it];
             *(float4*)((float*)g.C + (long)m * g.ldc + n) = make_float4(rr.x + v[0], rr.y + v[1], rr.z + v[2], rr.w + v[3]);
@@ -1057,7 +1091,8 @@
 int launch_epi256(const G256& g, hipStream_t st, const Knobs& kn) {
   using Cfg = Cfg256<AK, BKM, EPI, BN, F8, NWV, BMT, STG>;
   if constexpr (Cfg::supported) {
-    const dim3 grid(grid256((long)g.tiles_m * g.tiles_n * g.nsplit, Cfg::BLOCKS_PER_CU, kn));
+    const long ntile = Cfg::PART ? g.ntile_all : (long)g.tiles_m * g.tiles_n;
+    const dim3 grid(grid256(ntile * g.nsplit, Cfg::BLOCKS_PER_CU, kn));
     hipLaunchKernelGGL((k_gemm256<AK, BKM, EPI, BN, F8, NWV, BMT, STG>), grid, dim3(Cfg::THREADS), 0, st, g);
     VJ_LAUNCH_CHECK("vj_gemm256");
     return VJ_OK;
@@ -1134,16 +1169,41 @@
   return launch_plan(p, a_kmajor, b_kmajor, epi, g, st, kn);
 }
 
+int vj_gemm256_partial_group(int np, const VjWgradProb* pr, int K, int kslice, int splitk, hipStream_t st);
+
 int vj_gemm256_partial(int M, int N, int K, const void* A, long lda, int a_kmajor, const void* B, long ldb,
                        int b_kmajor, int kslice, int splitk, float* ws, hipStream_t st, float* rsum) {
-  if (a_kmajor || b_kmajor || N % 8 || M < 256 || N < 128) return VJ_ERR_UNSUPPORTED;
+  if (a_kmajor || b_kmajor) return VJ_ERR_UNSUPPORTED;
+  const VjWgradProb one{A, lda, B, ldb, M, N, ws, rsum};
+  return vj_gemm256_partial_group(1, &one, K, kslice, splitk, st);
+}
+
+int vj_gemm256_partial_group(int np, const VjWgradProb* pr, int K, int kslice, int splitk, hipStream_t st) {
+  if (np < 1 || np > VJ_WGROUP_MAX) return VJ_ERR_UNSUPPORTED;
   const Knobs kn = read_knobs();
-  const Plan256 p{true, 256, wide_tile_ok(N) ? 256 : 128, 8, 0, 1, tile_group(kn)};
-  if ((long)vj_cdiv(M, p.bm) * vj_cdiv(N, p.bn) * splitk > 0x7fffffffL) return VJ_ERR_UNSUPPORTED;
-  G256 g{(const bf16_t*)A, (const bf16_t*)B, M, N, K, lda, ldb, nullptr, 0, nullptr, 0, nullptr, nullptr, 0,
-         0, 0, RopeP{}, kslice, splitk, ws, 0};
-  g.rsum = rsum;
-  return launch_plan(p, false, false, rsum ? EPI_PARTIAL_RS : EPI_PARTIAL, g, st, kn);
+  const Plan256 p{true, 256, wide_tile_ok(pr[0].N) ? 256 : 128, 8, 0, 1, tile_group(kn)};
+  G256 g{(const bf16_t*)pr[0].dy, (const bf16_t*)pr[0].x, pr[0].M, pr[0].N, K, pr[0].lddy, pr[0].ldx, nullptr, 0,
+         nullptr, 0, nullptr, nullptr, 0, 0, 0, RopeP{}, kslice, splitk, pr[0].ws, 0};
+  long tiles = 0;
+  bool rs = false;
+  for (int i = 0; i < VJ_WGROUP_MAX; ++i) {
+    WProb& q = g.pr[i];
+    if (i >= np) {
+      q = WProb{};
+      q.tile0 = 0x7fffffff;
+      continue;
+    }
+    const VjWgradProb& s = pr[i];
+    if (s.N % 8 || s.M < 256 || s.N < 128 || (wide_tile_ok(s.N) ? 256 : 128) != p.bn) return VJ_ERR_UNSUPPORTED;
+    q = WProb{(const bf16_t*)s.dy, (const bf16_t*)s.x, s.lddy, s.ldx, s.ws, s.rsum, s.M, s.N,
+              vj_cdiv(s.M, p.bm), vj_cdiv(s.N, p.bn), (int)tiles};
+    tiles += (long)q.tiles_m * q.tiles_n;
+    rs = rs || s.rsum;
+    if (tiles * splitk > 0x7fffffffL) return VJ_ERR_UNSUPPORTED;
+  }
+  g.ntile_all = (int)tiles;
+  g.rsum = pr[0].rsum;
+  return launch_plan(p, false, false, rs ? EPI_PARTIAL_RS : EPI_PARTIAL, g, st, kn);
 }
 
 extern "C" int vj_gemm_bf16(int M, int N, int K, const void* A, long lda, int a_kmajor, const void* B, long ldb,
diff --git a/vjepa2_amd/csrc/vj_gemm_tile.h b/vjepa2_amd/csrc/vj_gemm_tile.h
--- a/vjepa2_amd/csrc/vj_gemm_tile.h
+++ b/vjepa2_amd/csrc/vj_gemm_tile.h
@@ -5,6 +5,17 @@
 
 
 using RopeP = VjRope;
+
+struct WProb {
+  const bf16_t* A;
+  const bf16_t* B;
+  long lda, ldb;
+  float* ws;
+  float* rsum;
+  int M, N;
+  int tiles_m, tiles_n;
+  int tile0;
+};
 
 struct G256 {
   const bf16_t* A;
@@ -27,6 +38,8 @@
   const int* ea = nullptr;
   const int* eb = nullptr;
   float* rsum = nullptr;
+  int ntile_all = 0;
+  WProb pr[VJ_WGROUP_MAX] = {};
 };
 
 constexpr int BK = 64;
@@ -144,6 +157,10 @@
 
 struct Tile {
   int m0, n0, z, Keff, nk;
+  int p, M, N;
+  long lda, ldb;
+  const bf16_t* A;
+  const bf16_t* B;
 };
 
 __device__ __forceinline__ float bf_lo(uint32_t u) { return __builtin_bit_cast(float, u << 16); }
diff --git a/vjepa2_amd/functions.py b/vjepa2_amd/functions.py
--- a/vjepa2_amd/functions.py
+++ b/vjepa2_amd/functions.py
@@ -98,6 +98,11 @@
     buf, acc = wgrad_buf(w)
     db = _bias_buf(lin) if lin is not None else None
     ops.linear_wgrad(dy, x, buf if shape is None else buf.view(*shape), accumulate=acc, db=db)
+
+
+def wgrad_group(*items):
+    ops.linear_wgrad_group([(dy, x, *wgrad_buf(w), _bias_buf(lin) if lin is not None else None)
+                            for dy, x, w, lin in items])
 
 
 _ROPE_TABLES = {}
@@ -438,6 +443,11 @@
         dl = ops.linear_dgrad(dx1, weight_bf16(mlp.fc1.weight), wt=weight_bf16_t(mlp.fc1.weight))
         return ops.linear_dgrad(dx2, weight_bf16(mlp.fc2.weight), wt=weight_bf16_t(mlp.fc2.weight), resid=dl)
     dgelu, act = saved
+    if p == 0 and ops.wgrad_can_group(dy_b.shape[0], mlp.fc2.weight.shape, mlp.fc1.weight.shape):
+        dpre = ops.linear_dgrad(dy_b, weight_bf16(mlp.fc2.weight), gelu_grad=dgelu, wt=weight_bf16_t(mlp.fc2.weight))
+        with _OnWgradStream(dy_b, act, dpre, ln2):
+            wgrad_group((dy_b, act, mlp.fc2.weight, None), (dpre, ln2, mlp.fc1.weight, mlp.fc1))
+        return ops.linear_dgrad(dpre, weight_bf16(mlp.fc1.weight), wt=weight_bf16_t(mlp.fc1.weight))
     with _OnWgradStream(dy_b, act):
         wgrad(dy_b, act, mlp.fc2.weight)
     if p > 0:
@@ -478,8 +488,10 @@
     if not fused:
         dxm_b = _branch_grad(dxm, scales and scales[0], dc.pp if dc else 0.0, dc.sp if dc else 0)
         _bias_grad(attn.proj, dxm_b)
-    with _OnWgradStream(dxm_b, o):
-        wgrad(dxm_b, o, attn.proj.weight)
+    grouped = ops.wgrad_can_group(T, attn.proj.weight.shape, attn.qkv.weight.shape)
+    if not grouped:
+        with _OnWgradStream(dxm_b, o):
+            wgrad(dxm_b, o, attn.proj.weight)
     do = ops.linear_dgrad(dxm_b, weight_bf16(attn.proj.weight), wt=weight_bf16_t(attn.proj.weight))
     rope = None
     if attn.use_rope:
@@ -487,8 +499,12 @@
         rope = (lay.ids, lay.ids_mod, lay.tpf, lay.tpr, c, s)
     dqkv = ops.attn_bwd(qkv, o, do, stats, H, hd, lay.groups, _attn_scale(attn, hd, lay), rope=rope, fblk=lay.fblk,
                         dropout_p=dc.pa if dc else 0.0, seed=dc.sa if dc else 0)
-    with _OnWgradStream(dqkv, ln1):
-        wgrad(dqkv, ln1, attn.qkv.weight, lin=attn.qkv)
+    if grouped:
+        with _OnWgradStream(dxm_b, o, dqkv, ln1):
+            wgrad_group((dxm_b, o, attn.proj.weight, None), (dqkv, ln1, attn.qkv.weight, attn.qkv))
+    else:
+        with _OnWgradStream(dqkv, ln1):
+            wgrad(dqkv, ln1, attn.qkv.weight, lin=attn.qkv)
     dln1 = ops.linear_dgrad(dqkv, weight_bf16(attn.qkv.weight), wt=weight_bf16_t(attn.qkv.weight))
     gw, gb = _ln_grads(blk.norm1)
     dxi, dxi_b = ops.layernorm_bwd(dln1, x, m1, r1, blk.norm1.weight, dres_in=dxm, dweight=gw, dbias=gb,
@@ -562,7 +578,9 @@
         dy = ops.dropout(dy, dc.pp, dc.sp).float()
     dy_b = ops.cast_bf16(dy)
     do = ops.linear_dgrad(dy_b, weight_bf16(attn.proj.weight), wt=weight_bf16_t(attn.proj.weight))
-    wgrad(dy_b, o, attn.proj.weight)
+    grouped = ops.wgrad_can_group(dy_b.shape[0], attn.proj.weight.shape, attn.qkv.weight.shape)
+    if not grouped:
+        wgrad(dy_b, o, attn.proj.weight)
     _bias_grad(attn.proj, dy)
     rope = None
     if attn.use_rope:
@@ -571,7 +589,10 @@
     dqkv = ops.attn_bwd(qkv, o, do, stats, H, hd, lay.groups, _attn_scale(attn, hd, lay), rope=rope, fblk=lay.fblk,
                         dropout_p=dc.pa if dc else 0.0, seed=dc.sa if dc else 0)
     dx = ops.linear_dgrad(dqkv, weight_bf16(attn.qkv.weight), wt=weight_bf16_t(attn.qkv.weight))
-    wgrad(dqkv, x, attn.qkv.weight, lin=attn.qkv)
+    if grouped:
+        wgrad_group((dy_b, o, attn.proj.weight, None), (dqkv, x, attn.qkv.weight, attn.qkv))
+    else:
+        wgrad(dqkv, x, attn.qkv.weight, lin=attn.qkv)
     return dx
 
 
diff --git a/vjepa2_amd/ops.py b/vjepa2_amd/ops.py
--- a/vjepa2_amd/ops.py
+++ b/vjepa2_amd/ops.py
@@ -1,5 +1,6 @@
 
 import ctypes
+import functools
 import os
 
 import torch
@@ -124,6 +125,98 @@
         if best_t is None or t < best_t * 0.98:
             best, best_t = s, t
     return best
+
+
+def wgrad_group_time(shapes, K, s, cus=256):
+    tn = 256 if wgrad_wide_tile(shapes[0][1]) else 128
+    tiles = sum(-(-M // 256) * -(-N // tn) for M, N in shapes)
+    waves = -(-tiles * s // cus)
+    return waves * (K / s) * 256 * tn * 2 / 3.9e12 + (s * sum(M * N for M, N in shapes) * 8 / 5.0e12 if s > 1 else 0.0)
+
+
+def wgrad_groupable(M, N):
+    return M >= 256 and N >= 128 and M % 8 == 0 and N % 8 == 0
+
+
+def wgrad_group_splitk(shapes, K, cus=None):
+    return _wgrad_group_splitk(tuple((int(M), int(N)) for M, N in shapes), int(K), 256 if cus is None else cus)
+
+
+@functools.lru_cache(maxsize=None)
+def _wgrad_group_splitk(shapes, K, cus):
+    if len(shapes) == 1:
+        return wgrad_splitk(shapes[0][0], shapes[0][1], K, cus)
+    assert all(wgrad_groupable(M, N) for M, N in shapes), shapes
+    assert len({wgrad_wide_tile(N) for _, N in shapes}) == 1, "a group has one column-tile width"
+    best, best_t = 1, None
+    for s in range(1, max(1, K // 512) + 1):
+        t = wgrad_group_time(shapes, K, s, cus)
+        if best_t is None or t < best_t * 0.98:
+            best, best_t = s, t
+    single = sum(wgrad_group_time([mn], K, wgrad_splitk(mn[0], mn[1], K, cus), cus) for mn in shapes)
+    return best if best_t <= single else 0
+
+
+def wgrad_group_enabled():
+    return os.environ.get("VJ_WGRAD_GROUP", "1") != "0"
+
+
+def wgrad_can_group(tokens, *shapes):
+    shapes = tuple(tuple(s) for s in shapes)
+    if not (wgrad_group_enabled() and 2 <= len(shapes) <= 4 and all(wgrad_groupable(M, N) for M, N in shapes)
+            and len({wgrad_wide_tile(N) for _, N in shapes}) == 1):
+        return False
+    return _effective_splitk(tokens, wgrad_group_splitk(shapes, tokens)) > 1
+
+
+def _ptr_array(ts):
+    return (ctypes.c_void_p * len(ts))(*[_p(t) for t in ts])
+
+
+def linear_wgrad_group(items):
+    groups = {}
+    for i, (dy, x, dw, acc, db) in enumerate(items):
+        N, K = dw.shape
+        ok = (wgrad_group_enabled() and wgrad_groupable(N, K) and dy.dtype == BF16 and x.dtype == BF16
+              and (db is None or _WGRAD_BIAS) and dy.shape[0] == items[0][0].shape[0])
+        groups.setdefault(("w", wgrad_wide_tile(K)) if ok else ("s", i), []).append(i)
+    launched = []
+    for key, idx in groups.items():
+        tokens = items[idx[0]][0].shape[0]
+        s = 1
+        shapes = [tuple(items[i][2].shape) for i in idx[:4]]
+        if key[0] == "w" and wgrad_can_group(tokens, *shapes):
+            idx = idx[:4]
+            s = _effective_splitk(tokens, wgrad_group_splitk(shapes, tokens))
+        if s == 1:
+            for i in groups[key]:
+                dy, x, dw, acc, db = items[i]
+                linear_wgrad(dy, x, dw, accumulate=acc, db=db)
+                launched.append([i])
+            continue
+        sel = [items[i] for i in idx]
+        for dy, x, dw, acc, db in sel:
+            _dev(dy, x, dw, db)
+            assert x.shape[0] == tokens and dw.dtype == F32 and dw.shape == (dy.shape[1], x.shape[1])
+            assert db is None or (db.dtype == F32 and db.numel() == dw.shape[0] and db.is_contiguous())
+        n = len(sel)
+        ws = torch.empty(s * sum(dw.numel() + dw.shape[0] for _, _, dw, _, _ in sel), dtype=F32, device=sel[0][0].device)
+        ia = lambda v: (ctypes.c_int * n)(*v)
+        la = lambda v: (ctypes.c_long * n)(*v)
+        flops = sum(2.0 * tokens * dw.numel() for _, _, dw, _, _ in sel)
+        _call("vj_gemm_bf16_wgrad_group", n, ia([t[2].shape[0] for t in sel]), ia([t[2].shape[1] for t in sel]), tokens,
+              _ptr_array([t[0] for t in sel]), la([_rowmajor(t[0], "dy") for t in sel]),
+              _ptr_array([t[1] for t in sel]), la([_rowmajor(t[1], "x") for t in sel]),
+              _ptr_array([t[2] for t in sel]), la([_rowmajor(t[2], "dw") for t in sel]),
+              ia([int(t[3]) for t in sel]), _ptr_array([t[4] for t in sel]), ia([1] * n), s, _p(ws), ws.numel(),
+              _stream(), flops=flops,
+              label="k_gemm<0,0,wgrad+bias>" if any(t[4] is not None for t in sel) else "k_gemm<0,0,EPI_F32>[splitk]")
+        launched.append(list(idx))
+        for i in groups[key][4:]:
+            dy, x, dw, acc, db = items[i]
+            linear_wgrad(dy, x, dw, accumulate=acc, db=db)
+            launched.append([i])
+    return launched
 
 
 def linear_fwd(x, w, bias=None, epi=EPI_BF16, out=None, out2=None, resid=None):
```

New measurement: 236.7 clips/s (median of 6 runs). No clear change (+0.7%).
